# markp-gc/ipu_ray_lib

Measured on AMD Instinct MI355X. Metric: rays/sec (ray casts/s: CompactBvh intersect+occluded calls, whole node), built-in scene 1440x1440 path-trace, higher is better.
Workload: dtype f32

## Files before the change

__graft_entry__.py:

```python
from __future__ import annotations

import os
import shutil
import subprocess
import sys
from pathlib import Path

ROOT = Path(__file__).resolve().parent
PKG = ROOT / "ipu_ray_lib_amd"
CSRC = PKG / "csrc"

HOST_SRCS = [CSRC / "host" / n for n in ("bvh_sah.cpp", "lbvh.cpp", "glb_reader.cpp", "dae_reader.cpp", "scene_builtin.cpp", "scene_api.cpp", "nif_assets.cpp", "point_query_host.cpp", "box_query_host.cpp", "cross_host.cpp", "hot_order.cpp")]
HOST_DEPS = HOST_SRCS + [CSRC / "ray_math.h", CSRC / "hot_order.hpp", CSRC / "point_math.hpp", CSRC / "box_math.hpp", CSRC / "cross_math.hpp", CSRC / "canon_prims.hpp", CSRC / "bvh_cost_host.hpp", CSRC / "scene_blob.hpp", CSRC / "ray_shard.hpp", CSRC / "host" / "scene_types.hpp", CSRC / "host" / "json_min.hpp",
                         ROOT / "include" / "mi_raylib.h", ROOT / "include" / "mi_scene_host.h"]
HIP_SRCS = [CSRC / "raylib.hip"]
HIP_DEPS = HIP_SRCS + [CSRC / "ray_math.h", CSRC / "trace_kernels.hpp", CSRC / "trace_wavefront.hpp", CSRC / "hot_order.hpp", CSRC / "query_kernels.hpp", CSRC / "point_kernels.hpp", CSRC / "point_math.hpp", CSRC / "count_kernels.hpp", CSRC / "list_kernels.hpp", CSRC / "near_kernels.hpp", CSRC / "box_kernels.hpp", CSRC / "box_math.hpp", CSRC / "cross_math.hpp", CSRC / "refit_kernels.hpp", CSRC / "rebuild_kernels.hpp", CSRC / "canon_prims.hpp", CSRC / "canon_kernels.hpp", CSRC / "cost_kernels.hpp", CSRC / "bvh_cost_host.hpp", CSRC / "trace_pool.hpp", CSRC / "nif_kernels.hpp", CSRC / "nif_regs_pack.hpp", CSRC / "nif_regs_kernel.hpp", CSRC / "nif_asm_kernel.hpp", CSRC / "nif_asm_gen.py", CSRC / "scene_blob.hpp", CSRC / "ray_shard.hpp", CSRC / "group_render.hpp", CSRC / "query_drivers.hpp", ROOT / "include" / "mi_raylib.h"]

EXACT_FLAGS = ["-ffp-contract=off", "-fno-fast-math"]


def _deps_hash(deps, flags=()) -> str:
    import hashlib
    h = hashlib.sha256()
    for f in flags:
        h.update(str(f).encode() + b"\0")
    for d in sorted(str(x) for x in deps):
        q = Path(d)
        h.update(q.name.encode() + b"\0")
        if q.exists() and q.is_file():
            h.update(q.read_bytes())
    return h.hexdigest()


def _sidecar(target: Path) -> Path:
    return target.with_name(target.name + ".srchash")


def _stale(target: Path, deps, flags=()) -> bool:
    side = _sidecar(target)
    if not target.exists() or not side.exists():
        return True
    return side.read_text().strip() != _deps_hash(deps, flags)


def _record(target: Path, deps, flags=()) -> None:
    _sidecar(target).write_text(_deps_hash(deps, flags) + "\n")


class StaleBinary(RuntimeError):
    pass


def _run(cmd, **kw):
    if os.environ.get("MI_NO_BUILD") == "1":
        raise StaleBinary(f"stale binary: MI_NO_BUILD=1 forbids running `{' '.join(str(c) for c in cmd[:3])} ...` here; run "
                          "`python3 -c 'import __graft_entry__ as ge; ge.build()'` first, without a profiler")
    print("+", " ".join(str(c) for c in cmd), file=sys.stderr, flush=True)
    try:
        sys.stderr.fileno()
        kw.setdefault("stdout", sys.stderr)
    except (AttributeError, OSError, ValueError):
        kw.setdefault("stdout", sys.__stderr__)
    subprocess.run([str(c) for c in cmd], check=True, **kw)


def build_host() -> Path:
    out = PKG / "libmi_scene_host.so"
    if _stale(out, HOST_DEPS):
        _run(["g++", "-std=c++17", "-O2", *EXACT_FLAGS, "-fPIC", "-Wall", "-shared", "-o", out, *HOST_SRCS, "-ldl"])
        _record(out, HOST_DEPS)
    build_h5_plugin()
    return out


def hdf5_root():
    for cand in (os.environ.get("MI_HDF5_ROOT"), "/opt/conda", "/usr", "/usr/local"):
        if cand and (Path(cand) / "include" / "hdf5.h").exists() and (Path(cand) / "lib" / "libhdf5.so").exists():
            return Path(cand)
    return None


def build_h5_plugin():
    out = PKG / "libmi_nif_h5.so"
    src = CSRC / "host" / "nif_h5.c"
    root = hdf5_root()
    if root is None:
        print("note: no HDF5 installation found; converted.hdf5 NIF models cannot be read (nif_weights.bin still can)", file=sys.stderr)
        return None
    if _stale(out, [src]):
        _run(["gcc", "-std=c11", "-O2", "-fPIC", "-Wall", "-shared", "-I", root / "include", "-o", out, src,
              f"-L{root / 'lib'}", "-lhdf5", f"-Wl,-rpath,{root / 'lib'}"])
        _record(out, [src])
    return out


def build_oracle() -> Path:
    out = ROOT / "oracle" / "libray_oracle.so"
    deps = [ROOT / "oracle" / "ray_oracle.c", ROOT / "oracle" / "ray_oracle.h", ROOT / "oracle" / "Makefile"]
    if _stale(out, deps):
# ... 198 lines not shown
```

include/mi_scene_host.h:

```cpp
#ifndef MI_SCENE_HOST_H
#define MI_SCENE_HOST_H

#include "mi_raylib.h"

#ifdef __cplusplus
extern "C" {
#endif

typedef struct mi_host_scene mi_host_scene;

int mi_host_scene_builtin(const char* scene_name, const char* mesh_file, mi_host_scene** out);

int mi_host_scene_import(const char* file, int load_normals, mi_host_scene** out);

int mi_host_scene_from_arrays(const mi_scene_desc* geometry_only, mi_host_scene** out);

int mi_host_scene_fill_desc(const mi_host_scene* scene, mi_scene_desc* desc);

void mi_host_scene_destroy(mi_host_scene* scene);

int mi_build_compact_bvh(const float* lower, const float* upper, const uint16_t* geom_ids,
                         const uint32_t* prim_ids, uint32_t n,
                         mi_bvh_node* nodes, uint32_t* num_nodes, uint32_t* max_leaf_depth);

int mi_refit_compact_bvh(const mi_scene_desc* desc, mi_bvh_node* out);

int mi_build_lbvh_compact(const mi_scene_desc* desc, mi_bvh_node* out, uint32_t* num_nodes, uint32_t* max_leaf_depth);

int mi_canonical_prims(const mi_scene_desc* desc, void* out , uint32_t capacity, uint32_t* count);

int mi_bvh_cost_compact(const mi_bvh_node* nodes, uint32_t n, double out[3]);
int mi_bvh_cost_compact_block(const mi_bvh_node* nodes, uint32_t n, uint32_t block, double out[3]);
double mi_bvh_cost_estimate(const double cost[3]);

int mi_point_query_host(const mi_scene_desc* desc, int kind, const mi_point* points, void* out, size_t n, uint64_t visits[2]);

int mi_near_offsets_host(const mi_scene_desc* desc, const mi_point* points, uint64_t* offsets , size_t n, uint64_t visits[2]);
int mi_near_fill_host(const mi_scene_desc* desc, const mi_point* points, const uint64_t* offsets, mi_neighbour* hits, size_t capacity,
                      size_t n, uint64_t visits[2]);

int mi_box_query_host(const mi_scene_desc* desc, int kind, const mi_box* boxes, void* out, size_t n, uint64_t visits[2]);
int mi_box_offsets_host(const mi_scene_desc* desc, const mi_box* boxes, uint64_t* offsets , size_t n, uint64_t visits[2]);
int mi_box_fill_host(const mi_scene_desc* desc, const mi_box* boxes, const uint64_t* offsets, mi_overlap* hits, size_t capacity,
                     size_t n, uint64_t visits[2]);

uint32_t mi_sphere_crossings_host(const float centre[3], float radius2, const float origin[3], const float direction[3],
                                  float t_min, float t_max);

uint32_t mi_sphere_roots_host(const float centre[3], float radius2, const float origin[3], const float direction[3],
                              float t_min, float t_max, float t[2]);

int mi_hot_nodes(const mi_bvh_node* compact, uint32_t num_nodes, void* preorder, uint32_t* order, void* hot, uint32_t* leaf_link);

int mi_hot_share(const void* preorder, uint32_t num_nodes, const uint32_t* order, double* share);

uint32_t mi_hot_walk(const void* nodes, uint32_t num_nodes, const uint32_t* leaf_link, const float origin[3], const float direction[3],
                     uint32_t* visits, uint32_t capacity, int* status);

int mi_hot_collapse(const mi_bvh_node* compact, uint32_t num_nodes, double theta, void* preorder, uint8_t* keep, uint32_t* from, void* collapsed,
                    uint32_t* order, void* hot, uint32_t* leaf_link, double* share, uint32_t counts[2]);

int mi_hot_join(const void* thin, const uint32_t* thin_link, uint32_t m, const void* full, const uint32_t* full_link, uint32_t n, void* joined, uint32_t* joined_link,
                uint32_t* exact_start);
int mi_hot_cast_is_literal(const float origin[3], const float direction[3]);

uint32_t mi_hot_walk_count(const void* nodes, uint32_t num_nodes, const uint32_t* leaf_link, uint32_t start, const float origin[3], const float direction[3], float t_max,
                           uint32_t* visits, uint32_t capacity, uint32_t* box_tests, int* status);

int mi_init_ray_stream(const mi_scene_desc* desc, mi_trace_result* rays, size_t capacity);

void mi_scale_rgb(mi_trace_result* rays, size_t n, float scale);

size_t mi_scene_blob_size(const mi_scene_desc* desc);
int mi_scene_serialise(const mi_scene_desc* desc, uint8_t* out, size_t capacity, size_t* written);
int mi_scene_deserialise(const uint8_t* blob, size_t size, mi_scene_desc* desc, size_t* consumed);
uint32_t mi_blob_padding(uint32_t base_align, size_t offset, uint32_t align);

size_t mi_shard_band_rays(size_t n, uint32_t window_w);
size_t mi_shard_count(size_t n, size_t band, uint32_t replicas, uint32_t r);
int mi_shard_stream_index(size_t n, size_t band, uint32_t replicas, uint32_t r, uint64_t* out, size_t capacity);
int mi_shard_frame_index(size_t n, size_t band, uint32_t replicas, uint64_t* out);

typedef struct mi_host_nif mi_host_nif;

typedef struct mi_nif_desc {
  uint32_t num_layers;
  const float* const* kernels;
  const float* const* biases;
  const uint32_t* rows;
  const uint32_t* cols;
  const uint8_t* relu;
  uint32_t embedding_dimension;
  uint32_t hidden_size;
  float max_value;
  float mean[3];
  int32_t log_tonemap;
  int32_t weights_are_half;
  const char* name;
  const char* source;
} mi_nif_desc;

int mi_host_nif_load(const char* asset_path, mi_host_nif** out);
int mi_host_nif_describe(const mi_host_nif* nif, mi_nif_desc* desc);
void mi_host_nif_destroy(mi_host_nif* nif);
const char* mi_host_nif_last_error(void);

const char* mi_host_last_error(void);

#ifdef __cplusplus
}
#endif
#endif
```

ipu_ray_lib_amd/__init__.py:

```python
from __future__ import annotations

import ctypes as C
import os
import sys
from pathlib import Path

import numpy as np

PKG_DIR = Path(__file__).resolve().parent
REPO_ROOT = PKG_DIR.parent
DEFAULT_MESH = REPO_ROOT / "assets" / "monkey_bust.glb"

VEC3 = np.dtype([("x", "<f4"), ("y", "<f4"), ("z", "<f4")])
RAY = np.dtype([("origin", VEC3), ("tMin", "<f4"), ("direction", VEC3), ("tMax", "<f4")])
HIT = np.dtype([("r", RAY), ("primID", "<u4"), ("normal", VEC3), ("throughput", VEC3),
                ("geomID", "<u2"), ("flags", "<u2")])
TRACE_RESULT = np.dtype([("rgb", VEC3), ("u", "<f4"), ("v", "<f4"), ("h", HIT)])
BVH_NODE = np.dtype([("min_x", "<f4"), ("min_y", "<f4"), ("min_z", "<f4"), ("link", "<u4"),
                     ("dx", "<u2"), ("dy", "<u2"), ("dz", "<u2"), ("geomID", "<u2")])
MATERIAL = np.dtype([("albedo", VEC3), ("ior", "<f4"), ("emission", VEC3), ("type", "<i4"),
                     ("emissive", "u1"), ("pad", "u1", (3,))])
MESH_INFO = np.dtype([("firstIndex", "<u4"), ("firstVertex", "<u4"), ("numTriangles", "<u4"), ("numVertices", "<u4")])
GEOM_REF = np.dtype([("index", "<u2"), ("type", "u1"), ("pad", "u1")])
SPHERE = np.dtype([("x", "<f4"), ("y", "<f4"), ("z", "<f4"), ("radius", "<f4")])
# ... 78 lines not shown
class SceneGeometry(C.Structure):
    _fields_ = [("geometry", C.c_void_p), ("num_geometry", C.c_uint32),
                ("mesh_info", C.c_void_p), ("num_meshes", C.c_uint32),
                ("mat_ids", C.c_void_p), ("num_mat_ids", C.c_uint32),
                ("materials", C.c_void_p), ("num_materials", C.c_uint32),
                ("mesh_tris", C.c_void_p), ("num_tris", C.c_uint32),
                ("mesh_verts", C.c_void_p), ("num_verts", C.c_uint32),
                ("mesh_normals", C.c_void_p), ("num_normals", C.c_uint32),
                ("spheres", C.c_void_p), ("num_spheres", C.c_uint32),
                ("discs", C.c_void_p), ("num_discs", C.c_uint32)]

    @classmethod
    def from_desc(cls, desc: "SceneDesc") -> "SceneGeometry":
        g = cls()
        for name, _ in cls._fields_:
            setattr(g, name, getattr(desc, name))
        return g


CANON_PRIM = np.dtype([("a", "<u4"), ("b", "<u4"), ("c", "<u4"), ("kind", "<u4"), ("geomID", "<u4"), ("primID", "<u4"),
                       ("triBase", "<u4"), ("matIndex", "<u4")])
assert CANON_PRIM.itemsize == 32


class NifDesc(C.Structure):
    _fields_ = [("num_layers", C.c_uint32), ("kernels", C.POINTER(C.POINTER(C.c_float))),
                ("biases", C.POINTER(C.POINTER(C.c_float))), ("rows", C.POINTER(C.c_uint32)),
                ("cols", C.POINTER(C.c_uint32)), ("relu", C.POINTER(C.c_uint8)),
                ("embedding_dimension", C.c_uint32), ("hidden_size", C.c_uint32), ("max_value", C.c_float),
                ("mean", C.c_float * 3), ("log_tonemap", C.c_int32), ("weights_are_half", C.c_int32),
                ("name", C.c_char_p), ("source", C.c_char_p)]


class RaylibError(RuntimeError):
    pass


_host = None
_device = {}


def _load(path: Path) -> C.CDLL:
    if not path.exists():
        raise RaylibError(f"{path.name} is not built (run `python -c 'import __graft_entry__ as g; g.build()'` at the repo root)")
    return C.CDLL(str(path))


def host_lib() -> C.CDLL:
    global _host
    if _host is None:
        lib = _load(Path(os.environ["MI_SCENE_HOST_LIB"]) if os.environ.get("MI_SCENE_HOST_LIB") else PKG_DIR / "libmi_scene_host.so")
        lib.mi_host_last_error.restype = C.c_char_p
        lib.mi_host_scene_builtin.argtypes = [C.c_char_p, C.c_char_p, C.POINTER(C.c_void_p)]
        lib.mi_host_scene_import.argtypes = [C.c_char_p, C.c_int, C.POINTER(C.c_void_p)]
        lib.mi_host_scene_from_arrays.argtypes = [C.POINTER(SceneDesc), C.POINTER(C.c_void_p)]
        lib.mi_host_scene_fill_desc.argtypes = [C.c_void_p, C.POINTER(SceneDesc)]
        lib.mi_host_scene_destroy.argtypes = [C.c_void_p]
        lib.mi_host_scene_destroy.restype = None
        lib.mi_build_compact_bvh.argtypes = [C.c_void_p, C.c_void_p, C.c_void_p, C.c_void_p, C.c_uint32,
                                             C.c_void_p, C.POINTER(C.c_uint32), C.POINTER(C.c_uint32)]
        lib.mi_refit_compact_bvh.argtypes = [C.POINTER(SceneDesc), C.c_void_p]
        lib.mi_build_lbvh_compact.argtypes = [C.POINTER(SceneDesc), C.c_void_p, C.POINTER(C.c_uint32), C.POINTER(C.c_uint32)]
        lib.mi_canonical_prims.argtypes = [C.POINTER(SceneDesc), C.c_void_p, C.c_uint32, C.POINTER(C.c_uint32)]
        lib.mi_point_query_host.argtypes = [C.POINTER(SceneDesc), C.c_int, C.c_void_p, C.c_void_p, C.c_size_t, C.POINTER(C.c_uint64)]
        lib.mi_near_offsets_host.argtypes = [C.POINTER(SceneDesc), C.c_void_p, C.c_void_p, C.c_size_t, C.POINTER(C.c_uint64)]
        lib.mi_near_fill_host.argtypes = [C.POINTER(SceneDesc), C.c_void_p, C.c_void_p, C.c_void_p, C.c_size_t, C.c_size_t, C.POINTER(C.c_uint64)]
        lib.mi_box_query_host.argtypes = [C.POINTER(SceneDesc), C.c_int, C.c_void_p, C.c_void_p, C.c_size_t, C.POINTER(C.c_uint64)]
        lib.mi_box_offsets_host.argtypes = [C.POINTER(SceneDesc), C.c_void_p, C.c_void_p, C.c_size_t, C.POINTER(C.c_uint64)]
        lib.mi_box_fill_host.argtypes = [C.POINTER(SceneDesc), C.c_void_p, C.c_void_p, C.c_void_p, C.c_size_t, C.c_size_t, C.POINTER(C.c_uint64)]
        lib.mi_sphere_crossings_host.argtypes = [C.POINTER(C.c_float), C.c_float, C.POINTER(C.c_float), C.POINTER(C.c_float), C.c_float, C.c_float]
        lib.mi_sphere_crossings_host.restype = C.c_uint32
        lib.mi_sphere_roots_host.argtypes = [C.POINTER(C.c_float), C.c_float, C.POINTER(C.c_float), C.POINTER(C.c_float), C.c_float, C.c_float, C.POINTER(C.c_float)]
        lib.mi_sphere_roots_host.restype = C.c_uint32
        lib.mi_hot_nodes.argtypes = [C.c_void_p, C.c_uint32, C.c_void_p, C.c_void_p, C.c_void_p, C.c_void_p]
        lib.mi_hot_walk.argtypes = [C.c_void_p, C.c_uint32, C.c_void_p, C.POINTER(C.c_float), C.POINTER(C.c_float), C.c_void_p, C.c_uint32, C.POINTER(C.c_int)]
        lib.mi_hot_walk.restype = C.c_uint32
        lib.mi_hot_share.argtypes = [C.c_void_p, C.c_uint32, C.c_void_p, C.c_void_p]
        lib.mi_hot_collapse.argtypes = [C.c_void_p, C.c_uint32, C.c_double] + [C.c_void_p] * 8 + [C.POINTER(C.c_uint32)]
        lib.mi_hot_join.argtypes = [C.c_void_p, C.c_void_p, C.c_uint32, C.c_void_p, C.c_void_p, C.c_uint32, C.c_void_p, C.c_void_p, C.POINTER(C.c_uint32)]
        lib.mi_hot_cast_is_literal.argtypes = [C.POINTER(C.c_float), C.POINTER(C.c_float)]
        lib.mi_hot_walk_count.argtypes = [C.c_void_p, C.c_uint32, C.c_void_p, C.c_uint32, C.POINTER(C.c_float), C.POINTER(C.c_float), C.c_float, C.c_void_p, C.c_uint32,
                                          C.POINTER(C.c_uint32), C.POINTER(C.c_int)]
        lib.mi_hot_walk_count.restype = C.c_uint32
        lib.mi_bvh_cost_compact.argtypes = [C.c_void_p, C.c_uint32, C.POINTER(C.c_double)]
        lib.mi_bvh_cost_compact_block.argtypes = [C.c_void_p, C.c_uint32, C.c_uint32, C.POINTER(C.c_double)]
        lib.mi_bvh_cost_estimate.argtypes = [C.POINTER(C.c_double)]
        lib.mi_bvh_cost_estimate.restype = C.c_double
        lib.mi_init_ray_stream.argtypes = [C.POINTER(SceneDesc), C.c_void_p, C.c_size_t]
        lib.mi_scale_rgb.argtypes = [C.c_void_p, C.c_size_t, C.c_float]
        lib.mi_scale_rgb.restype = None
        lib.mi_scene_blob_size.argtypes = [C.POINTER(SceneDesc)]
        lib.mi_scene_blob_size.restype = C.c_size_t
        lib.mi_scene_serialise.argtypes = [C.POINTER(SceneDesc), C.c_void_p, C.c_size_t, C.POINTER(C.c_size_t)]
        lib.mi_scene_deserialise.argtypes = [C.c_void_p, C.c_size_t, C.POINTER(SceneDesc), C.POINTER(C.c_size_t)]
        lib.mi_blob_padding.argtypes = [C.c_uint32, C.c_size_t, C.c_uint32]
        lib.mi_blob_padding.restype = C.c_uint32
        lib.mi_shard_band_rays.argtypes = [C.c_size_t, C.c_uint32]
        lib.mi_shard_band_rays.restype = C.c_size_t
        lib.mi_shard_count.argtypes = [C.c_size_t, C.c_size_t, C.c_uint32, C.c_uint32]
        lib.mi_shard_count.restype = C.c_size_t
        lib.mi_shard_stream_index.argtypes = [C.c_size_t, C.c_size_t, C.c_uint32, C.c_uint32, C.c_void_p, C.c_size_t]
        lib.mi_shard_frame_index.argtypes = [C.c_size_t, C.c_size_t, C.c_uint32, C.c_void_p]
        lib.mi_host_nif_load.argtypes = [C.c_char_p, C.POINTER(C.c_void_p)]
        lib.mi_host_nif_describe.argtypes = [C.c_void_p, C.POINTER(NifDesc)]
        lib.mi_host_nif_destroy.argtypes = [C.c_void_p]
        lib.mi_host_nif_destroy.restype = None
        lib.mi_host_nif_last_error.restype = C.c_char_p
        _host = lib
    return _host


def device_lib(variants: bool = False) -> C.CDLL:
    global _device
    if variants not in _device:
        try:
            import torch
        except ImportError:
            pass
        if variants:
            lib = _load(Path(os.environ["MI_RAYLIB_VARIANTS_LIB"]) if os.environ.get("MI_RAYLIB_VARIANTS_LIB") else PKG_DIR / "libmi_raylib_variants.so")
        else:
            lib = _load(Path(os.environ["MI_RAYLIB_LIB"]) if os.environ.get("MI_RAYLIB_LIB") else PKG_DIR / "libmi_raylib.so")
        lib.mi_last_error.restype = C.c_char_p
        lib.mi_version.restype = C.c_char_p
        lib.mi_scene_create.argtypes = [C.POINTER(SceneDesc), C.POINTER(C.c_void_p)]
        lib.mi_scene_create_from_blob.argtypes = [C.c_void_p, C.c_size_t, C.POINTER(SceneDesc), C.POINTER(C.c_void_p)]
        lib.mi_scene_destroy.argtypes = [C.c_void_p]
        lib.mi_scene_destroy.restype = None
        lib.mi_render.argtypes = [C.c_void_p, C.c_int, C.c_void_p, C.c_size_t, C.c_void_p, C.c_void_p]
        lib.mi_render_device.argtypes = [C.c_void_p, C.c_int, C.c_void_p, C.c_size_t, C.c_void_p]
        lib.mi_trace_time_secs.argtypes = [C.c_void_p]
        lib.mi_trace_time_secs.restype = C.c_double
        lib.mi_get_counters.argtypes = [C.c_void_p, C.POINTER(C.c_uint64)]
        lib.mi_reset_counters.argtypes = [C.c_void_p]
        lib.mi_get_phase_stats.argtypes = [C.c_void_p, C.POINTER(C.c_uint64)]
        lib.mi_scene_set_nif.argtypes = [C.c_void_p, C.c_uint32, C.c_void_p, C.c_void_p, C.c_void_p, C.c_void_p,
                                         C.c_void_p, C.c_uint32, C.c_float, C.c_void_p, C.c_int32]
        lib.mi_scene_set_hdri_rotation.argtypes = [C.c_void_p, C.c_float]
        lib.mi_scene_set_max_nif_batch.argtypes = [C.c_void_p, C.c_size_t]
        lib.mi_scene_set_ray_batch.argtypes = [C.c_void_p, C.c_size_t]
        lib.mi_nif_infer_device.argtypes = [C.c_void_p, C.c_void_p, C.c_void_p, C.c_void_p, C.c_size_t, C.c_void_p]
        lib.mi_query.argtypes = [C.c_void_p, C.c_int, C.c_void_p, C.c_void_p, C.c_size_t]
        lib.mi_scene_update.argtypes = [C.c_void_p, C.POINTER(GeometryUpdate)]
        lib.mi_scene_update_device.argtypes = [C.c_void_p, C.POINTER(GeometryUpdate), C.c_void_p]
        lib.mi_scene_rebuild.argtypes = [C.c_void_p, C.c_void_p, C.POINTER(C.c_uint32)]
        lib.mi_scene_set_geometry.argtypes = [C.c_void_p, C.POINTER(SceneGeometry), C.POINTER(C.c_uint32)]
        lib.mi_scene_set_geometry_device.argtypes = [C.c_void_p, C.POINTER(SceneGeometry), C.c_void_p, C.POINTER(C.c_uint32)]
        lib.mi_get_rebuild_timing.argtypes = [C.c_void_p, C.POINTER(C.c_double)]
        lib.mi_scene_get_bvh.argtypes = [C.c_void_p, C.c_void_p, C.c_uint32, C.POINTER(C.c_uint32)]
        lib.mi_scene_bvh_cost.argtypes = [C.c_void_p, C.c_void_p, C.POINTER(C.c_double)]
        lib.mi_get_live_stats.argtypes = [C.c_void_p, C.POINTER(C.c_uint64)]
        lib.mi_query_device.argtypes = [C.c_void_p, C.c_int, C.c_void_p, C.c_void_p, C.c_size_t, C.c_void_p]
        lib.mi_point_query.argtypes = [C.c_void_p, C.c_int, C.c_void_p, C.c_void_p, C.c_size_t]
        lib.mi_point_query_device.argtypes = [C.c_void_p, C.c_int, C.c_void_p, C.c_void_p, C.c_size_t, C.c_void_p]
        lib.mi_count_query.argtypes = [C.c_void_p, C.c_void_p, C.c_void_p, C.c_size_t]
        lib.mi_count_query_device.argtypes = [C.c_void_p, C.c_void_p, C.c_void_p, C.c_size_t, C.c_void_p]
        lib.mi_list_offsets.argtypes = [C.c_void_p, C.c_void_p, C.c_void_p, C.c_size_t]
        lib.mi_list_offsets_device.argtypes = [C.c_void_p, C.c_void_p, C.c_void_p, C.c_size_t, C.c_void_p]
        lib.mi_list_fill.argtypes = [C.c_void_p, C.c_void_p, C.c_void_p, C.c_void_p, C.c_size_t, C.c_size_t]
        lib.mi_list_fill_device.argtypes = [C.c_void_p, C.c_void_p, C.c_void_p, C.c_void_p, C.c_size_t, C.c_size_t, C.c_void_p]
        lib.mi_near_offsets.argtypes = [C.c_void_p, C.c_void_p, C.c_void_p, C.c_size_t]
        lib.mi_near_offsets_device.argtypes = [C.c_void_p, C.c_void_p, C.c_void_p, C.c_size_t, C.c_void_p]
        lib.mi_near_fill.argtypes = [C.c_void_p, C.c_void_p, C.c_void_p, C.c_void_p, C.c_size_t, C.c_size_t]
        lib.mi_near_fill_device.argtypes = [C.c_void_p, C.c_void_p, C.c_void_p, C.c_void_p, C.c_size_t, C.c_size_t, C.c_void_p]
        lib.mi_box_query.argtypes = [C.c_void_p, C.c_int, C.c_void_p, C.c_void_p, C.c_size_t]
        lib.mi_box_query_device.argtypes = [C.c_void_p, C.c_int, C.c_void_p, C.c_void_p, C.c_size_t, C.c_void_p]
# ... 228 lines not shown
    _check_host(host_lib().mi_box_query_host(C.byref(desc), int(kind), src.ctypes.data if src.size else None,
                                             out.ctypes.data if src.size else None, src.size, visits))
    return (out.view(np.bool_) if kind == BOX_ANY else out), {"box_tests": int(visits[0]), "prim_evals": int(visits[1])}


def box_offsets_host(desc: SceneDesc, boxes: np.ndarray):
    assert boxes.dtype == BOX and boxes.ndim == 1
    src = np.ascontiguousarray(boxes)
    offsets = np.zeros(src.size + 1, np.uint64)
    visits = (C.c_uint64 * 2)()
    _check_host(host_lib().mi_box_offsets_host(C.byref(desc), src.ctypes.data if src.size else None, offsets.ctypes.data, src.size, visits))
    return offsets, {"box_tests": int(visits[0]), "prim_evals": int(visits[1])}


def box_fill_host(desc: SceneDesc, boxes: np.ndarray, offsets: np.ndarray, capacity: int | None = None, hits: np.ndarray | None = None):
    assert boxes.dtype == BOX and boxes.ndim == 1
    src = np.ascontiguousarray(boxes)
    offsets = np.ascontiguousarray(offsets, np.uint64)
    assert offsets.ndim == 1 and offsets.size == src.size + 1
    if hits is None:
        size = int(offsets.max()) if capacity is None else int(capacity)
        hits = np.zeros(max(size, 1), OVERLAP)[:size]
    assert hits.dtype == OVERLAP and hits.flags["C_CONTIGUOUS"]
    capacity = hits.size if capacity is None else int(capacity)
    assert 0 <= capacity <= hits.size
    visits = (C.c_uint64 * 2)()
    base = hits.ctypes.data if hits.size else np.zeros(1, OVERLAP).ctypes.data
    _check_host(host_lib().mi_box_fill_host(C.byref(desc), src.ctypes.data if src.size else None, offsets.ctypes.data, base, capacity, src.size, visits))
    return hits, {"box_tests": int(visits[0]), "prim_evals": int(visits[1])}


DEVICE_NODE = np.dtype([("box", "<f4", (6,)), ("link", "<u4"), ("hit", "<u4")])


def hot_nodes(nodes: np.ndarray) -> dict:
    nodes = np.ascontiguousarray(nodes, dtype=BVH_NODE)
    n = nodes.size
    out = {"preorder": np.zeros(n, DEVICE_NODE), "order": np.zeros(n, np.uint32), "hot": np.zeros(n, DEVICE_NODE), "leaf_link": np.zeros(n, np.uint32)}
    _check_host(host_lib().mi_hot_nodes(nodes.ctypes.data if n else None, n, *[out[k].ctypes.data if n else None for k in ("preorder", "order", "hot", "leaf_link")]))
    out["share"] = np.zeros(n, np.float64)
    _check_host(host_lib().mi_hot_share(out["preorder"].ctypes.data if n else None, n, out["order"].ctypes.data if n else None, out["share"].ctypes.data if n else None))
    return out


def hot_walk(device_nodes: np.ndarray, origin, direction, leaf_link: np.ndarray | None = None) -> np.ndarray:
    assert device_nodes.dtype == DEVICE_NODE and device_nodes.flags.c_contiguous
    o, d = ((C.c_float * 3)(*[float(np.float32(x)) for x in v]) for v in (origin, direction))
    link = None if leaf_link is None else np.ascontiguousarray(leaf_link, np.uint32)
    cap = 4 * device_nodes.size + 4
    visits = np.zeros(cap, np.uint32)
    status = C.c_int(0)
    cnt = host_lib().mi_hot_walk(device_nodes.ctypes.data, device_nodes.size, None if link is None else link.ctypes.data, o, d, visits.ctypes.data, cap, C.byref(status))
    _check_host(status.value)
    return visits[:min(cnt, cap)].copy()


def hot_collapse(nodes: np.ndarray, theta: float = -1.0) -> dict:
    nodes = np.ascontiguousarray(nodes, dtype=BVH_NODE)
    n = nodes.size
    out = {"preorder": np.zeros(n, DEVICE_NODE), "keep": np.zeros(n, np.uint8), "from": np.zeros(n, np.uint32), "collapsed": np.zeros(n, DEVICE_NODE),
           "order": np.zeros(n, np.uint32), "hot": np.zeros(n, DEVICE_NODE), "leaf_link": np.zeros(n, np.uint32), "share": np.zeros(n, np.float64)}
    counts = (C.c_uint32 * 2)()
    _check_host(host_lib().mi_hot_collapse(nodes.ctypes.data if n else None, n, float(theta),
                                           *[out[k].ctypes.data if n else None for k in ("preorder", "keep", "from", "collapsed", "order", "hot", "leaf_link", "share")], counts))
    m = int(counts[0])
    for k in ("from", "collapsed", "order", "hot", "leaf_link", "share"):
        out[k] = out[k][:m].copy()
    out["blocked"] = int(counts[1])
    return out


def hot_join(collapse: dict, full: dict) -> dict:
    m, n = collapse["hot"].size, full["hot"].size
    out = {"nodes": np.zeros(m + n, DEVICE_NODE), "leaf_link": np.zeros(m + n, np.uint32)}
    start = C.c_uint32(0)
    ptr = lambda a: a.ctypes.data if a.size else None
    _check_host(host_lib().mi_hot_join(ptr(collapse["hot"]), ptr(collapse["leaf_link"]), m, ptr(full["hot"]), ptr(full["leaf_link"]), n, ptr(out["nodes"]), ptr(out["leaf_link"]),
                                       C.byref(start)))
    out["exact_start"] = int(start.value)
    out["place"] = np.concatenate([collapse["from"][collapse["order"]], full["order"]]).astype(np.uint32)
    return out


def hot_cast_is_literal(origin, direction) -> bool:
    o, d = ((C.c_float * 3)(*[float(np.float32(x)) for x in v]) for v in (origin, direction))
    return bool(host_lib().mi_hot_cast_is_literal(o, d))


def hot_walk_count(device_nodes: np.ndarray, origin, direction, leaf_link: np.ndarray | None = None, t_max: float = float("inf"), start: int = 0):
    assert device_nodes.dtype == DEVICE_NODE and device_nodes.flags.c_contiguous
    o, d = ((C.c_float * 3)(*[float(np.float32(x)) for x in v]) for v in (origin, direction))
    link = None if leaf_link is None else np.ascontiguousarray(leaf_link, np.uint32)
    cap = 4 * device_nodes.size + 4
    visits = np.zeros(cap, np.uint32)
    status, tests = C.c_int(0), C.c_uint32(0)
    cnt = host_lib().mi_hot_walk_count(device_nodes.ctypes.data, device_nodes.size, None if link is None else link.ctypes.data, int(start), o, d, C.c_float(float(np.float32(t_max))),
                                       visits.ctypes.data, cap, C.byref(tests), C.byref(status))
    _check_host(status.value)
    return visits[:min(cnt, cap)].copy(), int(tests.value)


def sphere_crossings_host(centre, radius2, origin, direction, t_min=0.0, t_max=float("inf")) -> int:
    c, o, d = ((C.c_float * 3)(*[float(np.float32(x)) for x in v]) for v in (centre, origin, direction))
    return int(host_lib().mi_sphere_crossings_host(c, C.c_float(float(np.float32(radius2))), o, d, C.c_float(float(np.float32(t_min))),
                                                   C.c_float(float(np.float32(t_max)))))


def sphere_roots_host(centre, radius2, origin, direction, t_min=0.0, t_max=float("inf")):
    c, o, d = ((C.c_float * 3)(*[float(np.float32(x)) for x in v]) for v in (centre, origin, direction))
    t = (C.c_float * 2)(float("nan"), float("nan"))
    mask = int(host_lib().mi_sphere_roots_host(c, C.c_float(float(np.float32(radius2))), o, d, C.c_float(float(np.float32(t_min))),
                                               C.c_float(float(np.float32(t_max))), t))
    return mask, float(t[0]), float(t[1])


def _geometry_array(a, dtype, width):
    if a is None:
        return None
    a = np.asarray(a)
    if a.dtype != dtype:
        a = np.ascontiguousarray(a, dtype=np.float32)
        if a.ndim != 2 or a.shape[1] != width:
            raise ValueError(f"expected a {dtype} array or an [n, {width}] float32 array, got shape {a.shape}")
        return a.view(dtype).reshape(-1)
    return np.ascontiguousarray(a).reshape(-1)


def serialise_scene(desc: SceneDesc) -> np.ndarray:
    lib = host_lib()
    n = lib.mi_scene_blob_size(C.byref(desc))
    out = aligned_bytes(n)
    written = C.c_size_t()
    _check_host(lib.mi_scene_serialise(C.byref(desc), out.ctypes.data, n, C.byref(written)))
    assert written.value == n
    return out


def deserialise_scene(blob: np.ndarray, into: SceneDesc | None = None) -> SceneDesc:
    d = into if into is not None else SceneDesc()
    used = C.c_size_t()
    _check_host(host_lib().mi_scene_deserialise(blob.ctypes.data, blob.size, C.byref(d), C.byref(used)))
    d._blob = blob
    d._blob_bytes_used = used.value
    return d


class NifAssets:

    def __init__(self, asset_path):
        lib = host_lib()
        h = C.c_void_p()
        if lib.mi_host_nif_load(os.fspath(asset_path).encode(), C.byref(h)) != 0:
            raise RaylibError(lib.mi_host_nif_last_error().decode())
        try:
            d = NifDesc()
            if lib.mi_host_nif_describe(h, C.byref(d)) != 0:
                raise RaylibError(lib.mi_host_nif_last_error().decode())
            self.kernels, self.biases, self.relu = [], [], []
            for i in range(d.num_layers):
                r, c = int(d.rows[i]), int(d.cols[i])
                self.kernels.append(np.ctypeslib.as_array(d.kernels[i], shape=(r, c)).copy())
                self.biases.append(np.ctypeslib.as_array(d.biases[i], shape=(c,)).copy() if d.biases[i] else None)
                self.relu.append(bool(d.relu[i]))
            self.embedding_dimension = int(d.embedding_dimension)
            self.hidden_size = int(d.hidden_size)
            self.max_value = float(d.max_value)
# ... 681 lines not shown
```

ipu_ray_lib_amd/csrc/ray_math.h:

```cpp
#pragma once

#include <stdint.h>
#include <string.h>
#include <math.h>

#if defined(__HIPCC__)
#define MI_HD __host__ __device__ __forceinline__
#else
#define MI_HD inline
#endif

namespace mi {

struct f3 { float x, y, z; };

MI_HD f3 mk(float x, float y, float z) { f3 r; r.x = x; r.y = y; r.z = z; return r; }
MI_HD f3 operator+(f3 a, f3 b) { return mk(a.x + b.x, a.y + b.y, a.z + b.z); }
MI_HD f3 operator-(f3 a, f3 b) { return mk(a.x - b.x, a.y - b.y, a.z - b.z); }
MI_HD f3 operator*(f3 a, f3 b) { return mk(a.x * b.x, a.y * b.y, a.z * b.z); }
MI_HD f3 operator*(f3 a, float s) { return mk(a.x * s, a.y * s, a.z * s); }
MI_HD f3 operator-(f3 a) { return mk(-a.x, -a.y, -a.z); }
MI_HD f3 abs3(f3 a) { return mk(fabsf(a.x), fabsf(a.y), fabsf(a.z)); }
MI_HD float dot(f3 a, f3 b) { return a.x * b.x + a.y * b.y + a.z * b.z; }
MI_HD float sqnorm(f3 a) { return a.x * a.x + a.y * a.y + a.z * a.z; }
// ... 217 lines not shown
  return out;
}
MI_HD float rng_uniform01(Rng& r) {
  const uint64_t bits = (0x3FFull << 52) | (rng_next(r) >> 12);
  double d;
  __builtin_memcpy(&d, &bits, 8);
  return (float)(d - 1.0);
}

MI_HD uint32_t f2u_sat(float f) {
  if (!(f > 0.f)) return 0u;
  if (f >= 4294967296.f) return 0xFFFFFFFFu;
  return (uint32_t)f;
}
constexpr uint32_t kSegmentSamplesMin = 4, kSegmentSamplesMax = 64, kSegmentsPerPixel = 16;
MI_HD uint32_t segment_shift(uint32_t samplesPerPixel) {
  const uint32_t want = (samplesPerPixel + kSegmentsPerPixel - 1) / kSegmentsPerPixel;
  const uint32_t shift = want <= 1u ? 0u : 32u - (uint32_t)__builtin_clz(want - 1u);
  return shift < 2u ? 2u : shift > 6u ? 6u : shift;
}
MI_HD uint32_t segment_samples(uint32_t samplesPerPixel) { return 1u << segment_shift(samplesPerPixel); }
MI_HD void rng_seed_pixel_segment(Rng& r, uint64_t userSeed, float row, float col, uint32_t segment) {
  const uint64_t pix = ((uint64_t)f2u_sat(row) << 32) | (uint64_t)f2u_sat(col);
  rng_seed(r, (userSeed ^ ((pix + 1ull) * 0x9e3779b97f4a7c15ull)) ^ ((uint64_t)segment * 0xd1b54a32d192ed03ull));
}
MI_HD void rng_seed_pixel(Rng& r, uint64_t userSeed, float row, float col) { rng_seed_pixel_segment(r, userSeed, row, col, 0u); }

MI_HD float log_det(float x) {
  uint32_t b;
  __builtin_memcpy(&b, &x, 4);
  int e = (int)((b >> 23) & 0xFFu) - 126;
  const uint32_t mb = (b & 0x007FFFFFu) | 0x3F000000u;
  float m;
  __builtin_memcpy(&m, &mb, 4);
  if (m < 0.707106781186547524f) { e -= 1; m = m + m - 1.0f; }
  else { m = m - 1.0f; }
  float z = m * m;
  float y = 7.0376836292e-2f;
  y = y * m + -1.1514610310e-1f;
  y = y * m + 1.1676998740e-1f;
  y = y * m + -1.2420140846e-1f;
  y = y * m + 1.4249322787e-1f;
  y = y * m + -1.6668057665e-1f;
  y = y * m + 2.0000714765e-1f;
  y = y * m + -2.4999993993e-1f;
  y = y * m + 3.3333331174e-1f;
  y = y * m * z;
  const float fe = (float)e;
  y = y + -2.12194440e-4f * fe;
  y = y + -0.5f * z;
  z = m + y;
  z = z + 0.693359375f * fe;
  return z;
}
MI_HD void rng_gauss2(Rng& r, const float* sinTbl, float& g0, float& g1) {
  const float ua = rng_uniform01(r);
  const float ub = rng_uniform01(r);
  float w = 1.f - ua;
  if (w < 2.98023223876953125e-08f) w = 2.98023223876953125e-08f;
  const float rad = sqrtf(-2.f * log_det(w));
  float sn, cs;
  sincos_deg_table(6.283185307179586f * ub, sinTbl, sn, cs);
  g0 = rad * cs;
  g1 = rad * sn;
}

MI_HD f3 pixel_to_ray_dir(float x, float y, float w, float h, float tanTheta) {
  const float aspect = w / h;
  x = (x / w) - .5f;
  y = (y / h) - .5f;
  return normalized(mk(2.f * x * aspect * tanTheta, -2.f * y * tanTheta, -1.f));
}

MI_HD f3 offset_origin(f3 origin, f3 dir, f3 n) {
  const float m = (1.f + min_comp(abs3(origin))) * kRayEpsilon * copysignf(1.f, dot(n, dir));
  return origin + n * m;
}

MI_HD void sample_disc_concentric(float u1, float u2, const float* sinTbl, float& ox, float& oy) {
  const float ux = 2.f * u1 - 1.f, uy = 2.f * u2 - 1.f;
  if (ux == 0.f && uy == 0.f) { ox = ux; oy = uy; return; }
  const float piby4 = (float)(3.14159265358979323846264338327950288 / 4.0);
  const float piby2 = (float)(3.14159265358979323846264338327950288 / 2.0);
  float r, th;
  if (fabsf(ux) > fabsf(uy)) { r = ux; th = piby4 * (uy / ux); }
  else { r = uy; th = piby2 - piby4 * (ux / uy); }
  float s, c;
  sincos_deg_table(th, sinTbl, s, c);
  ox = r * c; oy = r * s;
}
MI_HD f3 cosine_sample_hemisphere(float u1, float u2, const float* sinTbl) {
  float x, y;
  sample_disc_concentric(u1, u2, sinTbl, x, y);
  const float z = sqrtf(fmaxf(0.f, 1.f - x * x - y * y));
  return mk(x, y, z);
}
MI_HD f3 sample_diffuse(f3 n, float u1, float u2, const float* sinTbl) {
  f3 xb;
  const f3 a = abs3(n), sq = n * n;
  if (a.x > a.y) { const float il = 1.f / sqrtf(sq.x + sq.z); xb = mk(-n.z * il, 0.f, n.x * il); }
  else { const float il = 1.f / sqrtf(sq.y + sq.z); xb = mk(0.f, n.z * il, -n.y * il); }
  const f3 yb = cross(n, xb);
  const f3 wi = cosine_sample_hemisphere(u1, u2, sinTbl);
  return mk(dot(mk(xb.x, yb.x, n.x), wi), dot(mk(xb.y, yb.y, n.y), wi), dot(mk(xb.z, yb.z, n.z), wi));
}
MI_HD f3 reflect_dir(f3 d, f3 n) {
  const float cosTheta = dot(d, n);
  return normalized(d - n * (cosTheta * 2.f));
}
MI_HD float schlick(float cosTheta, float ri) {
  float r0 = (1.f - ri) / (1.f + ri);
  r0 = r0 * r0;
  const float base = 1.f - cosTheta;
  const float base2 = base * base;
  const float base5 = base2 * base * base2;
  return r0 + (1.f - r0) * base5;
}
MI_HD f3 refract_dir(f3 dir, f3 n, float ndotr, float ri) {
  const float cosTheta = -ndotr;
  const f3 rPerp = (dir + n * cosTheta) * ri;
  const f3 rPar = n * -sqrtf(fabsf(1.f - sqnorm(rPerp)));
  return rPerp + rPar;
}
MI_HD bool dielectric(f3 dir, f3 n, float ri, float u1, f3& out) {
  if (dot(n, dir) > 0.f) n = -n; else ri = 1.f / ri;
  const float ndotr = dot(n, dir);
  const float cost1 = -ndotr;
  const float cost2 = 1.f - ri * ri * (1.f - cost1 * cost1);
  if (cost2 > 0.f && u1 > schlick(cost1, ri)) { out = refract_dir(dir, n, ndotr, ri); return true; }
  out = reflect_dir(dir, n);
  return false;
}
MI_HD bool roulette_stop(float u1, f3& tp) {
  const float p = min_comp(tp);
  if (p == 0.f || u1 > p) return true;
  tp = tp * (1.f / p);
  return false;
}

#define MI_SIN_TABLE_BITS \
  0x00000000u, 0x3c8ef859u, 0x3d0ef2c6u, 0x3d565e3au, 0x3d8edc7bu, 0x3db27eb6u, 0x3dd61305u, 0x3df996a2u, \
  0x3e0e8365u, 0x3e20305bu, 0x3e31d0d4u, 0x3e43636fu, 0x3e54e6cdu, 0x3e665992u, 0x3e77ba60u, 0x3e8483eeu, \
  0x3e8d2057u, 0x3e95b1beu, 0x3e9e377au, 0x3ea6b0dfu, 0x3eaf1d44u, 0x3eb77c01u, 0x3ebfcc6fu, 0x3ec80de9u, \
  0x3ed03fc9u, 0x3ed8616cu, 0x3ee0722fu, 0x3ee87171u, 0x3ef05e94u, 0x3ef838f7u, 0x3f000000u, 0x3f03d989u, \
  0x3f07a8cau, 0x3f0b6d77u, 0x3f0f2744u, 0x3f12d5e8u, 0x3f167918u, 0x3f1a108du, 0x3f1d9bfeu, 0x3f211b24u, \
  0x3f248dbbu, 0x3f27f37cu, 0x3f2b4c25u, 0x3f2e9772u, 0x3f31d522u, 0x3f3504f3u, 0x3f3826a7u, 0x3f3b39ffu, \
  0x3f3e3ebdu, 0x3f4134a6u, 0x3f441b7du, 0x3f46f30au, 0x3f49bb13u, 0x3f4c7360u, 0x3f4f1bbdu, 0x3f51b3f3u, \
  0x3f543bceu, 0x3f56b31du, 0x3f5919aeu, 0x3f5b6f51u, 0x3f5db3d7u, 0x3f5fe714u, 0x3f6208dau, 0x3f641901u, \
  0x3f66175eu, 0x3f6803cau, 0x3f69de1du, 0x3f6ba635u, 0x3f6d5becu, 0x3f6eff20u, 0x3f708fb2u, 0x3f720d81u, \
  0x3f737871u, 0x3f74d063u, 0x3f76153fu, 0x3f7746eau, 0x3f78654du, 0x3f797051u, 0x3f7a67e2u, 0x3f7b4bebu, \
  0x3f7c1c5cu, 0x3f7cd925u, 0x3f7d8235u, 0x3f7e1781u, 0x3f7e98fdu, 0x3f7f069eu, 0x3f7f605cu, 0x3f7fa62fu, \
  0x3f7fd814u, 0x3f7ff605u, 0x3f800000u, 0x3f7ff605u

}
```

ipu_ray_lib_amd/csrc/raylib.hip:

```cpp
#include <hip/hip_runtime.h>

#include <algorithm>
#include <chrono>
#include <cmath>
#include <cstdio>
#include <cstring>
#include <map>
#include <stdexcept>
#include <string>
#include <vector>

#include "../../include/mi_raylib.h"
#include "ray_math.h"
#include "trace_kernels.hpp"
#include "trace_wavefront.hpp"
#include "hot_order.hpp"
#include "query_kernels.hpp"
#include "point_kernels.hpp"
#include "count_kernels.hpp"
#include "list_kernels.hpp"
#include "near_kernels.hpp"
#include "box_kernels.hpp"
#include "refit_kernels.hpp"
#include "rebuild_kernels.hpp"
// ... 19 lines not shown
static_assert(sizeof(mi_ray) == 32, "Ray layout");
static_assert(sizeof(mi_bvh_node) == 24, "CompactBVH2Node layout");
static_assert(sizeof(mi_material) == 36, "Material layout");
static_assert(sizeof(mi_mesh_info) == 16 && sizeof(mi_geom_ref) == 4, "MeshInfo/GeomRef layout");
static_assert(offsetof(mi_trace_result, u) == 12 && offsetof(mi_trace_result, h) == 20, "TraceResult offsets");
static_assert(offsetof(mi_hit_record, prim_id) == 32 && offsetof(mi_hit_record, normal) == 36 &&
              offsetof(mi_hit_record, throughput) == 48 && offsetof(mi_hit_record, geom_id) == 60 &&
              offsetof(mi_hit_record, flags) == 62, "HitRecord offsets");
static_assert(sizeof(mi_query_hit) == 32 && offsetof(mi_query_hit, prim_id) == 4 && offsetof(mi_query_hit, geom_id) == 8 &&
              offsetof(mi_query_hit, flags) == 10 && offsetof(mi_query_hit, normal) == 12 && offsetof(mi_query_hit, b1) == 24 &&
              offsetof(mi_query_hit, b2) == 28, "mi_query_hit layout");
static_assert(sizeof(mi_point) == 16 && offsetof(mi_point, radius) == 12, "mi_point layout");
static_assert(sizeof(mi_point_hit) == 32 && offsetof(mi_point_hit, prim_id) == 4 && offsetof(mi_point_hit, geom_id) == 8 &&
              offsetof(mi_point_hit, flags) == 10 && offsetof(mi_point_hit, point) == 12 && offsetof(mi_point_hit, b1) == 24 &&
              offsetof(mi_point_hit, b2) == 28, "mi_point_hit layout");

namespace {

thread_local std::string g_err;

struct DeviceError : std::runtime_error { using std::runtime_error::runtime_error; };
struct ArgError : std::runtime_error { using std::runtime_error::runtime_error; };

#define HIP_CHECK(expr)                                                                      \
  do {                                                                                       \
    hipError_t _e = (expr);                                                                  \
    if (_e != hipSuccess)                                                                    \
      throw DeviceError(std::string(#expr) + ": " + hipGetErrorString(_e));                  \
  } while (0)

template <class F>
int guarded(F&& f) {
  try { f(); g_err.clear(); return MI_OK; }
  catch (const ArgError& e) { g_err = e.what(); return MI_ERR_INVALID_ARG; }
  catch (const DeviceError& e) { g_err = e.what(); return MI_ERR_DEVICE; }
  catch (const std::exception& e) { g_err = e.what(); return MI_ERR_DEVICE; }
  catch (...) { g_err = "unknown exception (not derived from std::exception)"; return MI_ERR_DEVICE; }
}

template <class T>
T* upload(const std::vector<T>& v) {
  if (v.empty()) return nullptr;
  T* d = nullptr;
  HIP_CHECK(hipMalloc(&d, v.size() * sizeof(T)));
  HIP_CHECK(hipMemcpy(d, v.data(), v.size() * sizeof(T), hipMemcpyHostToDevice));
  return d;
}

const float* hostSinTable() {
  static const uint32_t bits[92] = {MI_SIN_TABLE_BITS};
  static float tbl[92];
  static bool init = false;
  if (!init) { memcpy(tbl, bits, sizeof tbl); init = true; }
  return tbl;
}

}

constexpr uint32_t kNifSplDefault = 512, kNifSplMax = 1024;
constexpr int kHotNodesAuto = -1;
constexpr double kHotAutoShare = 0.9;
constexpr uint32_t kHotThreads = 768;
constexpr uint32_t kLdsPerCU = 160 * 1024, kLdsGranule = 1280;
struct SceneOptions {
  bool fullStats = false;
  WaveTune tune = kDefaultTune;
  int kernelChoice = 1;
#if MI_RAYLIB_VARIANTS
  PoolTune poolTune;
#endif
  uint32_t cus = 0;
  std::string why;
  int poolWaves = 4;
  int wavesPerSimd = 6;
  bool mergeTurns = true;
  bool specLeaf = false;
  bool tiles = true;
  size_t segBudgetKb = (size_t)8 * 1024 * 1024;
  uint32_t nifSamplesPerLaunch = 0;
  bool pin = true;
  uint32_t nifShape = 7;
  bool leafRot = true;
  bool leanHit = true;
  bool coords = true;
  int nifOverlap = -1;
  uint32_t nifTraceWgs = 0;
  uint32_t nifSplit = 0;
  bool nifFirstTest = false;
  bool nifTiming = false;
  bool refitTiming = false;
  bool rebuildTiming = false;
  uint32_t nifGenerations = kNifGenerations;
  bool rootStart = true;
  bool sayGrid = false;
  bool doubleFallback = false;
  bool fast = false;
  int queryKernel = 0;
  QueryTune queryTune = kDefaultQueryTune;
  int hotNodes = kHotNodesAuto;
  double autoRebuild = 0.0;

  static bool flag01(const char* v, bool& out) {
    if ((v[0] != '0' && v[0] != '1') || v[1] != '\0') return false;
    out = v[0] == '1';
    return true;
  }
  static bool number(const char* v, unsigned long long lo, unsigned long long hi, unsigned long long& out) {
    if (!*v) return false;
    char* end = nullptr;
    const unsigned long long q = strtoull(v, &end, 10);
    if (!end || *end != '\0' || v[0] == '-' || q < lo || q > hi) return false;
    out = q;
    return true;
  }
  static bool autoRebuildValue(const char* v, double& out) {
    if (!v || !*v) return false;
    if (!strcmp(v, "0")) { out = 0.0; return true; }
    for (const char* c = v; *c; ++c) if (!((*c >= '0' && *c <= '9') || *c == '.' || *c == 'e' || *c == 'E' || *c == '+' || *c == '-')) return false;
    char* end = nullptr;
    const double r = strtod(v, &end);
    if (!end || end == v || *end != '\0' || !(r > 1.0) || !std::isfinite(r)) return false;
    out = r;
    return true;
  }
  bool set(const std::string& key, const char* v) {
    why = "unknown option or bad value";
    if (!v) return false;
    unsigned long long q = 0;
    if (key == "full_stats") {
      bool b = fullStats;
      if (!flag01(v, b)) return false;
      if (b && fast) { why = "full_stats cannot be combined with fast (the tolerance tier has no instrumented build)"; return false; }
      fullStats = b; return true;
    }
#if MI_RAYLIB_VARIANTS
    if (fast && (key == "kernel" || key == "waves" || key == "spec" || key == "merge" || key == "tune")) {
      SceneOptions probe = *this; probe.fast = false;
      if (!probe.set(key, v)) { why = probe.why; return false; }
      if (probe.kernelChoice != 1 || probe.specLeaf || probe.wavesPerSimd != 6 || !probe.mergeTurns || !(probe.tune == kDefaultTune)) {
        why = "fast is a build of the default kernel only (kernel 1, 6 waves, one SHADE / GEN turn, default weights, no spec): clear fast first"; return false;
      }
      return true;
    }
    if (key == "kernel") { if (!number(v, 0, 3, q)) return false; kernelChoice = (int)q; return true; }
    if (key == "pool_waves") { if (!number(v, 4, 16, q) || (q != 4 && q != 8 && q != 16)) return false; poolWaves = (int)q; return true; }
    if (key == "pool_tune") {
      unsigned a, b, c, d, e, f, db = 4, mx = 5, ln = 1, pr = 1;
      if (sscanf(v, "%u,%u,%u,%u,%u,%u,%u,%u,%u,%u", &a, &b, &c, &d, &e, &f, &db, &mx, &ln, &pr) < 6) return false;
      poolTune = {a, b, c ? c : 1, d ? d : 1, e, f, db ? db : 65, mx, ln, pr};
      return true;
    }
    if (key == "waves") { if (!number(v, 4, 7, q)) return false; wavesPerSimd = (int)q; return true; }
    if (key == "spec") return flag01(v, specLeaf);
    if (key == "merge") return flag01(v, mergeTurns);
#else
    if (key == "kernel") {
      if (!number(v, 0, 3, q)) return false;
      if (q > 1) { why = "kernel 2 / 3 are not compiled into this library (the variants build, -DMI_RAYLIB_VARIANTS=1, has them)"; return false; }
      kernelChoice = (int)q; return true;
    }
    if (key == "pool_waves" || key == "pool_tune" || key == "tune") { why = "not compiled into this library (the variants build, -DMI_RAYLIB_VARIANTS=1, has it)"; return false; }
    if (key == "waves") { if (!number(v, 4, 7, q)) return false; if (q != 6) { why = "the 4-, 5- and 7-wave builds are not compiled into this library (variants build)"; return false; } return true; }
    if (key == "merge") { bool b = true; if (!flag01(v, b)) return false; if (!b) { why = "the two-turn form is not compiled into this library (variants build)"; return false; } return true; }
    if (key == "spec") { bool b = false; if (!flag01(v, b)) return false; if (b) { why = "the speculative walk is not compiled into this library (variants build)"; return false; } return true; }
#endif
    if (key == "cus") { if (!number(v, 0, 4096, q)) return false; cus = (uint32_t)q; return true; }
    if (key == "tiles") return flag01(v, tiles);
    if (key == "seg_budget_kb") { if (!number(v, 1, ~0ull >> 12, q)) return false; segBudgetKb = (size_t)q; return true; }
    if (key == "nif_spl") { if (!number(v, 0, kNifSplMax, q)) return false; nifSamplesPerLaunch = (uint32_t)q; return true; }
    if (key == "pin") return flag01(v, pin);
    if (key == "nif_timing") return flag01(v, nifTiming);
    if (key == "refit_timing") return flag01(v, refitTiming);
    if (key == "rebuild_timing") return flag01(v, rebuildTiming);
    if (key == "nif_generations") { if (!number(v, 1, 4096, q)) return false; nifGenerations = (uint32_t)q; return true; }
    if (key == "root_start") return flag01(v, rootStart);
    if (key == "say_grid") return flag01(v, sayGrid);
    if (key == "nif_overlap") { if (!strcmp(v, "auto")) { nifOverlap = -1; return true; } bool on = false; if (!flag01(v, on)) return false; nifOverlap = on ? 1 : 0; return true; }
    if (key == "nif_first_test") return flag01(v, nifFirstTest);
    if (key == "nif_split") { if (!number(v, 0, 1024, q)) return false; nifSplit = (uint32_t)q; return true; }
    if (key == "nif_trace_wgs") { if (!number(v, 0, 16, q)) return false; nifTraceWgs = (uint32_t)q; return true; }
    if (key == "coords") return flag01(v, coords);
    if (key == "query_kernel") { if (!number(v, 0, 1, q)) return false; queryKernel = (int)q; return true; }
    if (key == "query_tune") {
      unsigned a, b, c, dd, e;
      char tail = 0;
      if (sscanf(v, "%u,%u,%u,%u,%u%c", &a, &b, &c, &dd, &e, &tail) != 5) return false;
      if (b == 0 || dd == 0 || e > 8 || c > 64) return false;
      queryTune = {a, b, c, dd, e};
      return true;
    }
    if (key == "lean_hit") return flag01(v, leanHit);
    if (key == "auto_rebuild") { if (!autoRebuildValue(v, autoRebuild)) { why = "auto_rebuild takes 0 (off) or a decimal ratio above 1"; return false; } return true; }
    if (key == "leaf_rot") return flag01(v, leafRot);
    if (key == "hot_nodes") { if (!strcmp(v, "auto")) { hotNodes = kHotNodesAuto; return true; } if (!number(v, 0, 65535, q)) return false; hotNodes = (int)q; return true; }
    if (key == "double_fallback") {
      bool b = doubleFallback;
      if (!flag01(v, b)) return false;
      if (b && fast) { why = "double_fallback cannot be combined with fast"; return false; }
      doubleFallback = b; return true;
    }
    if (key == "fast") {
      bool b = fast;
      if (!flag01(v, b)) return false;
      if (b && (fullStats || doubleFallback)) { why = "fast cannot be combined with full_stats or double_fallback"; return false; }
#if MI_RAYLIB_VARIANTS
      if (b && (kernelChoice != 1 || specLeaf || wavesPerSimd != 6 || !mergeTurns || !(tune == kDefaultTune))) { why = "fast is a build of the default kernel only (kernel 1, 6 waves, one SHADE / GEN turn, default weights, no spec)"; return false; }
#endif
      fast = b; return true;
    }
    if (key == "nif_shape") {
      const std::string s(v);
      if (s == "w6") nifShape = 0; else if (s == "t6") nifShape = 1; else if (s == "t4") nifShape = 2; else if (s == "a8") nifShape = 6; else if (s == "auto") nifShape = 7; else if (s == "b4") nifShape = 8;
#if MI_RAYLIB_VARIANTS
      else if (s == "r8") nifShape = 4; else if (s == "r8s") nifShape = 5;
#else
      else if (s == "r8" || s == "r8s") { why = "K3r (nif_shape r8 / r8s) is not compiled into this library (the variants build, -DMI_RAYLIB_VARIANTS=1, has it)"; return false; }
#endif
      else return false;
      return true;
    }
#if MI_RAYLIB_VARIANTS
    if (key == "tune") {
      unsigned a, b, c, dd = 48, k8 = 3, db = 4, mx = 6, ln = 1, pr = 1, lp = 40, pb = 0;
      if (sscanf(v, "%u,%u,%u,%u,%u,%u,%u,%u,%u,%u,%u", &a, &b, &c, &dd, &k8, &db, &mx, &ln, &pr, &lp, &pb) < 3) return false;
      if (mx > 7 || pb > 3) return false;
      tune = {a, b, c, dd, k8, db ? db : 65, mx, ln, pr, lp ? lp : 1, pb};
      return true;
    }
#endif
    return false;
  }
  void fromEnvironment() {
    static const char* const map[][2] = {{"MI_RAYLIB_FULL_STATS", "full_stats"}, {"MI_RAYLIB_KERNEL", "kernel"}, {"MI_RAYLIB_WAVES", "waves"}, {"MI_RAYLIB_SPEC", "spec"},
                                         {"MI_RAYLIB_SEG_BUDGET_KB", "seg_budget_kb"}, {"MI_RAYLIB_NIF_SPL", "nif_spl"}, {"MI_RAYLIB_PIN", "pin"},
                                         {"MI_RAYLIB_NIF_SHAPE", "nif_shape"}, {"MI_RAYLIB_TUNE", "tune"},
                                         {"MI_RAYLIB_POOL_TUNE", "pool_tune"}, {"MI_RAYLIB_POOL_WAVES", "pool_waves"}, {"MI_RAYLIB_CUS", "cus"},
                                         {"MI_RAYLIB_NIF_OVERLAP", "nif_overlap"}, {"MI_RAYLIB_COORDS", "coords"},
                                         {"MI_RAYLIB_NIF_TRACE_WGS", "nif_trace_wgs"}, {"MI_RAYLIB_NIF_SPLIT", "nif_split"}, {"MI_RAYLIB_NIF_GENERATIONS", "nif_generations"},
                                         {"MI_RAYLIB_HOT_NODES", "hot_nodes"}};
    for (const auto& m : map) if (const char* e = getenv(m[0])) (void)set(m[1], e);
    if (getenv("MI_RAYLIB_NO_TILES")) tiles = false;
    if (getenv("MI_RAYLIB_NO_ROOT_START")) rootStart = false;
    if (getenv("MI_RAYLIB_SAY_GRID")) sayGrid = true;
  }
};

struct LaunchSlot {
  hipStream_t stream = nullptr;
  uint32_t* d_workCounter = nullptr;
  float* d_segPart = nullptr; size_t segPartFloats = 0;
  float2* d_coords = nullptr; size_t coordsCap = 0;
  uint32_t* d_poolScratch = nullptr; size_t poolScratchWords = 0;
  hipEvent_t lastWork = nullptr;
  uint64_t* d_scanSums = nullptr; size_t scanSumsCap = 0;
};

struct mi_scene {
  int device = 0;
  int numCUs = 256;
  mi_scene_desc params{};
  DeviceScene ds{};
  SceneOptions opt;
  std::vector<void*> allocations;
  unsigned long long* d_counters = nullptr;
  std::vector<LaunchSlot> slots;
  std::map<const void*, int> residentPerCU;
  uint32_t cus() const { return opt.cus ? opt.cus : (uint32_t)numCUs; }
  bool nifOverlapOn() const { return opt.nifOverlap < 0 ? (opt.nifSplit > 0 || !((opt.nifShape >= 6 && opt.nifShape <= 8) && nif_asm_covers(nif.regs))) : opt.nifOverlap != 0; }
  DeviceScene view() const { DeviceScene v = ds; if (!opt.rootStart) v.rootInterior = 0; return v; }
  struct HotCopy { const GNode* nodes = nullptr; const GLeaf* leaves = nullptr; const GLeafRot* rot = nullptr; const float* leafNormals = nullptr; bool valid = false;
                   uint32_t numNodes = 0, thinNodes = 0, exactBase = 0;
                   std::vector<double> share; } hot, thin;
  DeviceScene hotView(const HotCopy& c) const { DeviceScene v = view(); v.nodes = c.nodes; v.numNodes = c.numNodes; v.exactBase = c.exactBase; v.leaves = c.leaves; v.leavesRot = c.rot; v.leafNormals = c.leafNormals; return v; }
  DeviceScene& touchArrays() { hot.valid = false; thin.valid = false; return ds; }
  void freeRetiredHot() {
    if (hot.valid || thin.valid) return;
    for (const HotCopy* c : {&hot, &thin})
      for (const void* p : {(const void*)c->nodes, (const void*)c->leaves, (const void*)c->rot, (const void*)c->leafNormals}) release(p);
    hot = HotCopy{};
    thin = HotCopy{};
  }
  bool hotRoomSaid = false;
  std::map<const void*, uint32_t> hotRoomOf;
  uint32_t hotRoom(const void* kern, int threads) {
    auto it = hotRoomOf.find(kern);
    if (it != hotRoomOf.end()) return it->second;
    hipFuncAttributes fa{};
    int nb0 = 0;
    uint32_t room = 0;
    if (hipFuncGetAttributes(&fa, kern) == hipSuccess && hipOccupancyMaxActiveBlocksPerMultiprocessor(&nb0, kern, threads, 0) == hipSuccess && nb0 > 0) {
      long bytes = ((long)(kLdsPerCU / (uint32_t)nb0 / kLdsGranule * kLdsGranule) - (long)fa.sharedSizeBytes) & ~31L;
      for (; bytes >= 32; bytes -= 256) {
        int nb = 0;
        if (hipOccupancyMaxActiveBlocksPerMultiprocessor(&nb, kern, threads, (size_t)bytes) == hipSuccess && nb >= nb0) break;
      }
      if (bytes >= 32) room = (uint32_t)bytes;
    }
    (void)hipGetLastError();
    if (room && hipFuncSetAttribute(kern, hipFuncAttributeMaxDynamicSharedMemorySize, (int)room) != hipSuccess) { (void)hipGetLastError(); room = 0; }
    if (!room && !hotRoomSaid) {
      hotRoomSaid = true;
      fprintf(stderr, "mi_raylib: option hot_nodes: the runtime leaves no LDS for hot nodes beside a %d-thread workgroup's own; rendering from the shared arrays\n", threads);
    }
    hotRoomOf.emplace(kern, room);
    return room;
  }
  uint32_t residentBlocks(const void* kern, int threads, size_t ldsBytes) {
    auto it = residentPerCU.find(kern);
    if (it == residentPerCU.end()) {
      int nb = 0;
      if (hipOccupancyMaxActiveBlocksPerMultiprocessor(&nb, kern, threads, ldsBytes) != hipSuccess || nb <= 0) { (void)hipGetLastError(); nb = 8; }
      it = residentPerCU.emplace(kern, nb).first;
    }
    return (uint32_t)it->second;
  }
  bool poolAttrSet[2][3] = {{false, false, false}, {false, false, false}};
  bool ldsAttrSet[2] = {false, false};
  hipEvent_t nifDone = nullptr; bool nifPending = false;
  mi_trace_result* d_batch[2] = {nullptr, nullptr}; size_t batchCap[2] = {0, 0};
  hipStream_t pipeStream[2] = {nullptr, nullptr};
  double traceTimeSecs = 0.0;
  float hdriRotationDegrees = 0.f;
  size_t maxNifBatch = 0;
  size_t rayBatch = 0;
  void* d_qRays[2] = {nullptr, nullptr}; void* d_qOut[2] = {nullptr, nullptr}; size_t qCap[2] = {0, 0};
  NifDevice nif;
  struct NifSlots {
    float* u = nullptr; float* v = nullptr; float* bgr = nullptr; float* color = nullptr; float* tp = nullptr;
    uint32_t* index = nullptr; uint32_t* count = nullptr;
    hipEvent_t traced = nullptr, done = nullptr; bool donePending = false;
  } nifSlots[2];
  hipStream_t nifAux = nullptr;
  hipStream_t debugStream = nullptr;
  hipStream_t nifSplitMlp = nullptr, nifSplitTrace = nullptr;
  uint32_t splitUnits = 0; bool splitRefused = false;
  hipEvent_t splitFirst = nullptr;
  Rng* d_rng = nullptr; size_t scratchRays = 0;
  float* d_segTotal = nullptr;
  uint32_t scratchSamples = 0;
  uint32_t scratchAsked = 0;
  bool scratchOneSet = false;
  std::vector<std::pair<hipEvent_t, hipEvent_t>> nifTimes;
  struct Refit {
    std::vector<mi_bvh_node> nodes;
    bool tables = false; uint32_t levelCap = 0;
    std::vector<uint32_t> matIds;
    std::vector<mi_geom_ref> geometry; std::vector<mi_mesh_info> meshInfo; std::vector<uint16_t> tris;
    std::vector<mi_vec3> verts; std::vector<mi_sphere> spheres; std::vector<mi_disc> discs;
    uint32_t numVerts = 0, numNormals = 0, numSpheres = 0, numDiscs = 0;
    bool ready = false;
    RefitPrim* d_prims = nullptr;
    uint32_t* d_order = nullptr;
    std::vector<uint32_t> levelStart; uint32_t* d_levelStart = nullptr;
    uint32_t topFirst = 0;
    RefitBox* d_boxes = nullptr;
    mi_bvh_node* d_cnodes[2] = {nullptr, nullptr}; int live = -1;
// ... 163 lines not shown
        const mi_disc& c = d.discs[r.index];
        L.f[0] = c.nx; L.f[1] = c.ny; L.f[2] = c.nz; L.f[3] = c.cx; L.f[4] = c.cy; L.f[5] = c.cz; L.f[6] = c.r * c.r;
        L.type = LEAF_DISC | ((uint32_t)n.geom_id << 16); L.primID = 0;
      }
      L.matIndex = d.mat_ids[n.geom_id];
      g.hit = (skip[i] << 5) | kLeafFlag;
      leaves[i] = L;
      isLeafNode[i] = 1;
    }
    nodes[i] = g;
  }

  DeviceScene& ds = S.ds;
  ds.nodes = S.keep(upload(nodes)); ds.numNodes = N;
  ds.leaves = S.keep(upload(leaves)); ds.numLeaves = (uint32_t)leaves.size();
  struct Private { mi_scene::HotCopy* copy; std::vector<uint32_t> at, link; std::vector<GNode> nodes; } priv[2] = {{&S.hot, {}, {}, {}}, {&S.thin, {}, {}, {}}};
  {
    const HotNode* pre = reinterpret_cast<const HotNode*>(nodes.data());
    std::vector<uint8_t> keepNode(N);
    const uint32_t M = hot_collapse_keep(pre, N, kHotCollapseTheta, keepNode.data(), nullptr);
    std::vector<HotNode> thinPre(M);
    std::vector<uint32_t> thinFrom(M);
    hot_collapse_nodes(pre, N, keepNode.data(), thinPre.data(), thinFrom.data());
    need(M == 0 || (thinFrom[0] == 0 && (M == 1 || (thinPre[0].hit == 32u) == !node_is_leaf(nodes[0]))), "the collapsed tree lost its root");
    for (int c = 0; c < 2; ++c) {
      const HotNode* src = c ? thinPre.data() : pre;
      const uint32_t n = c ? M : N;
      std::vector<uint32_t> order(n);
      priv[c].nodes.resize(n);
      priv[c].link.resize(n);
      hot_first_order(src, n, order.data());
      hot_permute_nodes(src, n, order.data(), reinterpret_cast<HotNode*>(priv[c].nodes.data()), priv[c].link.data());
      priv[c].copy->share.resize(n);
      if (c) hot_prefix_share_any(src, n, order.data(), S.thin.share.data()); else hot_prefix_share(src, n, order.data(), S.hot.share.data());
      priv[c].at.resize(n);
      for (uint32_t k = 0; k < n; ++k) priv[c].at[k] = c ? thinFrom[order[k]] : order[k];
      priv[c].copy->numNodes = priv[c].copy->thinNodes = n;
    }
    {
      std::vector<GNode> joined(M + N);
      std::vector<uint32_t> joinedLink(M + N);
      hot_join_regions(reinterpret_cast<const HotNode*>(priv[1].nodes.data()), priv[1].link.data(), M, reinterpret_cast<const HotNode*>(priv[0].nodes.data()), priv[0].link.data(), N,
                       reinterpret_cast<HotNode*>(joined.data()), joinedLink.data());
      priv[1].nodes.swap(joined);
      priv[1].link.swap(joinedLink);
      priv[1].at.insert(priv[1].at.end(), priv[0].at.begin(), priv[0].at.end());
      S.thin.numNodes = M + N;
      S.thin.exactBase = M << 5;
    }
    for (Private& p : priv) p.copy->nodes = S.keep(upload(p.nodes));
    for (Private& p : priv) {
      std::vector<GLeaf> hotLeaves(p.at.size());
      for (uint32_t k = 0; k < p.at.size(); ++k) { hotLeaves[k] = leaves[p.at[k]]; if (isLeafNode[p.at[k]]) hotLeaves[k].triBase = p.link[k]; }
      p.copy->leaves = S.keep(upload(hotLeaves));
    }
  }
  {
    std::vector<GLeafRot> rot(leaves.size());
    memset(rot.data(), 0, rot.size() * sizeof(GLeafRot));
    for (size_t i = 0; i < leaves.size(); ++i)
      for (uint32_t kz = 0; kz < 3; ++kz) {
        GLeafBlock& B = rot[i].b[kz];
        B.type = leaves[i].type;
        for (int q = 0; q < 9; ++q) B.f[q] = leaves[i].f[q];
        if (leaf_kind(leaves[i]) == LEAF_TRI) {
          const uint32_t kx = (kz + 1) % 3, ky = (kz + 2) % 3;
          for (int v = 0; v < 3; ++v) { B.f[3 * v] = leaves[i].f[3 * v + kx]; B.f[3 * v + 1] = leaves[i].f[3 * v + ky]; B.f[3 * v + 2] = leaves[i].f[3 * v + kz]; }
        }
      }
    ds.leavesRot = S.keep(upload(rot));
    for (Private& p : priv) {
      std::vector<GLeafRot> hotRot(p.at.size());
      for (uint32_t k = 0; k < p.at.size(); ++k) {
        hotRot[k] = rot[p.at[k]];
        if (isLeafNode[p.at[k]]) for (uint32_t kz = 0; kz < 3; ++kz) hotRot[k].b[kz].type = p.link[k] | leaf_kind(leaves[p.at[k]]);
      }
      p.copy->rot = S.keep(upload(hotRot));
    }
  }
  ds.matIDs = S.keep(upload(std::vector<uint32_t>(d.mat_ids, d.mat_ids + d.num_mat_ids)));
  ds.materials = S.keep(upload(std::vector<mi_material>(d.materials, d.materials + d.num_materials)));
  ds.numMaterials = d.num_materials;
  ds.hasNormals = d.num_normals ? 1u : 0u;
  ds.leafNormals = nullptr;
  S.hot.leafNormals = S.thin.leafNormals = nullptr;
  S.hot.valid = S.thin.valid = true;
  if (ds.hasNormals) {
    std::vector<float> ln(9 * leaves.size(), 0.f);
    for (size_t k = 0; k < leaves.size(); ++k) {
      const GLeaf& L = leaves[k];
      if (!isLeafNode[k] || leaf_kind(L) != LEAF_TRI) continue;
      const uint32_t fv = geomFirstVertex[leaf_geom(L)];
      for (int c = 0; c < 3; ++c) {
        const size_t at = (size_t)fv + d.mesh_tris[L.triBase + c];
        need(at < d.num_normals, "vertex normal index out of range");
        const mi_vec3& nn = d.mesh_normals[at];
        ln[9 * k + 3 * c] = nn.x; ln[9 * k + 3 * c + 1] = nn.y; ln[9 * k + 3 * c + 2] = nn.z;
      }
    }
    ds.leafNormals = S.keep(upload(ln));
    for (Private& p : priv) {
      std::vector<float> hotLn(9 * p.at.size());
      for (uint32_t k = 0; k < p.at.size(); ++k) memcpy(&hotLn[9 * (size_t)k], &ln[9 * (size_t)p.at[k]], 9 * sizeof(float));
      p.copy->leafNormals = S.keep(upload(hotLn));
    }
    ds.meshTris = S.keep(upload(std::vector<uint16_t>(d.mesh_tris, d.mesh_tris + 3 * (size_t)d.num_tris)));
    ds.meshNormals = S.keep(upload(std::vector<mi_vec3>(d.mesh_normals, d.mesh_normals + d.num_normals)));
    ds.geomFirstVertex = S.keep(upload(geomFirstVertex));
  }
  ds.rootInterior = 0;
  if (N > 1) {
    ds.rootLoX = nodes[0].minx; ds.rootHiX = nodes[0].maxx; ds.rootLoY = nodes[0].miny; ds.rootHiY = nodes[0].maxy;
    ds.rootLoZ = nodes[0].minz; ds.rootHiZ = nodes[0].maxz; ds.rootInterior = node_is_leaf(nodes[0]) ? 0u : 1u;
  }
  ds.imageWidth = d.image_width; ds.imageHeight = d.image_height;
  float s, c;
  sincos_deg_table(d.fov_radians / 2.f, hostSinTable(), s, c);
  ds.tanTheta = s / c;
  ds.antiAliasScale = d.anti_alias_scale;
  ds.maxPathLength = d.max_path_length; ds.rouletteStartDepth = d.roulette_start_depth;
  ds.samplesPerPixel = d.samples_per_pixel;
  ds.rngSeed = d.rng_seed;
  HIP_CHECK(hipMalloc(&S.d_counters, 32 * sizeof(unsigned long long)));
  S.keep(S.d_counters);
  HIP_CHECK(hipMemset(S.d_counters, 0, 32 * sizeof(unsigned long long)));
  ds.counters = S.d_counters;

  mi_scene::Refit& R = S.refit;
  R.nodes.assign(d.bvh_nodes, d.bvh_nodes + N);
  R.geometry.assign(d.geometry, d.geometry + d.num_geometry);
  R.matIds.assign(d.mat_ids, d.mat_ids + d.num_geometry);
  R.meshInfo.assign(d.mesh_info, d.mesh_info + d.num_meshes);
  R.tris.assign(d.mesh_tris, d.mesh_tris + (d.num_meshes ? 3 * (size_t)d.num_tris : 0));
  R.verts.assign(d.mesh_verts, d.mesh_verts + (d.num_meshes ? d.num_verts : 0));
  R.spheres.assign(d.spheres, d.spheres + d.num_spheres);
  R.discs.assign(d.discs, d.discs + d.num_discs);
  R.numVerts = d.num_meshes ? d.num_verts : 0; R.numNormals = d.num_normals; R.numSpheres = d.num_spheres; R.numDiscs = d.num_discs;
}

void refitAlloc(mi_scene& S) {
  mi_scene::Refit& R = S.refit;
  if (R.ready) return;
  const uint32_t N = (uint32_t)R.nodes.size();
  if (N) {
    HIP_CHECK(hipMalloc(&R.d_prims, (size_t)N * sizeof(RefitPrim)));
    S.keep(R.d_prims);
    HIP_CHECK(hipMalloc(&R.d_order, (size_t)N * sizeof(uint32_t)));
    S.keep(R.d_order);
    HIP_CHECK(hipMalloc(&R.d_boxes, (size_t)N * sizeof(RefitBox)));
    S.keep(R.d_boxes);
  }
  R.d_cnodes[0] = S.keep(upload(R.nodes));
  R.d_cnodes[1] = S.keep(upload(R.nodes));
  HIP_CHECK(hipMalloc(&R.d_err, sizeof(uint32_t)));
  S.keep(R.d_err);
  R.d_verts = S.keep(upload(R.verts));
  R.d_spheres = S.keep(upload(R.spheres));
  R.d_discs = S.keep(upload(R.discs));
  R.verts = {}; R.spheres = {}; R.discs = {};
  R.ready = true;
}

void refitLevelRoom(mi_scene& S, mi_scene::Refit& R, uint32_t entries) {
  if (entries <= R.levelCap) return;
  R.levelCap = 2 * entries;
  HIP_CHECK(hipMalloc(&R.d_levelStart, R.levelCap * sizeof(uint32_t)));
  S.keep(R.d_levelStart);
}

void refitTopFirst(mi_scene::Refit& R) {
  const uint32_t H = (uint32_t)R.levelStart.size() - 2;
  R.topFirst = H + 1;
  while (R.topFirst > 1 && R.levelStart[R.topFirst] - R.levelStart[R.topFirst - 1] <= kRefitTopThreads) --R.topFirst;
}

void refitTables(mi_scene& S) {
  mi_scene::Refit& R = S.refit;
  refitAlloc(S);
  if (R.tables) return;
  ++S.live.hostDerivations;
  const uint32_t N = (uint32_t)R.nodes.size();
  std::vector<RefitPrim> prims(N);
  std::vector<uint32_t> height(N, 0);
  for (uint32_t i = N; i-- > 0;) {
    const mi_bvh_node& n = R.nodes[i];
    RefitPrim p{0u, 0u, 0u, REFIT_INTERIOR};
    if (n.geom_id == MI_INVALID_GEOM) {
      p.a = n.prim_or_second_child;
      height[i] = 1 + std::max(height[i + 1], height[p.a]);
    } else {
      const mi_geom_ref& r = R.geometry[n.geom_id];
      if (r.type == 0) {
        const mi_mesh_info& m = R.meshInfo[r.index];
        const size_t base = 3 * ((size_t)m.first_index + n.prim_or_second_child);
        p = {m.first_vertex + R.tris[base], m.first_vertex + R.tris[base + 1], m.first_vertex + R.tris[base + 2], REFIT_TRI};
      } else {
        p = {r.index, 0u, 0u, r.type == 1 ? (uint32_t)REFIT_SPHERE : (uint32_t)REFIT_DISC};
      }
    }
    prims[i] = p;
  }
  const uint32_t H = N ? height[0] : 0;
  R.levelStart.assign(H + 2, 0);
  for (uint32_t i = 0; i < N; ++i) ++R.levelStart[height[i] + 1];
  for (uint32_t h = 0; h <= H; ++h) R.levelStart[h + 1] += R.levelStart[h];
  std::vector<uint32_t> order(N), at(R.levelStart.begin(), R.levelStart.end() - 1);
  for (uint32_t i = 0; i < N; ++i) order[at[height[i]]++] = i;
  refitTopFirst(R);
  refitLevelRoom(S, R, (uint32_t)R.levelStart.size());
  HIP_CHECK(hipMemcpy(R.d_levelStart, R.levelStart.data(), R.levelStart.size() * sizeof(uint32_t), hipMemcpyHostToDevice));
  if (N) {
    HIP_CHECK(hipMemcpy(R.d_prims, prims.data(), (size_t)N * sizeof(RefitPrim), hipMemcpyHostToDevice));
    HIP_CHECK(hipMemcpy(R.d_order, order.data(), (size_t)N * sizeof(uint32_t), hipMemcpyHostToDevice));
  }
  R.tables = true;
}

void sceneCost(mi_scene& S, hipStream_t stream, double out[3]) {
  const uint32_t N = S.ds.numNodes;
  mi_scene::Live& L = S.live;
  const mi_scene::Refit& R = S.refit;
  ++L.costEvals;
  out[0] = out[1] = out[2] = 0.0;
  if (!N) return;
  if (R.live < 0) { bvh_cost_host(R.nodes.data(), N, kCostBlock, out); return; }
  uint32_t sizes[8]; int levels = 0;
  uint32_t total = 0;
  for (uint32_t n = N;;) { n = cost_blocks(n, kCostBlock); sizes[levels++] = n; total += n; if (n == 1) break; }
  if (!L.d_cost) { HIP_CHECK(hipMalloc(&L.d_cost, ((size_t)total + 1) * sizeof(Cost2))); S.keep(L.d_cost); }
  auto levelAt = [&](int k) { uint32_t at = 1; for (int j = levels - 1; j > k; --j) at += sizes[j]; return L.d_cost + at; };
  hipLaunchKernelGGL(cost_term_kernel, dim3(sizes[0]), dim3(kCostBlock), 0, stream, R.d_cnodes[R.live], N, levelAt(0), &L.d_cost[0].all);
  for (int k = 1; k < levels; ++k)
    hipLaunchKernelGGL(cost_partials_kernel, dim3(sizes[k]), dim3(kCostBlock), 0, stream, levelAt(k - 1), sizes[k - 1], levelAt(k));
  HIP_CHECK(hipGetLastError());
  Cost2 back[2];
  HIP_CHECK(hipMemcpyAsync(back, L.d_cost, sizeof back, hipMemcpyDeviceToHost, stream));
  HIP_CHECK(hipStreamSynchronize(stream));
  out[0] = back[1].all; out[1] = back[1].leaf; out[2] = back[0].all;
}

void updateArgs(const char* fn, const mi_scene* S, const mi_geometry_update* u) {
  auto bad = [&](const char* why) { throw ArgError(std::string(fn) + ": " + why); };
  if (!S) bad("null scene");
  if (!u) bad("null update");
  if ((!u->mesh_verts && u->num_verts) || (!u->mesh_normals && u->num_normals) || (!u->spheres && u->num_spheres) || (!u->discs && u->num_discs))
    bad("a count without its array");
  const mi_scene::Refit& R = S->refit;
  if (u->mesh_verts && u->num_verts != R.numVerts) bad("num_verts differs from the scene's vertex count");
  if (u->mesh_normals && R.numNormals == 0) bad("normals given to a scene created without normals");
  if (u->mesh_normals && u->num_normals != R.numNormals) bad("num_normals differs from the scene's normal count");
  if (u->spheres && u->num_spheres != R.numSpheres) bad("num_spheres differs from the scene's sphere count");
  if (u->discs && u->num_discs != R.numDiscs) bad("num_discs differs from the scene's disc count");
}

uint32_t rebuildScene(mi_scene& S, hipStream_t stream);
void refitScene(mi_scene& S, const mi_geometry_update& u, hipStream_t stream) {
  refitTables(S);
  mi_scene::Refit& R = S.refit;
  DeviceScene& ds = S.touchArrays();
  const uint32_t N = ds.numNodes;
  RefitGeom g;
  g.verts = u.mesh_verts ? (const mi_vec3*)u.mesh_verts : R.d_verts;
  g.spheres = u.spheres ? u.spheres : R.d_spheres;
  g.discs = u.discs ? u.discs : R.d_discs;
  g.normals = u.mesh_normals;
  const int scratch = R.live == 0 ? 1 : 0;
  mi_bvh_node* cn = R.d_cnodes[scratch];
  mi_bvh_node root{};
  const bool timing = S.opt.refitTiming && N;
  if (timing && !R.ev[0]) for (hipEvent_t& e : R.ev) HIP_CHECK(hipEventCreate(&e));
  if (N) {
    HIP_CHECK(hipMemsetAsync(R.d_err, 0, sizeof(uint32_t), stream));
    const uint32_t leaves = R.levelStart[1];
    if (timing) HIP_CHECK(hipEventRecord(R.ev[0], stream));
    hipLaunchKernelGGL(refit_leaf_kernel, dim3((leaves + 255) / 256), dim3(256), 0, stream, R.d_order, leaves, R.d_prims, g, R.d_boxes, cn, R.d_err);
    if (timing) HIP_CHECK(hipEventRecord(R.ev[1], stream));
    for (uint32_t h = 1; h < R.topFirst; ++h) {
      const uint32_t cnt = R.levelStart[h + 1] - R.levelStart[h];
      hipLaunchKernelGGL(refit_level_kernel, dim3((cnt + 255) / 256), dim3(256), 0, stream, R.d_order, R.levelStart[h], cnt, R.d_prims, R.d_boxes, cn, R.d_err);
    }
    const uint32_t H = (uint32_t)R.levelStart.size() - 2;
    if (R.topFirst <= H)
      hipLaunchKernelGGL(refit_top_kernel, dim3(1), dim3(kRefitTopThreads), 0, stream, R.d_order, R.d_levelStart, R.topFirst, H, R.d_prims, R.d_boxes, cn, R.d_err);
    HIP_CHECK(hipGetLastError());
    if (timing) HIP_CHECK(hipEventRecord(R.ev[2], stream));
    uint32_t err = 0;
    HIP_CHECK(hipMemcpyAsync(&err, R.d_err, sizeof err, hipMemcpyDeviceToHost, stream));
    HIP_CHECK(hipMemcpyAsync(&root, cn, sizeof root, hipMemcpyDeviceToHost, stream));
    HIP_CHECK(hipStreamSynchronize(stream));
    if (timing) {
      float a = 0.f, b = 0.f;
      HIP_CHECK(hipEventElapsedTime(&a, R.ev[0], R.ev[1])); HIP_CHECK(hipEventElapsedTime(&b, R.ev[1], R.ev[2]));
      R.ms[0] = a; R.ms[1] = b;
    }
    if (err) ++S.live.refused;
    if (err & (1u << kBoxNotFinite)) throw ArgError("mi_scene_update: a node box is not finite; the scene is unchanged");
    if (err) throw ArgError("mi_scene_update: a node extent is above 65504 (Cannot compress BVH bounds into fp16 (half)); the scene is unchanged");
  }
  const double ratio = S.opt.autoRebuild;
  if (ratio > 0.0 && N && !S.live.baselineValid) {
    double c[3];
    sceneCost(S, stream, c);
    S.live.baseline = bvh_cost_estimate(c); S.live.baselineValid = true;
  }
  for (LaunchSlot& l : S.slots) if (l.stream != stream) HIP_CHECK(hipStreamWaitEvent(stream, l.lastWork, 0));
  if (N) {
    if (timing) HIP_CHECK(hipEventRecord(R.ev[3], stream));
    hipLaunchKernelGGL(refit_write_kernel, dim3((N + 255) / 256), dim3(256), 0, stream, N, R.d_prims, cn, g, const_cast<GNode*>(ds.nodes),
                       const_cast<GLeaf*>(ds.leaves), const_cast<GLeafRot*>(ds.leavesRot), const_cast<float*>(ds.leafNormals));
    HIP_CHECK(hipGetLastError());
  }
  if (u.mesh_verts && R.numVerts) HIP_CHECK(hipMemcpyAsync(R.d_verts, u.mesh_verts, (size_t)R.numVerts * sizeof(mi_vec3), hipMemcpyDeviceToDevice, stream));
  if (u.spheres && R.numSpheres) HIP_CHECK(hipMemcpyAsync(R.d_spheres, u.spheres, (size_t)R.numSpheres * sizeof(mi_sphere), hipMemcpyDeviceToDevice, stream));
  if (u.discs && R.numDiscs) HIP_CHECK(hipMemcpyAsync(R.d_discs, u.discs, (size_t)R.numDiscs * sizeof(mi_disc), hipMemcpyDeviceToDevice, stream));
  if (u.mesh_normals && ds.meshNormals)
    HIP_CHECK(hipMemcpyAsync(const_cast<mi_vec3*>(ds.meshNormals), u.mesh_normals, (size_t)R.numNormals * sizeof(mi_vec3), hipMemcpyDeviceToDevice, stream));
  if (timing) HIP_CHECK(hipEventRecord(R.ev[1], stream));
  HIP_CHECK(hipStreamSynchronize(stream));
  if (timing) { float w = 0.f; HIP_CHECK(hipEventElapsedTime(&w, R.ev[3], R.ev[1])); R.ms[2] = w; }
  ++S.live.applied;
  S.freeRetiredHot();
  if (!N) return;
  R.live = scratch;
  if (N > 1) {
    ds.rootLoX = root.min_x; ds.rootHiX = root.min_x + half_bits_to_float(root.dx);
    ds.rootLoY = root.min_y; ds.rootHiY = root.min_y + half_bits_to_float(root.dy);
    ds.rootLoZ = root.min_z; ds.rootHiZ = root.min_z + half_bits_to_float(root.dz);
  }
  if (ratio > 0.0) {
    double c[3];
    sceneCost(S, stream, c);
    if (c[2] > 0.0 && bvh_cost_estimate(c) > ratio * S.live.baseline) {
      rebuildScene(S, stream);
      ++S.live.autoRebuilds;
    }
  }
}

template <class K>
void rebuildSort(mi_scene::Rebuild& B, K* keys[2], uint32_t* vals[2], uint32_t n, unsigned endBit, hipStream_t stream, K*& keysOut, uint32_t*& valsOut) {
  rocprim::double_buffer<K> kb(keys[0], keys[1]);
  rocprim::double_buffer<uint32_t> vb(vals[0], vals[1]);
  size_t bytes = B.sortTmpBytes;
  HIP_CHECK(rocprim::radix_sort_pairs(B.d_sortTmp, bytes, kb, vb, n, 0u, endBit, stream));
  keysOut = kb.current(); valsOut = vb.current();
}
template <class K>
size_t rebuildSortBytes(uint32_t n, unsigned endBit) {
  rocprim::double_buffer<K> kb(nullptr, nullptr);
  rocprim::double_buffer<uint32_t> vb(nullptr, nullptr);
  size_t bytes = 0;
  HIP_CHECK(rocprim::radix_sort_pairs(nullptr, bytes, kb, vb, n, 0u, endBit, (hipStream_t) nullptr));
  return bytes;
}

void rebuildScratch(mi_scene& S, mi_scene::Rebuild& B, uint32_t P) {
  const size_t N = 2 * (size_t)P - 1;
  const uint32_t I = P - 1;
  const size_t sortBytes = std::max({rebuildSortBytes<uint64_t>(P, 3 * kMortonBits), rebuildSortBytes<uint32_t>(std::max(I, 1u), 8),
                                     rebuildSortBytes<uint32_t>((uint32_t)N, 8)});
  if (B.capPrims >= P && B.sortTmpBytes >= sortBytes) return;
  auto alloc = [&](auto*& p, size_t count) { HIP_CHECK(hipMalloc(&p, std::max<size_t>(count, 1) * sizeof(*p))); S.keep(p); };
  alloc(B.d_primBoxes, P); alloc(B.d_parts, kRebuildParts); alloc(B.d_sceneBox, 1);
  for (int k = 0; k < 2; ++k) { alloc(B.d_keys[k], P); alloc(B.d_vals[k], P); alloc(B.d_depth[k], I); alloc(B.d_ids[k], I); }
  alloc(B.d_child, I); alloc(B.d_range, I); alloc(B.d_parent, N); alloc(B.d_swapped, I); alloc(B.d_index, N);
  alloc(B.d_levelStart, kRebuildMaxDepth + 2);
  alloc(B.d_height, N); alloc(B.d_hvals[0], N); alloc(B.d_hvals[1], N); alloc(B.d_heightStart, kRebuildHeightSlots);
  B.sortTmpBytes = sortBytes;
  HIP_CHECK(hipMalloc(&B.d_sortTmp, std::max<size_t>(B.sortTmpBytes, 16)));
  S.keep(B.d_sortTmp);
  B.capPrims = P;
}
std::vector<void*> rebuildScratchBuffers(const mi_scene::Rebuild& B) {
  return {B.d_primBoxes, B.d_parts, B.d_sceneBox, B.d_keys[0], B.d_keys[1], B.d_vals[0], B.d_vals[1], B.d_depth[0], B.d_depth[1],
          B.d_ids[0], B.d_ids[1], B.d_child, B.d_range, B.d_parent, B.d_swapped, B.d_index, B.d_levelStart, B.d_height, B.d_hvals[0],
          B.d_hvals[1], B.d_heightStart, B.d_sortTmp};
}

void rebuildTables(mi_scene& S) {
  mi_scene::Rebuild& B = S.rebuild;
  if (B.ready) return;
  const mi_scene::Refit& R = S.refit;
  mi_scene_geometry d{};
  d.geometry = R.geometry.data(); d.num_geometry = (uint32_t)R.geometry.size(); d.mesh_info = R.meshInfo.data(); d.num_meshes = (uint32_t)R.meshInfo.size();
  std::vector<uint32_t> primStart(d.num_geometry + 1);
  const size_t P = canon_prim_starts(d, primStart.data()), N = R.nodes.size();
  std::vector<RebuildPrim> canon(P);
  for (uint32_t p = 0; p < (uint32_t)P; ++p)
    (void)canon_prim(p, primStart.data(), d.num_geometry, d.geometry, d.mesh_info, R.matIds.data(), R.tris.data(), canon[p]);
  if (N != (P ? 2 * P - 1 : 0)) throw ArgError("mi_scene_rebuild: the scene's BVH does not hold every primitive exactly once (one leaf per primitive is what a rebuild keeps)");
  B.numPrims = (uint32_t)P;
  if (P) {
// ... 4 lines not shown
}

uint32_t rebuildPasses(mi_scene& S, mi_scene::Refit& R, mi_scene::Rebuild& B, DeviceScene& ds, hipStream_t stream, const char* fn, bool inPlace) {
  const uint32_t N = ds.numNodes;
  const uint32_t P = B.numPrims, I = P - 1;
  RefitGeom g;
  g.verts = R.d_verts; g.spheres = R.d_spheres; g.discs = R.d_discs;
  g.normals = ds.hasNormals ? ds.meshNormals : nullptr;
  const int scratch = R.live == 0 ? 1 : 0;
  const bool timing = S.opt.rebuildTiming;
  if (timing && !B.ev[0]) for (hipEvent_t& e : B.ev) HIP_CHECK(hipEventCreate(&e));
  auto mark = [&](int k) { if (timing) HIP_CHECK(hipEventRecord(B.ev[k], stream)); };
  auto blocks = [](uint32_t n) { return dim3((n + 255) / 256); };
  RebuildTree t;
  t.numPrims = P; t.child = B.d_child; t.range = B.d_range; t.parent = B.d_parent; t.swapped = B.d_swapped; t.boxes = R.d_boxes; t.index = B.d_index;
  t.height = B.d_height;

  if (inPlace) HIP_CHECK(hipMemsetAsync(R.d_err, 0, sizeof(uint32_t), stream));
  mark(0);
  const uint32_t parts = std::min((P + 255) / 256, kRebuildParts);
  hipLaunchKernelGGL(rebuild_prim_kernel, dim3(parts), dim3(256), 0, stream, P, B.d_canon, g, B.d_primBoxes, B.d_parts, R.d_err);
  hipLaunchKernelGGL(rebuild_scene_kernel, dim3(1), dim3(kRebuildParts), 0, stream, B.d_parts, parts, B.d_sceneBox);
  hipLaunchKernelGGL(rebuild_key_kernel, blocks(P), dim3(256), 0, stream, P, B.d_primBoxes, B.d_sceneBox, B.d_keys[0], B.d_vals[0]);
  HIP_CHECK(hipGetLastError());
  mark(1);
  uint64_t* keys = nullptr; uint32_t* sorted = nullptr;
  rebuildSort<uint64_t>(B, B.d_keys, B.d_vals, P, 3 * kMortonBits, stream, keys, sorted);
  t.sorted = sorted;
  mark(2);
  hipLaunchKernelGGL(rebuild_hierarchy_kernel, blocks(P), dim3(256), 0, stream, keys, B.d_primBoxes, t);
  uint32_t levelStart[kRebuildMaxDepth + 2] = {0};
  uint32_t* order = nullptr;
  if (I) {
    hipLaunchKernelGGL(rebuild_depth_kernel, blocks(I), dim3(256), 0, stream, I, B.d_parent, B.d_depth[0], B.d_ids[0]);
    HIP_CHECK(hipGetLastError());
    uint32_t* depth = nullptr;
    rebuildSort<uint32_t>(B, B.d_depth, B.d_ids, I, 8, stream, depth, order);
    HIP_CHECK(hipMemsetAsync(B.d_levelStart, 0, sizeof levelStart, stream));
    hipLaunchKernelGGL(rebuild_levels_kernel, blocks(I), dim3(256), 0, stream, I, depth, B.d_levelStart);
    HIP_CHECK(hipGetLastError());
    HIP_CHECK(hipMemcpyAsync(levelStart, B.d_levelStart, sizeof levelStart, hipMemcpyDeviceToHost, stream));
    HIP_CHECK(hipStreamSynchronize(stream));
  }
  mark(3);
  const uint32_t D = levelStart[kRebuildMaxDepth + 1];
  if (I) {
    if (D >= kRebuildMaxDepth) throw DeviceError(std::string(fn) + ": interior depth out of range");
    uint32_t top = 0;
    while (top < D && levelStart[top + 2] - levelStart[top + 1] <= kRefitTopThreads) ++top;
    for (uint32_t d = D; d > top; --d) {
      const uint32_t cnt = levelStart[d + 1] - levelStart[d];
      hipLaunchKernelGGL(rebuild_level_kernel, blocks(cnt), dim3(256), 0, stream, order, levelStart[d], cnt, t, R.d_err);
    }
    hipLaunchKernelGGL(rebuild_top_kernel, dim3(1), dim3(kRefitTopThreads), 0, stream, order, B.d_levelStart, top, t, R.d_err);
    HIP_CHECK(hipGetLastError());
  }
  mark(4);
  hipLaunchKernelGGL(rebuild_preorder_kernel, blocks(N), dim3(256), 0, stream, t);
  HIP_CHECK(hipGetLastError());
  mark(5);
  uint32_t* hkeys[2] = {(uint32_t*)B.d_keys[0], (uint32_t*)B.d_keys[1]};
  hipLaunchKernelGGL(rebuild_heightkey_kernel, blocks(N), dim3(256), 0, stream, t, hkeys[0], B.d_hvals[0]);
  HIP_CHECK(hipGetLastError());
  uint32_t* heights = nullptr; uint32_t* byHeight = nullptr;
  rebuildSort<uint32_t>(B, hkeys, B.d_hvals, N, 8, stream, heights, byHeight);
  uint32_t heightStart[kRebuildHeightSlots] = {0};
  HIP_CHECK(hipMemsetAsync(B.d_heightStart, 0, sizeof heightStart, stream));
  hipLaunchKernelGGL(rebuild_heights_kernel, blocks(N), dim3(256), 0, stream, N, heights, B.d_heightStart);
  HIP_CHECK(hipGetLastError());
  uint32_t err = 0;
  RefitBox rootBox{};
  HIP_CHECK(hipMemcpyAsync(&err, R.d_err, sizeof err, hipMemcpyDeviceToHost, stream));
  HIP_CHECK(hipMemcpyAsync(&rootBox, R.d_boxes, sizeof rootBox, hipMemcpyDeviceToHost, stream));
  HIP_CHECK(hipMemcpyAsync(heightStart, B.d_heightStart, sizeof heightStart, hipMemcpyDeviceToHost, stream));
  HIP_CHECK(hipStreamSynchronize(stream));
  if (err & (1u << kTriIndexOutOfRange)) throw ArgError(std::string(fn) + ": triangle vertex index out of range; the scene is unchanged");
  if (err & (1u << kBoxNotFinite)) throw ArgError(std::string(fn) + ": a node box is not finite; the scene is unchanged");
  if (err) throw ArgError(std::string(fn) + ": a node extent is above 65504 (Cannot compress BVH bounds into fp16 (half)); the scene is unchanged");
  const uint32_t H = heightStart[kRebuildHeightSlots - 1];
  if (H > kRebuildMaxDepth || heightStart[H + 1] != N) throw DeviceError(std::string(fn) + ": node heights out of range");
  refitLevelRoom(S, R, H + 2);
  if (inPlace) for (LaunchSlot& l : S.slots) if (l.stream != stream) HIP_CHECK(hipStreamWaitEvent(stream, l.lastWork, 0));
  hipLaunchKernelGGL(rebuild_scatter_kernel, blocks(N), dim3(256), 0, stream, t, B.d_canon, g, R.d_cnodes[scratch], const_cast<GNode*>(ds.nodes),
                     const_cast<GLeaf*>(ds.leaves), const_cast<GLeafRot*>(ds.leavesRot), const_cast<float*>(ds.leafNormals), R.d_prims);
  HIP_CHECK(hipGetLastError());
  HIP_CHECK(hipMemcpyAsync(R.d_cnodes[1 - scratch], R.d_cnodes[scratch], (size_t)N * sizeof(mi_bvh_node), hipMemcpyDeviceToDevice, stream));
  HIP_CHECK(hipMemcpyAsync(R.d_order, byHeight, (size_t)N * sizeof(uint32_t), hipMemcpyDeviceToDevice, stream));
  HIP_CHECK(hipMemcpyAsync(R.d_levelStart, B.d_heightStart, (H + 2) * sizeof(uint32_t), hipMemcpyDeviceToDevice, stream));
  mark(6);
  HIP_CHECK(hipStreamSynchronize(stream));
  if (timing)
    for (int k = 0; k < 6; ++k) { float w = 0.f; HIP_CHECK(hipEventElapsedTime(&w, B.ev[k], B.ev[k + 1])); B.ms[k] = w; }
  R.live = scratch;
  R.levelStart.assign(heightStart, heightStart + H + 2);
  refitTopFirst(R);
  R.tables = true;
  ds.rootInterior = 0;
  if (N > 1) {
    Box3 rb; rb.lo = mk(rootBox.lx, rootBox.ly, rootBox.lz); rb.hi = mk(rootBox.hx, rootBox.hy, rootBox.hz);
    mi_bvh_node root{};
    box_encode(rb, root.min_x, root.min_y, root.min_z, root.dx, root.dy, root.dz);
    ds.rootLoX = root.min_x; ds.rootHiX = root.min_x + half_bits_to_float(root.dx);
    ds.rootLoY = root.min_y; ds.rootHiY = root.min_y + half_bits_to_float(root.dy);
    ds.rootLoZ = root.min_z; ds.rootHiZ = root.min_z + half_bits_to_float(root.dz);
    ds.rootInterior = 1u;
  }
  return I ? D + 2 : 1u;
}

void rebuildBaseline(mi_scene& S, hipStream_t stream) {
  S.live.baselineValid = false;
  if (S.opt.autoRebuild > 0.0 && S.ds.numNodes) {
    double c[3];
    sceneCost(S, stream, c);
    S.live.baseline = bvh_cost_estimate(c); S.live.baselineValid = true;
  }
}

uint32_t rebuildScene(mi_scene& S, hipStream_t stream) {
  if (!S.ds.numNodes) return 0;
  refitAlloc(S);
  rebuildTables(S);
  S.live.maxLeafDepth = rebuildPasses(S, S.refit, S.rebuild, S.touchArrays(), stream, "mi_scene_rebuild", true);
  rebuildBaseline(S, stream);
  S.freeRetiredHot();
  return S.live.maxLeafDepth;
}

uint32_t setGeometry(mi_scene& S, const mi_scene_geometry& g, hipStream_t stream, hipMemcpyKind kind, const char* fn) {
  canon_check_control(g, kLeafFlag >> 5, [&](bool ok, const char* what) { if (!ok) throw ArgError(std::string(fn) + ": " + what); });
  const uint32_t G = g.num_geometry, M = g.num_meshes;
  std::vector<uint32_t> primStart(G + 1);
  const uint32_t P = canon_prim_starts(g, primStart.data());
  const uint32_t N = P ? 2 * P - 1 : 0;
  const uint32_t numVerts = M ? g.num_verts : 0, numTris = M ? g.num_tris : 0;
  if (!S.refit.d_err) { HIP_CHECK(hipMalloc(&S.refit.d_err, sizeof(uint32_t))); S.keep(S.refit.d_err); }
  if (S.opt.rebuildTiming && !S.rebuild.ev[0]) for (hipEvent_t& e : S.rebuild.ev) HIP_CHECK(hipEventCreate(&e));

  const size_t mark = S.allocations.size();
  std::vector<void*> staged;
  DeviceScene ds = S.ds;
  mi_scene::Refit R;
  mi_scene::Rebuild B = S.rebuild;
  uint32_t depth = 0;
  try {
    auto alloc = [&](auto*& p, size_t count) { p = nullptr; if (count) { HIP_CHECK(hipMalloc(&p, count * sizeof(*p))); S.keep(p); } };
    auto put = [&](void* dst, const void* src, size_t bytes, hipMemcpyKind k) { if (bytes) HIP_CHECK(hipMemcpyAsync(dst, src, bytes, k, stream)); };
    auto stage = [&](auto*& p, const void* src, size_t count) {
      p = nullptr;
      if (!count) return;
      HIP_CHECK(hipMalloc(&p, count * sizeof(*p)));
      staged.push_back(p);
      put(p, src, count * sizeof(*p), hipMemcpyHostToDevice);
    };
    uint32_t* matIDs; mi_material* materials; uint16_t* tris; mi_vec3* normals; uint32_t* firstVertex;
    alloc(matIDs, g.num_mat_ids); put(matIDs, g.mat_ids, (size_t)g.num_mat_ids * sizeof(uint32_t), hipMemcpyHostToDevice);
    alloc(materials, g.num_materials); put(materials, g.materials, (size_t)g.num_materials * sizeof(mi_material), hipMemcpyHostToDevice);
    alloc(R.d_verts, numVerts); put(R.d_verts, g.mesh_verts, (size_t)numVerts * sizeof(mi_vec3), kind);
    alloc(R.d_spheres, g.num_spheres); put(R.d_spheres, g.spheres, (size_t)g.num_spheres * sizeof(mi_sphere), kind);
    alloc(R.d_discs, g.num_discs); put(R.d_discs, g.discs, (size_t)g.num_discs * sizeof(mi_disc), kind);
    alloc(tris, 3 * (size_t)numTris); put(tris, g.mesh_tris, 3 * (size_t)numTris * sizeof(uint16_t), kind);
    alloc(normals, g.num_normals); put(normals, g.mesh_normals, (size_t)g.num_normals * sizeof(mi_vec3), kind);
    alloc(firstVertex, G);
    R.numVerts = numVerts; R.numNormals = g.num_normals; R.numSpheres = g.num_spheres; R.numDiscs = g.num_discs;
    R.d_err = S.refit.d_err;
    for (int k = 0; k < 4; ++k) R.ev[k] = S.refit.ev[k];
    for (int k = 0; k < 3; ++k) R.ms[k] = S.refit.ms[k];
    R.ready = true;
    GNode* nodes; GLeaf* leaves; GLeafRot* rot; float* leafNormals;
    alloc(nodes, N); alloc(leaves, N); alloc(rot, N); alloc(leafNormals, g.num_normals ? 9 * (size_t)N : 0);
    alloc(R.d_prims, N); alloc(R.d_order, N); alloc(R.d_boxes, N); alloc(R.d_cnodes[0], N); alloc(R.d_cnodes[1], N);
    ds.nodes = nodes; ds.numNodes = N; ds.leaves = leaves; ds.numLeaves = N; ds.leavesRot = rot;
    ds.matIDs = matIDs; ds.materials = materials; ds.numMaterials = g.num_materials;
    ds.hasNormals = g.num_normals ? 1u : 0u; ds.leafNormals = leafNormals;
    ds.meshTris = tris; ds.meshNormals = normals; ds.geomFirstVertex = firstVertex;
    ds.rootInterior = 0;
    ds.rootLoX = ds.rootHiX = ds.rootLoY = ds.rootHiY = ds.rootLoZ = ds.rootHiZ = 0.f;
    B.numPrims = P; B.ready = true;
    alloc(B.d_canon, P);
    if (P) {
      rebuildScratch(S, B, P);
      uint32_t* d_primStart; mi_geom_ref* d_geometry; mi_mesh_info* d_meshInfo;
      stage(d_primStart, primStart.data(), (size_t)G + 1); stage(d_geometry, g.geometry, G); stage(d_meshInfo, g.mesh_info, M);
      HIP_CHECK(hipMemsetAsync(R.d_err, 0, sizeof(uint32_t), stream));
      hipLaunchKernelGGL(canon_prim_kernel, dim3((P + 255) / 256), dim3(256), 0, stream, P, d_primStart, G, d_geometry, d_meshInfo, matIDs, tris, B.d_canon, R.d_err);
      hipLaunchKernelGGL(canon_first_vertex_kernel, dim3((G + 255) / 256), dim3(256), 0, stream, G, d_geometry, d_meshInfo, firstVertex);
      HIP_CHECK(hipGetLastError());
      depth = rebuildPasses(S, R, B, ds, stream, fn, false);
    } else {
      if (G) {
        mi_geom_ref* d_geometry; mi_mesh_info* d_meshInfo;
        stage(d_geometry, g.geometry, G); stage(d_meshInfo, g.mesh_info, M);
        hipLaunchKernelGGL(canon_first_vertex_kernel, dim3((G + 255) / 256), dim3(256), 0, stream, G, d_geometry, d_meshInfo, firstVertex);
        HIP_CHECK(hipGetLastError());
      }
      HIP_CHECK(hipStreamSynchronize(stream));
      R.levelStart.assign(2, 0u);
      refitTopFirst(R);
      R.tables = true; R.live = 0;
    }
    for (LaunchSlot& l : S.slots) HIP_CHECK(hipEventSynchronize(l.lastWork));
  } catch (...) {
    (void)hipStreamSynchronize(stream);
    for (void* p : staged) (void)hipFree(p);
    for (size_t k = mark; k < S.allocations.size(); ++k) (void)hipFree(S.allocations[k]);
    S.allocations.resize(mark);
    throw;
  }
  for (void* p : staged) (void)hipFree(p);
  const DeviceScene& o = S.ds;
  const mi_scene::Refit& oR = S.refit;
  std::vector<const void*> old = {o.nodes, o.leaves, o.leavesRot, o.matIDs, o.materials, o.leafNormals, o.meshTris, o.meshNormals, o.geomFirstVertex,
                                  oR.d_prims, oR.d_order, oR.d_boxes, oR.d_cnodes[0], oR.d_cnodes[1], oR.d_levelStart, oR.d_verts, oR.d_spheres, oR.d_discs,
                                  S.rebuild.d_canon, S.live.d_cost,
                                  S.hot.nodes, S.hot.leaves, S.hot.rot, S.hot.leafNormals,
                                  S.thin.nodes, S.thin.leaves, S.thin.rot, S.thin.leafNormals};
  if (B.d_primBoxes != S.rebuild.d_primBoxes) for (void* p : rebuildScratchBuffers(S.rebuild)) old.push_back(p);
  for (const void* p : old) S.release(p);
  S.hot = mi_scene::HotCopy{};
  S.thin = mi_scene::HotCopy{};
  S.touchArrays() = ds;
  S.refit = std::move(R);
  S.rebuild = B;
  S.live.d_cost = nullptr;
  S.live.maxLeafDepth = depth;
  ++S.live.geometrySets;
  rebuildBaseline(S, stream);
  return depth;
}

constexpr uint32_t kMaxSlotWorkgroups = 4096;

void ensureScratch(mi_scene& S, size_t n) {
  {
    const uint32_t asked = S.opt.nifSamplesPerLaunch;
    const uint32_t segLen = segment_samples(S.ds.samplesPerPixel);
    uint32_t v = (asked >= 1 && asked <= kNifSplMax) ? asked : kNifSplDefault;
    v = ((v + segLen - 1) / segLen) * segLen;
    v = std::min(v, std::max(segLen, ((S.ds.samplesPerPixel + segLen - 1) / segLen) * segLen));
    const bool haveTwo = S.nifSlots[1].u != nullptr;
    auto setsFor = [&](uint32_t vv) { return (S.nifOverlapOn() && S.ds.samplesPerPixel > vv) ? 2u : 1u; };
    constexpr uint64_t kSlotBytes = 48;
    uint64_t budget = (uint64_t)64 << 30;
    {
      size_t freeB = 0, totalB = 0;
      if (hipMemGetInfo(&freeB, &totalB) == hipSuccess) {
        const uint64_t held = (uint64_t)S.scratchRays * S.scratchSamples * kSlotBytes * (haveTwo ? 2u : 1u);
        budget = std::min<uint64_t>(budget, ((uint64_t)freeB + held) / 2);
      } else (void)hipGetLastError();
    }
    if (!(asked >= 1 && asked <= kNifSplMax))
      while (v > segLen && (uint64_t)n * v * kSlotBytes * setsFor(v) > budget) v -= segLen;
    const bool oneSetOnly = setsFor(v) == 2u && (uint64_t)n * v * kSlotBytes * 2u > budget;
    if (S.scratchRays >= n && S.scratchAsked == asked && S.scratchSamples >= segLen && S.scratchSamples % segLen == 0 &&
        (haveTwo || oneSetOnly || !(S.nifOverlapOn() && S.ds.samplesPerPixel > S.scratchSamples))) return;
    S.scratchAsked = asked;
    S.scratchOneSet = oneSetOnly;
    if (v != S.scratchSamples || (!haveTwo && !oneSetOnly && S.nifOverlapOn() && S.ds.samplesPerPixel > v)) { S.scratchSamples = v; S.scratchRays = 0; }
  }
  if (S.scratchRays >= n) return;
  if (S.nifPending) { HIP_CHECK(hipDeviceSynchronize()); S.nifPending = false; }
  if (S.d_rng) (void)hipFree(S.d_rng);
  if (S.d_segTotal) (void)hipFree(S.d_segTotal);
  S.freeNifSlots();
  S.d_rng = nullptr; S.d_segTotal = nullptr; S.scratchRays = 0;
  const size_t slots = n * S.scratchSamples;
  HIP_CHECK(hipMalloc(&S.d_rng, n * sizeof(Rng)));
  HIP_CHECK(hipMalloc(&S.d_segTotal, 3 * n * sizeof(float)));
  const int sets = (S.nifOverlapOn() && S.ds.samplesPerPixel > S.scratchSamples && !S.scratchOneSet) ? 2 : 1;
  for (int k = 0; k < sets; ++k) {
    mi_scene::NifSlots& q = S.nifSlots[k];
    HIP_CHECK(hipMalloc(&q.u, slots * sizeof(float)));
    HIP_CHECK(hipMalloc(&q.v, slots * sizeof(float)));
    HIP_CHECK(hipMalloc(&q.bgr, 3 * slots * sizeof(float)));
    HIP_CHECK(hipMalloc(&q.color, 3 * slots * sizeof(float)));
    HIP_CHECK(hipMalloc(&q.tp, 3 * slots * sizeof(float)));
    HIP_CHECK(hipMalloc(&q.index, (slots + (size_t)kMaxSlotWorkgroups * 4u * kEnvChunk) * sizeof(uint32_t)));
    if (!q.count) HIP_CHECK(hipMalloc(&q.count, sizeof(uint32_t)));
    if (!q.traced) HIP_CHECK(hipEventCreateWithFlags(&q.traced, hipEventDisableTiming));
    if (!q.done) HIP_CHECK(hipEventCreateWithFlags(&q.done, hipEventDisableTiming));
  }
  S.scratchRays = n;
}

[[maybe_unused]] constexpr uint32_t kLdsBudgetBytes = 160 * 1024 - 2048 - 23 * 1024 * 4;

constexpr uint64_t kMaxWorkItems = 0xFFFFFFFFull - ((uint64_t)1 << 22);

template <bool STATS>
void launchWavefront(mi_scene& S, mi_trace_result* d_rays, uint32_t cnt, hipStream_t stream, const WaveExtras& ex = WaveExtras{}, uint32_t wgCap = 0, uint32_t unitsHere = 0) {
  LaunchSlot& slot = S.slotFor(stream);
  const uint32_t units = unitsHere ? unitsHere : S.cus();
  uint32_t* workCounter = slot.d_workCounter;
  const DeviceScene dsv = S.view();
  const uint32_t w = (uint32_t)S.params.window_w;
// ... 664 lines not shown
```

ipu_ray_lib_amd/csrc/rebuild_kernels.hpp:

```cpp
#pragma once

#include <hip/hip_runtime.h>

#include "ray_math.h"
#include "trace_kernels.hpp"
#include "refit_kernels.hpp"
#include "canon_prims.hpp"
#include "../../include/mi_raylib.h"

namespace mi {

static_assert(REFIT_TRI == 0 && REFIT_SPHERE == 1 && REFIT_DISC == 2, "a RebuildPrim's kind is its geometry's type");

struct RebuildTree {
  uint32_t numPrims;
  const uint32_t* sorted;
  uint2* child;
  uint2* range;
  uint32_t* parent;
  uint8_t* swapped;
  RefitBox* boxes;
  uint32_t* index;
  uint32_t* height;
};
// ... 62 lines not shown
  t.child[j] = make_uint2(l, r);
  t.range[j] = make_uint2(first, last);
  t.parent[l] = j; t.parent[r] = j;
}

__global__ void __launch_bounds__(256) rebuild_depth_kernel(uint32_t I, const uint32_t* parent, uint32_t* depth, uint32_t* iota) {
  const uint32_t i = blockIdx.x * blockDim.x + threadIdx.x;
  if (i >= I) return;
  uint32_t d = 0;
  for (uint32_t c = i; c != 0; c = parent[c]) ++d;
  depth[i] = d;
  iota[i] = i;
}
__global__ void __launch_bounds__(256) rebuild_levels_kernel(uint32_t I, const uint32_t* depth, uint32_t* levelStart) {
  const uint32_t k = blockIdx.x * blockDim.x + threadIdx.x;
  if (k >= I) return;
  const uint32_t d = depth[k];
  if (d >= kRebuildMaxDepth) { if (k == I - 1) levelStart[kRebuildMaxDepth + 1] = d; return; }
  if (k == 0 || depth[k - 1] != d) levelStart[d] = k;
  if (k == I - 1) { levelStart[d + 1] = I; levelStart[kRebuildMaxDepth + 1] = d; }
}

__device__ __forceinline__ void rebuild_interior(uint32_t i, const RebuildTree& t, uint32_t* err) {
  const uint2 c = t.child[i];
  const Box3 l = refit_load_box(t.boxes, c.x), r = refit_load_box(t.boxes, c.y);
  const bool sw = box_centre_dist2(r) < box_centre_dist2(l);
  const Box3 u = sw ? box_union(r, l) : box_union(l, r);
  t.swapped[i] = sw ? 1 : 0;
  const uint32_t hl = t.height[c.x], hr = t.height[c.y];
  t.height[i] = 1u + (hl > hr ? hl : hr);
  rebuild_store_box(t.boxes, i, u);
  rebuild_check_box(u, err);
}
__global__ void __launch_bounds__(256) rebuild_level_kernel(const uint32_t* order, uint32_t begin, uint32_t count, RebuildTree t, uint32_t* err) {
  const uint32_t k = blockIdx.x * blockDim.x + threadIdx.x;
  if (k >= count) return;
  rebuild_interior(order[begin + k], t, err);
}
__global__ void __launch_bounds__(kRefitTopThreads) rebuild_top_kernel(const uint32_t* order, const uint32_t* levelStart, uint32_t first, RebuildTree t, uint32_t* err) {
  for (uint32_t d = first + 1; d-- > 0;) {
    const uint32_t b = levelStart[d], e = levelStart[d + 1];
    for (uint32_t k = b + threadIdx.x; k < e; k += blockDim.x) rebuild_interior(order[k], t, err);
    __syncthreads();
  }
}

__device__ __forceinline__ uint32_t rebuild_size(const RebuildTree& t, uint32_t n) {
  if (n >= t.numPrims - 1) return 1u;
  const uint2 r = t.range[n];
  return 2u * (r.y - r.x + 1u) - 1u;
}

__global__ void __launch_bounds__(256) rebuild_preorder_kernel(RebuildTree t) {
  const uint32_t n = blockIdx.x * blockDim.x + threadIdx.x;
  if (n >= 2 * t.numPrims - 1) return;
  uint32_t at = 0;
  for (uint32_t c = n; c != 0;) {
    const uint32_t a = t.parent[c];
    const uint2 ch = t.child[a];
    const uint32_t firstChild = t.swapped[a] ? ch.y : ch.x;
    at += c == firstChild ? 1u : 1u + rebuild_size(t, firstChild);
    c = a;
  }
  t.index[n] = at;
}

__global__ void __launch_bounds__(256) rebuild_heightkey_kernel(RebuildTree t, uint32_t* keys, uint32_t* vals) {
  const uint32_t n = blockIdx.x * blockDim.x + threadIdx.x;
  if (n >= 2 * t.numPrims - 1) return;
  const uint32_t i = t.index[n];
  keys[i] = t.height[n];
  vals[i] = i;
}
__global__ void __launch_bounds__(256) rebuild_heights_kernel(uint32_t N, const uint32_t* height, uint32_t* heightStart) {
  const uint32_t k = blockIdx.x * blockDim.x + threadIdx.x;
  if (k >= N) return;
  const uint32_t h = height[k];
  if (h > kRebuildMaxDepth) { if (k == N - 1) heightStart[kRebuildHeightSlots - 1] = h; return; }
  if (k == 0 || height[k - 1] != h) heightStart[h] = k;
  if (k == N - 1) { heightStart[h + 1] = N; heightStart[kRebuildHeightSlots - 1] = h; }
}

__global__ void __launch_bounds__(256) rebuild_scatter_kernel(RebuildTree t, const RebuildPrim* canon, RefitGeom g, mi_bvh_node* cnodes,
                                                              GNode* nodes, GLeaf* leaves, GLeafRot* rot, float* leafNormals, RefitPrim* prims) {
  const uint32_t n = blockIdx.x * blockDim.x + threadIdx.x;
  const uint32_t P = t.numPrims, I = P - 1;
  if (n >= 2 * P - 1) return;
  const uint32_t i = t.index[n];
  const uint32_t end = i + rebuild_size(t, n);
  mi_bvh_node c;
  box_encode(refit_load_box(t.boxes, n), c.min_x, c.min_y, c.min_z, c.dx, c.dy, c.dz);
  GNode nd;
  nd.minx = c.min_x; nd.maxx = c.min_x + half_bits_to_float(c.dx);
  nd.miny = c.min_y; nd.maxy = c.min_y + half_bits_to_float(c.dy);
  nd.minz = c.min_z; nd.maxz = c.min_z + half_bits_to_float(c.dz);
  nd.link = end << 5;
  GLeaf L;
  GLeafRot R;
  __builtin_memset(&L, 0, sizeof L);
  __builtin_memset(&R, 0, sizeof R);
  float vn[9] = {0.f, 0.f, 0.f, 0.f, 0.f, 0.f, 0.f, 0.f, 0.f};
  RefitPrim rp;
  if (n < I) {
    const uint2 ch = t.child[n];
    c.geom_id = MI_INVALID_GEOM;
    c.prim_or_second_child = i + 1u + rebuild_size(t, t.swapped[n] ? ch.y : ch.x);
    nd.hit = (i + 1u) << 5;
    rp.a = c.prim_or_second_child; rp.b = 0u; rp.c = 0u; rp.kind = REFIT_INTERIOR;
  } else {
    const RebuildPrim p = canon[t.sorted[n - I]];
    rp.a = p.a; rp.b = p.b; rp.c = p.c; rp.kind = p.kind;
    c.geom_id = (uint16_t)p.geomID;
    c.prim_or_second_child = p.primID;
    nd.hit = (end << 5) | kLeafFlag;
    L.primID = p.primID; L.matIndex = p.matIndex;
    if (p.kind == REFIT_TRI) {
      const f3 p0 = refit_vertex(g.verts, p.a), p1 = refit_vertex(g.verts, p.b), p2 = refit_vertex(g.verts, p.c);
      L.f[0] = p0.x; L.f[1] = p0.y; L.f[2] = p0.z; L.f[3] = p1.x; L.f[4] = p1.y; L.f[5] = p1.z; L.f[6] = p2.x; L.f[7] = p2.y; L.f[8] = p2.z;
      L.type = LEAF_TRI | (p.geomID << 16); L.triBase = p.triBase;
      const f3 fn = normalized(cross(p1 - p0, p2 - p0));
      L.n[0] = fn.x; L.n[1] = fn.y; L.n[2] = fn.z;
      if (g.normals) {
        const uint32_t v[3] = {p.a, p.b, p.c};
        for (int k = 0; k < 3; ++k) { const mi_vec3 q = g.normals[v[k]]; vn[3 * k] = q.x; vn[3 * k + 1] = q.y; vn[3 * k + 2] = q.z; }
      }
    } else if (p.kind == REFIT_SPHERE) {
      const mi_sphere s = g.spheres[p.a];
      L.f[0] = s.x; L.f[1] = s.y; L.f[2] = s.z; L.f[3] = s.radius; L.f[4] = s.radius * s.radius;
      L.type = LEAF_SPHERE | (p.geomID << 16);
    } else {
      const mi_disc d = g.discs[p.a];
      L.f[0] = d.nx; L.f[1] = d.ny; L.f[2] = d.nz; L.f[3] = d.cx; L.f[4] = d.cy; L.f[5] = d.cz; L.f[6] = d.r * d.r;
      L.type = LEAF_DISC | (p.geomID << 16);
    }
    for (uint32_t kz = 0; kz < 3; ++kz) {
      GLeafBlock& B = R.b[kz];
      B.type = L.type;
      for (int q = 0; q < 9; ++q) B.f[q] = L.f[q];
      if (p.kind == REFIT_TRI) {
        const uint32_t kx = (kz + 1) % 3, ky = (kz + 2) % 3;
        for (int v = 0; v < 3; ++v) { B.f[3 * v] = L.f[3 * v + kx]; B.f[3 * v + 1] = L.f[3 * v + ky]; B.f[3 * v + 2] = L.f[3 * v + kz]; }
      }
    }
  }
  cnodes[i] = c;
  prims[i] = rp;
  nodes[i] = nd;
  leaves[i] = L;
  rot[i] = R;
  if (leafNormals) for (int k = 0; k < 9; ++k) leafNormals[9 * (size_t)i + k] = vn[k];
}

}
```

ipu_ray_lib_amd/csrc/refit_kernels.hpp:

```cpp
#pragma once

#include <hip/hip_runtime.h>

#include "ray_math.h"
#include "trace_kernels.hpp"
#include "../../include/mi_raylib.h"

namespace mi {

enum : uint32_t { REFIT_TRI = 0, REFIT_SPHERE = 1, REFIT_DISC = 2, REFIT_INTERIOR = 3 };
struct __attribute__((aligned(16))) RefitPrim { uint32_t a, b, c, kind; };
static_assert(sizeof(RefitPrim) == 16, "RefitPrim: 16 B");

struct RefitGeom {
  const mi_vec3* verts;
  const mi_sphere* spheres;
  const mi_disc* discs;
  const mi_vec3* normals;
};

struct __attribute__((aligned(8))) RefitBox { float lx, ly, lz, hx, hy, hz; };
static_assert(sizeof(RefitBox) == 24, "RefitBox: 24 B");

__device__ __forceinline__ f3 refit_vertex(const mi_vec3* v, uint32_t i) { const mi_vec3 p = v[i]; return mk(p.x, p.y, p.z); }

__device__ __forceinline__ Box3 refit_prim_box(const RefitPrim& p, const RefitGeom& g) {
  if (p.kind == REFIT_TRI) return triangle_box(refit_vertex(g.verts, p.a), refit_vertex(g.verts, p.b), refit_vertex(g.verts, p.c));
  if (p.kind == REFIT_SPHERE) { const mi_sphere s = g.spheres[p.a]; return ball_box(s.x, s.y, s.z, s.radius); }
  const mi_disc c = g.discs[p.a];
  return ball_box(c.cx, c.cy, c.cz, c.r);
}

__device__ __forceinline__ Box3 refit_load_box(const RefitBox* boxes, uint32_t i) {
  const RefitBox r = boxes[i];
  Box3 b; b.lo = mk(r.lx, r.ly, r.lz); b.hi = mk(r.hx, r.hy, r.hz);
  return b;
}

__device__ __forceinline__ void refit_store(uint32_t i, const Box3& b, RefitBox* boxes, mi_bvh_node* cnodes, uint32_t* err) {
  RefitBox r; r.lx = b.lo.x; r.ly = b.lo.y; r.lz = b.lo.z; r.hx = b.hi.x; r.hy = b.hi.y; r.hz = b.hi.z;
  boxes[i] = r;
  mi_bvh_node c = cnodes[i];
  const uint32_t code = box_encode(b, c.min_x, c.min_y, c.min_z, c.dx, c.dy, c.dz);
  cnodes[i] = c;
  if (code != kBoxOk) atomicOr(err, 1u << code);
}

__global__ void __launch_bounds__(256) refit_leaf_kernel(const uint32_t* order, uint32_t count, const RefitPrim* prims, RefitGeom g,
                                                         RefitBox* boxes, mi_bvh_node* cnodes, uint32_t* err) {
  const uint32_t k = blockIdx.x * blockDim.x + threadIdx.x;
  if (k >= count) return;
  const uint32_t i = order[k];
  refit_store(i, refit_prim_box(prims[i], g), boxes, cnodes, err);
}

__device__ __forceinline__ void refit_interior(uint32_t i, const RefitPrim* prims, RefitBox* boxes, mi_bvh_node* cnodes, uint32_t* err) {
  refit_store(i, box_union(refit_load_box(boxes, i + 1), refit_load_box(boxes, prims[i].a)), boxes, cnodes, err);
}

__global__ void __launch_bounds__(256) refit_level_kernel(const uint32_t* order, uint32_t begin, uint32_t count, const RefitPrim* prims,
                                                          RefitBox* boxes, mi_bvh_node* cnodes, uint32_t* err) {
  const uint32_t k = blockIdx.x * blockDim.x + threadIdx.x;
  if (k >= count) return;
  refit_interior(order[begin + k], prims, boxes, cnodes, err);
}

constexpr uint32_t kRefitTopThreads = 1024;
__global__ void __launch_bounds__(kRefitTopThreads) refit_top_kernel(const uint32_t* order, const uint32_t* levelStart, uint32_t first, uint32_t last,
                                                                     const RefitPrim* prims, RefitBox* boxes, mi_bvh_node* cnodes, uint32_t* err) {
  for (uint32_t h = first; h <= last; ++h) {
    const uint32_t b = levelStart[h], e = levelStart[h + 1];
    for (uint32_t k = b + threadIdx.x; k < e; k += blockDim.x) refit_interior(order[k], prims, boxes, cnodes, err);
    __syncthreads();
  }
}

__global__ void __launch_bounds__(256) refit_write_kernel(uint32_t n, const RefitPrim* prims, const mi_bvh_node* cnodes, RefitGeom g,
                                                          GNode* nodes, GLeaf* leaves, GLeafRot* rot, float* leafNormals) {
  const uint32_t i = blockIdx.x * blockDim.x + threadIdx.x;
  if (i >= n) return;
  const mi_bvh_node c = cnodes[i];
  GNode nd = nodes[i];
  nd.minx = c.min_x; nd.maxx = c.min_x + half_bits_to_float(c.dx);
  nd.miny = c.min_y; nd.maxy = c.min_y + half_bits_to_float(c.dy);
  nd.minz = c.min_z; nd.maxz = c.min_z + half_bits_to_float(c.dz);
  nodes[i] = nd;
  const RefitPrim p = prims[i];
  if (p.kind == REFIT_INTERIOR) return;
  GLeaf L = leaves[i];
  if (p.kind == REFIT_TRI) {
    const f3 p0 = refit_vertex(g.verts, p.a), p1 = refit_vertex(g.verts, p.b), p2 = refit_vertex(g.verts, p.c);
    L.f[0] = p0.x; L.f[1] = p0.y; L.f[2] = p0.z; L.f[3] = p1.x; L.f[4] = p1.y; L.f[5] = p1.z; L.f[6] = p2.x; L.f[7] = p2.y; L.f[8] = p2.z;
    const f3 fn = normalized(cross(p1 - p0, p2 - p0));
    L.n[0] = fn.x; L.n[1] = fn.y; L.n[2] = fn.z;
    if (g.normals && leafNormals) {
      const uint32_t v[3] = {p.a, p.b, p.c};
      for (int k = 0; k < 3; ++k) {
        const mi_vec3 q = g.normals[v[k]];
        leafNormals[9 * (size_t)i + 3 * k] = q.x; leafNormals[9 * (size_t)i + 3 * k + 1] = q.y; leafNormals[9 * (size_t)i + 3 * k + 2] = q.z;
      }
    }
  } else if (p.kind == REFIT_SPHERE) {
    const mi_sphere s = g.spheres[p.a];
    L.f[0] = s.x; L.f[1] = s.y; L.f[2] = s.z; L.f[3] = s.radius; L.f[4] = s.radius * s.radius;
  } else {
    const mi_disc d = g.discs[p.a];
    L.f[0] = d.nx; L.f[1] = d.ny; L.f[2] = d.nz; L.f[3] = d.cx; L.f[4] = d.cy; L.f[5] = d.cz; L.f[6] = d.r * d.r;
  }
  leaves[i] = L;
  for (uint32_t kz = 0; kz < 3; ++kz) {
    GLeafBlock B;
    B.type = L.type;
    for (int q = 0; q < 9; ++q) B.f[q] = L.f[q];
    if (p.kind == REFIT_TRI) {
      const uint32_t kx = (kz + 1) % 3, ky = (kz + 2) % 3;
      for (int v = 0; v < 3; ++v) { B.f[3 * v] = L.f[3 * v + kx]; B.f[3 * v + 1] = L.f[3 * v + ky]; B.f[3 * v + 2] = L.f[3 * v + kz]; }
    }
    rot[i].b[kz] = B;
  }
}

}
```

ipu_ray_lib_amd/csrc/trace_kernels.hpp:

```cpp
#pragma once

#include <hip/hip_runtime.h>

#include "ray_math.h"
#include "../../include/mi_raylib.h"

namespace mi {

struct __attribute__((aligned(16))) GNode {
  float minx, maxx, miny, maxy, minz, maxz;
  uint32_t link;
  uint32_t hit;
};
constexpr uint32_t kLeafFlag = 0x80000000u;
__host__ __device__ __forceinline__ bool node_is_leaf(const GNode& nd) { return (nd.hit & kLeafFlag) != 0u; }
static_assert(sizeof(GNode) == 32, "GNode must stay 32 bytes");

enum : uint32_t { LEAF_TRI = 0, LEAF_SPHERE = 1, LEAF_DISC = 2 };

struct __attribute__((aligned(16))) GLeaf {
  uint32_t type;
  float f[9];
  uint32_t primID;
  uint32_t triBase;
  float n[3];
  uint32_t matIndex;
};
static_assert(sizeof(GLeaf) == 64, "GLeaf must stay 64 bytes");
__host__ __device__ __forceinline__ uint32_t leaf_kind(const GLeaf& L) { return L.type & 0xFFFFu; }
__host__ __device__ __forceinline__ uint32_t leaf_geom(const GLeaf& L) { return L.type >> 16; }

struct __attribute__((aligned(8))) GLeafBlock { uint32_t type; float f[9]; };
struct __attribute__((aligned(128))) GLeafRot { GLeafBlock b[3]; uint32_t pad[2]; };
static_assert(sizeof(GLeafBlock) == 40 && sizeof(GLeafRot) == 128, "GLeafRot: three 40-byte blocks in a 128-byte line");
__device__ __forceinline__ uint32_t leaf_kind(const GLeafBlock& B) { return B.type & 0xFFFFu; }

struct DeviceScene {
  const GNode* nodes;        uint32_t numNodes;
  const GLeaf* leaves;       uint32_t numLeaves;
  const GLeafRot* leavesRot;
  const uint32_t* matIDs;
  const mi_material* materials; uint32_t numMaterials;
  const uint16_t* meshTris; const mi_vec3* meshNormals; const uint32_t* geomFirstVertex; uint32_t hasNormals;
  const float* leafNormals;
  float imageWidth, imageHeight, tanTheta, antiAliasScale;
  uint32_t maxPathLength, rouletteStartDepth, samplesPerPixel;
  uint64_t rngSeed;
  unsigned long long* counters;
  float rootLoX, rootLoY, rootLoZ, rootHiX, rootHiY, rootHiZ;
  uint32_t rootInterior;
  uint32_t exactBase;
};

__device__ __forceinline__ uint32_t root_start(const DeviceScene& sc, f3 o, uint32_t& visited) {
  const bool inside = (o.x > sc.rootLoX) & (o.x < sc.rootHiX) & (o.y > sc.rootLoY) & (o.y < sc.rootHiY) & (o.z > sc.rootLoZ) & (o.z < sc.rootHiZ) & (sc.rootInterior != 0u);
  visited = inside ? 1u : 0u;
  return inside ? 1u : 0u;
}

struct Shear { uint32_t kz; float sx, sy, sz; };

__device__ __forceinline__ Shear make_shear(f3 d) {
  Shear s;
  s.kz = min_index(d);
  uint32_t kx = s.kz + 1; if (kx == 3) kx = 0;
  uint32_t ky = kx + 1; if (ky == 3) ky = 0;
  const float dx = comp(d, kx), dy = comp(d, ky), dz = comp(d, s.kz);
  s.sx = -dx / dz;
  s.sy = -dy / dz;
  s.sz = 1.f / dz;
  return s;
}
__device__ __forceinline__ Shear make_shear(f3 d, f3 inv) {
  Shear s;
  s.kz = min_index(d);
  uint32_t kx = s.kz + 1; if (kx == 3) kx = 0;
  uint32_t ky = kx + 1; if (ky == 3) ky = 0;
  const float dx = comp(d, kx), dy = comp(d, ky), dz = comp(d, s.kz);
  s.sx = -dx / dz;
  s.sy = -dy / dz;
  s.sz = comp(inv, s.kz);
  return s;
}

__device__ __forceinline__ f3 fast_inverse(f3 d) { return mk(__builtin_amdgcn_rcpf(d.x), __builtin_amdgcn_rcpf(d.y), __builtin_amdgcn_rcpf(d.z)); }
__device__ __forceinline__ Shear make_shear_fast(f3 d, f3 inv) {
  Shear s;
  s.kz = min_index(d);
  uint32_t kx = s.kz + 1; if (kx == 3) kx = 0;
  uint32_t ky = kx + 1; if (ky == 3) ky = 0;
  s.sz = comp(inv, s.kz);
  s.sx = -comp(d, kx) * s.sz;
  s.sy = -comp(d, ky) * s.sz;
  return s;
}

__device__ __forceinline__ void fast_box_setup(f3 o, f3& inv, f3& oi, float& slabPad) {
  const float big = 1e18f;
  const bool px = !(fabsf(inv.x) < big), py = !(fabsf(inv.y) < big), pz = !(fabsf(inv.z) < big);
  inv = mk(px ? copysignf(big, inv.x) : inv.x, py ? copysignf(big, inv.y) : inv.y, pz ? copysignf(big, inv.z) : inv.z);
  oi = mk(-(o.x * inv.x), -(o.y * inv.y), -(o.z * inv.z));
  slabPad = 4.8e-7f * fmaxf(fmaxf(px ? 0.f : fabsf(oi.x), py ? 0.f : fabsf(oi.y)), pz ? 0.f : fabsf(oi.z));
}

__device__ __forceinline__ f3 permute_kz(f3 p, uint32_t kz) {
  const bool r1 = kz == 0;
  const bool r2 = kz == 1;
  return mk(r1 ? p.y : (r2 ? p.z : p.x), r1 ? p.z : (r2 ? p.x : p.y), r1 ? p.x : (r2 ? p.y : p.z));
}

template <bool DF = false, bool PRE = false>
__device__ __forceinline__ float intersect_triangle(f3 p0, f3 p1, f3 p2, f3 o, const Shear& sh, float& b0, float& b1, float& b2) {
  f3 p0t = PRE ? p0 - o : permute_kz(p0 - o, sh.kz), p1t = PRE ? p1 - o : permute_kz(p1 - o, sh.kz), p2t = PRE ? p2 - o : permute_kz(p2 - o, sh.kz);
  p0t.x += sh.sx * p0t.z; p0t.y += sh.sy * p0t.z;
  p1t.x += sh.sx * p1t.z; p1t.y += sh.sy * p1t.z;
  p2t.x += sh.sx * p2t.z; p2t.y += sh.sy * p2t.z;
  float e0 = p1t.x * p2t.y - p1t.y * p2t.x;
  float e1 = p2t.x * p0t.y - p2t.y * p0t.x;
  float e2 = p0t.x * p1t.y - p0t.y * p1t.x;
  if constexpr (DF) {
    if (e0 == 0.0f || e1 == 0.0f || e2 == 0.0f) {
      const double p2txp1ty = (double)p2t.x * (double)p1t.y;
      const double p2typ1tx = (double)p2t.y * (double)p1t.x;
      e0 = (float)(p2typ1tx - p2txp1ty);
      const double p0txp2ty = (double)p0t.x * (double)p2t.y;
      const double p0typ2tx = (double)p0t.y * (double)p2t.x;
      e1 = (float)(p0typ2tx - p0txp2ty);
// ... 133 lines not shown
__device__ __forceinline__ bool box_hit_exact(const GNode& nd, f3 o, f3 inv, float tMin, float tCur, bool literal) {
  return box_hit(box_hit_span<false>(box_hit_products(nd, o, inv), tMin, tCur, 0.f, literal));
}
__device__ __forceinline__ bool box_hit_fast(const GNode& nd, f3 inv, f3 oi, float slabPad, float tMin, float tCur) {
  return box_hit(box_hit_span<true>(box_hit_products_fast(nd, inv, oi), tMin, tCur, slabPad, false));
}

__device__ __forceinline__ bool needs_literal_box(f3 o, f3 inv) {
  return !(fabsf(inv.x) < kInf && fabsf(inv.y) < kInf && fabsf(inv.z) < kInf && fabsf(o.x) < kInf && fabsf(o.y) < kInf && fabsf(o.z) < kInf);
}

__device__ __forceinline__ f3 ray_dir(f3 d) { return d; }
template <class F> __device__ __forceinline__ f3 ray_dir(const F& load) { return load(); }

template <bool DF = false, bool FAST = false, bool ROT = false, class Rec, class Dir>
__device__ __forceinline__ bool prim_hit(const Rec& L, f3 o, const Dir& d, const Shear& sh, float tMin, float tCur, float& t, float& b0, float& b1, float& b2) {
  static_assert(!(FAST && ROT), "the FAST triangle test has no pre-rotated form");
  b0 = b1 = b2 = 0.f;
  bool cand;
  if (leaf_kind(L) == LEAF_TRI) {
    const f3 p0 = mk(L.f[0], L.f[1], L.f[2]), p1 = mk(L.f[3], L.f[4], L.f[5]), p2 = mk(L.f[6], L.f[7], L.f[8]);
    if constexpr (ROT) t = intersect_triangle<DF, true>(p0, p1, p2, permute_kz(o, sh.kz), sh, b0, b1, b2);
    else if constexpr (FAST) t = intersect_triangle_fast(p0, p1, p2, o, sh, b0, b1, b2);
    else t = intersect_triangle<DF>(p0, p1, p2, o, sh, b0, b1, b2);
    cand = t > 0.f && t < kInf;
  } else {
    const f3 dir = ray_dir(d);
    if (leaf_kind(L) == LEAF_SPHERE) t = intersect_sphere(L, o, dir, tMin);
    else t = intersect_disc(L, o, dir);
    cand = true;
  }
  return cand & (t > tMin) & (t < tCur);
}

struct Hit {
  float t;
  uint32_t leaf;
  uint32_t geomID;
  float b0, b1, b2;
};

struct CastStats { uint32_t nodes, leaves; };

template <bool ANY_HIT, bool STATS, bool DF = false, bool FAST = false>
__device__ __forceinline__ bool traverse(const DeviceScene& sc, f3 o, f3 d, float tMin, float tMax, Hit& hit, CastStats& cs) {
  f3 inv = FAST ? fast_inverse(d) : mk(1.f / d.x, 1.f / d.y, 1.f / d.z), oi = mk(0.f, 0.f, 0.f);
  const Shear sh = FAST ? make_shear_fast(d, inv) : make_shear(d);
  float slabPad = 0.f;
  if constexpr (FAST) fast_box_setup(o, inv, oi, slabPad);
  hit.t = tMax; hit.leaf = 0xFFFFFFFFu; hit.geomID = 0xFFFFu; hit.b0 = hit.b1 = hit.b2 = 0.f;
  const uint32_t numNodes = sc.numNodes;
  uint32_t i = 0;
  while (i < numNodes) {
    const GNode nd = sc.nodes[i];
    if (STATS) cs.nodes++;
    bool boxHit;
    if constexpr (FAST) boxHit = box_hit_fast(nd, inv, oi, slabPad, tMin, hit.t);
    else {
      float t0 = tMin, t1 = hit.t;
      box_hit_literal_axis((nd.minx - o.x) * inv.x, (nd.maxx - o.x) * inv.x, t0, t1);
      box_hit_literal_axis((nd.miny - o.y) * inv.y, (nd.maxy - o.y) * inv.y, t0, t1);
      box_hit_literal_axis((nd.minz - o.z) * inv.z, (nd.maxz - o.z) * inv.z, t0, t1);
      boxHit = !(t0 > t1);
    }
    const bool isLeaf = node_is_leaf(nd);
    if (boxHit && isLeaf) {
      if (STATS) cs.leaves++;
      const GLeaf L = sc.leaves[i];
      float t, b0, b1, b2;
      if (prim_hit<DF, FAST>(L, o, d, sh, tMin, hit.t, t, b0, b1, b2)) {
        if (ANY_HIT) return true;
        hit.t = t; hit.leaf = i; hit.geomID = leaf_geom(L); hit.b0 = b0; hit.b1 = b1; hit.b2 = b2;
      }
    }
    i = (boxHit && !isLeaf) ? i + 1 : (nd.link >> 5);
  }
  return hit.leaf != 0xFFFFFFFFu;
}

__device__ __forceinline__ f3 hit_normal(const DeviceScene& sc, const Hit& h, f3 hp) {
  const GLeaf L = sc.leaves[h.leaf];
  if (leaf_kind(L) == LEAF_TRI) {
    if (!sc.hasNormals) return mk(L.n[0], L.n[1], L.n[2]);
    const float* q = sc.leafNormals + 9 * (size_t)h.leaf;
    return normalized((mk(q[0], q[1], q[2]) * h.b0) + (mk(q[3], q[4], q[5]) * h.b1) + (mk(q[6], q[7], q[8]) * h.b2));
  }
  if (leaf_kind(L) == LEAF_SPHERE) return normalized(hp - mk(L.f[0], L.f[1], L.f[2]));
  return mk(L.f[0], L.f[1], L.f[2]);
}

__device__ __forceinline__ void flush_stats(const DeviceScene& sc, uint32_t casts, const CastStats& cs, uint32_t paths) {
  unsigned long long c = casts, n = cs.nodes, l = cs.leaves, p = paths;
  for (int off = 32; off > 0; off >>= 1) {
    c += __shfl_down(c, off); n += __shfl_down(n, off); l += __shfl_down(l, off); p += __shfl_down(p, off);
  }
  if ((threadIdx.x & 63) == 0) {
    atomicAdd(&sc.counters[0], c);
    if (n) atomicAdd(&sc.counters[1], n);
    if (l) atomicAdd(&sc.counters[2], l);
    if (p) atomicAdd(&sc.counters[3], p);
  }
}

__constant__ uint32_t kSinBits[92] = {MI_SIN_TABLE_BITS};

__device__ __forceinline__ void load_sin_table(float* tbl) {
  for (uint32_t k = threadIdx.x; k < 92; k += blockDim.x) tbl[k] = __uint_as_float(kSinBits[k]);
  __syncthreads();
}

template <bool STATS, bool DF = false>
__global__ void __launch_bounds__(256) shadow_trace_kernel(DeviceScene sc, mi_trace_result* rays, uint32_t n, float ambient, f3 lightPos) {
  const uint32_t idx = blockIdx.x * blockDim.x + threadIdx.x;
  CastStats cs = {0, 0};
  uint32_t casts = 0;
  if (idx < n) {
    mi_trace_result* res = rays + idx;
    const mi_hit_record h = res->h;
    f3 o = mk(h.r.origin.x, h.r.origin.y, h.r.origin.z), d = mk(h.r.direction.x, h.r.direction.y, h.r.direction.z);
    Hit hit;
    ++casts;
    if (traverse<false, STATS, DF>(sc, o, d, h.r.t_min, h.r.t_max, hit, cs)) {
      const f3 hp = o + d * hit.t;
      const f3 nrm = hit_normal(sc, hit, hp);
      const mi_material mat = sc.materials[sc.matIDs[hit.geomID]];
      const f3 lightOffset = lightPos - hp;
      const f3 sd = normalized(lightOffset);
      const f3 so = offset_origin(hp, sd, nrm);
      const float sTmax = sqrtf(sqnorm(lightOffset));
      const f3 albedo = mk(mat.albedo.x, mat.albedo.y, mat.albedo.z);
      f3 color = albedo * ambient;
      Hit shadowHit;
      ++casts;
      if (!traverse<true, STATS, DF>(sc, so, sd, 0.f, sTmax, shadowHit, cs)) color = color + albedo * dot(sd, nrm);
      res->rgb = {color.x, color.y, color.z};
      res->h.r.origin = {hp.x, hp.y, hp.z};
      res->h.r.t_max = hit.t;
      res->h.prim_id = sc.leaves[hit.leaf].primID;
      res->h.normal = {nrm.x, nrm.y, nrm.z};
      res->h.geom_id = (uint16_t)hit.geomID;
    } else {
      res->h.flags = h.flags | MI_FLAG_ESCAPED;
    }
  }
  flush_stats(sc, casts, cs, idx < n ? 1u : 0u);
}

struct PathState {
  f3 o, d, n, tp;
  float tMax;
  uint32_t primID, geomID, flags;
};

template <bool STATS, bool DF = false>
__global__ void __launch_bounds__(256) path_trace_kernel(DeviceScene sc, mi_trace_result* rays, uint32_t n, uint32_t firstSample, uint32_t numSamples, Rng* rngStates) {
  __shared__ float sinTbl[92];
  load_sin_table(sinTbl);
  const uint32_t idx = blockIdx.x * blockDim.x + threadIdx.x;
  CastStats cs = {0, 0};
  uint32_t casts = 0, paths = 0;
  if (idx < n) {
    mi_trace_result* res = rays + idx;
    const float prow = res->u, pcol = res->v;
    Rng rng;
    const uint32_t segLenRender = segment_samples(sc.samplesPerPixel);
    if (rngStates && (firstSample % segLenRender) != 0) rng = rngStates[idx];
    else rng_seed_pixel_segment(rng, sc.rngSeed, prow, pcol, rngStates ? firstSample / segLenRender : 0u);
// ... 86 lines not shown
```

ipu_ray_lib_amd/csrc/trace_wavefront.hpp:

```cpp
#pragma once

#include "trace_kernels.hpp"

namespace mi {

enum : uint32_t { PH_NODE = 0, PH_LEAF = 1, PH_SHADE = 2, PH_GEN = 3, PH_FETCH = 4, PH_DONE = 5 };
constexpr uint32_t kGenNode = 0x7FFFFFFDu, kFetchNode = 0x7FFFFFFEu, kDoneNode = 0x7FFFFFFFu;
static_assert(kGenNode > ((kLeafFlag >> 5) - 1u) << 5 && kDoneNode < kLeafFlag && kFetchNode == kGenNode + (PH_FETCH - PH_GEN) && kDoneNode == kGenNode + (PH_DONE - PH_GEN), "the parked phases lie between the largest byte offset and the leaf flag");

struct WaveTune { uint32_t leafAt, shadeAt, genAt, burst, keep8, dbl = 4, maxExtra = 6, leafThenNode = 1, prio = 1, leafP = 40, probe = 0;
  bool operator==(const WaveTune& o) const { return leafAt == o.leafAt && shadeAt == o.shadeAt && genAt == o.genAt && burst == o.burst && keep8 == o.keep8 && dbl == o.dbl && maxExtra == o.maxExtra && leafThenNode == o.leafThenNode && prio == o.prio && leafP == o.leafP && probe == o.probe; } };

struct WaveExtras {
  uint32_t sampleCount = 0;
  float* u = nullptr; float* v = nullptr;
  float* slotColor = nullptr; float* slotTp = nullptr;
  uint32_t* index = nullptr; uint32_t* count = nullptr;
  float azimuthRotation = 0.f;
  uint32_t fetchChunk = 0;
  float* segPart = nullptr;
  uint32_t segments = 1;
  uint32_t segBase = 0;
  const float2* coords = nullptr;
  uint32_t firstInSetup = 0;
// ... 310 lines not shown
              }
              if (cand && t > 0.f && t < hit.t) {
                hit.t = t; hit.leaf = pend1; hit.b0 = b0; hit.b1 = b1; hit.b2 = b2;
                node = pend1Node;
                pend1 = 0xFFFFFFFFu;
                if (STATS) specNodes = 0;
                ph = (node >= numNodes) ? PH_SHADE : PH_NODE;
              } else {
                if (STATS) { cs.nodes += specNodes; specNodes = 0; }
                pend1 = 0xFFFFFFFFu;
                if (ph == PH_LEAF) {
                  if (pendLeaf != 0xFFFFFFFFu) {
                    pend1 = pendLeaf; pend1Node = node;
                    if (node >= numNodes) pendLeaf = 0xFFFFFFFFu; else ph = PH_NODE;
                  } else ph = PH_SHADE;
                }
              }
            }
          } else
          if (inLeaf()) {
            if (STATS) cs.leaves++;
            const uint32_t at = node & ~kLeafFlag;
            if (!HOT) node = at;
            const uint32_t atLeaf = HOT ? (at >> 5) : (at >> 5) - 1u;
            const uint32_t recNode = HOT ? at : at - 32u;
            GLeaf L;
            if constexpr (ROT) {
              const GLeafBlock B = *reinterpret_cast<const GLeafBlock*>(reinterpret_cast<const char*>(sc.leavesRot) + ((recNode << 2) + sh.kz * 40u));
              L.type = B.type;
#pragma unroll
              for (int q = 0; q < 9; ++q) L.f[q] = B.f[q];
            } else {
              L = *reinterpret_cast<const GLeaf*>(reinterpret_cast<const char*>(sc.leaves) + (recNode << 1));
            }
            float t, b0 = 0.f, b1 = 0.f, b2 = 0.f;
            bool cand;
            const uint32_t kind = (HOT && ROT) ? (L.type & 31u) : leaf_kind(L);
            if constexpr (HOT) node = ROT ? (L.type & ~31u) : L.triBase;
            if (STATS) { const unsigned long long qm = __ballot(kind != LEAF_TRI); itQ += qm ? 1u : 0u; lnQ += (uint32_t)__popcll(qm); }
            if (kind == LEAF_TRI) {
              if constexpr (ROT) t = intersect_triangle<DF, true>(mk(L.f[0], L.f[1], L.f[2]), mk(L.f[3], L.f[4], L.f[5]), mk(L.f[6], L.f[7], L.f[8]), permute_kz(o, sh.kz), sh, b0, b1, b2);
              else
              t = FAST ? intersect_triangle_fast(mk(L.f[0], L.f[1], L.f[2]), mk(L.f[3], L.f[4], L.f[5]), mk(L.f[6], L.f[7], L.f[8]), o, sh, b0, b1, b2)
                       : intersect_triangle<DF>(mk(L.f[0], L.f[1], L.f[2]), mk(L.f[3], L.f[4], L.f[5]), mk(L.f[6], L.f[7], L.f[8]), o, sh, b0, b1, b2);
              cand = t > 0.f && t < kInf;
            } else if (kind == LEAF_SPHERE) {
              t = intersect_sphere(L, o, d, 0.f);
              cand = true;
            } else {
              t = intersect_disc(L, o, d);
              cand = true;
            }
            const bool closer = cand & (t > 0.f) & (t < hit.t);
            hit.t = closer ? t : hit.t; hit.leaf = closer ? atLeaf : hit.leaf;
            if constexpr (BARY) { hit.b0 = closer ? b0 : hit.b0; hit.b1 = closer ? b1 : hit.b1; hit.b2 = closer ? b2 : hit.b2; }
          }
          if (tune.leafThenNode) {
            if (STATS) { itN++; lnN += (uint32_t)__popcll(__ballot(inNode())); }
            if constexpr (SPEC) nodeStep();
            else if (inNode()) {
              if (anyExact) (void)nodeBodyT(std::true_type{}, std::false_type{});
              else (void)nodeBody();
            }
            ++steps;
          }
        }
        cN = (uint32_t)__popcll(__ballot(inNode()));
        cL = (uint32_t)__popcll(__ballot(inLeaf()));
        if (++steps >= tune.burst || (cN + cL) * 8u < startT * tune.keep8 || (cN + cL) == 0) break;
      }
      if (tune.prio == 1) __builtin_amdgcn_s_setprio(0); else if (tune.prio == 2) __builtin_amdgcn_s_setprio(1);
      if (STATS) tTrav += __builtin_amdgcn_s_memtime() - tq0;
    } else if (MERGE) {
      if (STATS) { itS++; lnS += cS + cG; }
      const unsigned long long tq1 = STATS ? __builtin_amdgcn_s_memtime() : 0ull;
      bool envRay = false, pathEnd = false, genNow = false, setup = false;
      uint32_t envSlot = 0;
      const bool wasShade = inShade(), wasGen = inGen();
      if (wasShade || wasGen) pathLoad();
      if (wasShade) {
        bool terminated = false;
        if (hit.leaf != 0xFFFFFFFFu) {
          const GLeaf L = sc.leaves[hit.leaf];
          hit.geomID = leaf_geom(L);
          coldU(6) = hit.leaf; coldF(7) = hit.t;
          o = o + d * hit.t;
          nrm = hit_normal(sc, hit, o);
          mi_material mat;
          if (matsInLds) { mat = matS[L.matIndex].m; asm volatile("" ::: "memory"); } else mat = sc.materials[L.matIndex];
          const f3 albedo = mk(mat.albedo.x, mat.albedo.y, mat.albedo.z);
          if (mat.emissive) color = color + tp * mk(mat.emission.x, mat.emission.y, mat.emission.z);
          if (mat.type == 0) {
            const float u1 = rng_uniform01(rng);
            const float u2 = rng_uniform01(rng);
            d = sample_diffuse(nrm, u1, u2, sinTbl);
            tp = tp * albedo;
          } else if (mat.type == 1) {
            d = reflect_dir(d, nrm);
            tp = tp * albedo;
          } else if (mat.type == 2) {
            const float u1 = rng_uniform01(rng);
            f3 nd2;
            const bool refracted = dielectric(d, nrm, mat.ior, u1, nd2);
            d = nd2;
            if (refracted) tp = tp * albedo;
          } else {
            const float qn = __builtin_nanf("");
            coldF(3) = coldF(3) * qn; coldF(4) = coldF(4) * qn; coldF(5) = coldF(5) * qn;
            oFlags |= MI_FLAG_ERROR;
          }
        } else {
          coldF(7) = kInf;
          oFlags |= MI_FLAG_ESCAPED;
          terminated = true;
        }
        if (!terminated && bounce > sc.rouletteStartDepth) {
          const float u1 = rng_uniform01(rng);
          if (roulette_stop(u1, tp)) terminated = true;
        }
        bounce++;
        if (bounce >= sc.maxPathLength) terminated = true;
        if (terminated) {
          const uint32_t pixNow = getPix();
          mi_trace_result* res = rays + pixNow;
          if (slots) {
            const size_t q = (size_t)sample * n + pixNow;
            ex.slotColor[3 * q] = color.x; ex.slotColor[3 * q + 1] = color.y; ex.slotColor[3 * q + 2] = color.z;
            envRay = (oFlags & MI_FLAG_ESCAPED) != 0;
            envSlot = (uint32_t)q;
            if (!envRay) ex.u[q] = -1.f;
          } else { coldF(3) = coldF(3) + color.x; coldF(4) = coldF(4) + color.y; coldF(5) = coldF(5) + color.z; }
          pathEnd = true;
          ++sample;
          const bool more = segd ? ((sample & segMask) != 0u && sample < spp) : (sample < spp);
          if (more) genNow = true;
          else if (segd && sample < spp) {
            if (!slots && ex.segPart) {
              float* part = ex.segPart + 3 * ((size_t)(((sample - 1u) >> segShift) - ex.segBase) * n + pixNow);
              part[0] = coldF(3); part[1] = coldF(4); part[2] = coldF(5);
            }
            park(PH_FETCH);
          } else {
            if (!slots && ex.segPart) {
              float* part = ex.segPart + 3 * ((size_t)(((sample - 1u) >> segShift) - ex.segBase) * n + pixNow);
              part[0] = coldF(3); part[1] = coldF(4); part[2] = coldF(5);
            } else
            if (!slots) res->rgb = {coldF(3), coldF(4), coldF(5)};
            uint32_t oPrim = MI_INVALID_PRIM, oGeom = MI_INVALID_GEOM;
            const uint32_t lastLeaf = coldU(6);
            if (lastLeaf != 0xFFFFFFFFu) { const GLeaf LL = sc.leaves[lastLeaf]; oPrim = LL.primID; oGeom = leaf_geom(LL); }
            mi_hit_record hr;
            hr.r.origin = {o.x, o.y, o.z}; hr.r.t_min = 0.f;
            hr.r.direction = {d.x, d.y, d.z}; hr.r.t_max = coldF(7);
            hr.prim_id = oPrim;
            hr.normal = {nrm.x, nrm.y, nrm.z};
            hr.throughput = {tp.x, tp.y, tp.z};
            hr.geom_id = (uint16_t)oGeom; hr.flags = (uint16_t)oFlags;
            res->h = hr;
            park(PH_FETCH);
          }
        } else {
          o = offset_origin(o, d, nrm);
          setup = true;
        }
      }
      if (slots) pushEscaped(envRay, envSlot);
      if (genNow || wasGen) {
        if constexpr (kCoordsFromStream) {
          const uint32_t e = coldU(0);
          if (ex.coords) { const float2 pc = ex.coords[e]; prow = pc.x; pcol = pc.y; } else { prow = rays[e].u; pcol = rays[e].v; }
        } else { prow = coldF(1); pcol = coldF(2); }
        float g0, g1;
        rng_gauss2(rng, sinTbl, g0, g1);
        const float jr = prow + sc.antiAliasScale * g0, jc = pcol + sc.antiAliasScale * g1;
        d = pixel_to_ray_dir(jc, jr, sc.imageWidth, sc.imageHeight, sc.tanTheta);
        o = mk(0.f, 0.f, 0.f);
        nrm = mk(0.f, 0.f, 1.f);
// ... 228 lines not shown
```

Measured before the change: 21.08 billion.

## Precompute per-leaf diffuse tangent frames and read them in wavefront shading

Adds a 32-byte per-leaf tangent frame (xb, yb) built from the flat face normal or disc normal. The refit and rebuild kernels fill it when the scene has no vertex normals, reusing the leaf normal buffer. The wavefront shade step loads the frame instead of recomputing the basis with a sqrt and branches for diffuse bounces, falling back to computing it when the frame is zero. The concentric disc sampler and frame construction are also made branchless with selects. The cost is an extra 32-byte gather per hit and more memory, which may cost more than the few ALU ops it saves.

```diff
diff --git a/__graft_entry__.py b/__graft_entry__.py
--- a/__graft_entry__.py
+++ b/__graft_entry__.py
@@ -10,11 +10,11 @@
 PKG = ROOT / "ipu_ray_lib_amd"
 CSRC = PKG / "csrc"
 
-HOST_SRCS = [CSRC / "host" / n for n in ("bvh_sah.cpp", "lbvh.cpp", "glb_reader.cpp", "dae_reader.cpp", "scene_builtin.cpp", "scene_api.cpp", "nif_assets.cpp", "point_query_host.cpp", "box_query_host.cpp", "cross_host.cpp", "hot_order.cpp")]
-HOST_DEPS = HOST_SRCS + [CSRC / "ray_math.h", CSRC / "hot_order.hpp", CSRC / "point_math.hpp", CSRC / "box_math.hpp", CSRC / "cross_math.hpp", CSRC / "canon_prims.hpp", CSRC / "bvh_cost_host.hpp", CSRC / "scene_blob.hpp", CSRC / "ray_shard.hpp", CSRC / "host" / "scene_types.hpp", CSRC / "host" / "json_min.hpp",
+HOST_SRCS = [CSRC / "host" / n for n in ("bvh_sah.cpp", "lbvh.cpp", "glb_reader.cpp", "dae_reader.cpp", "scene_builtin.cpp", "scene_api.cpp", "nif_assets.cpp", "point_query_host.cpp", "box_query_host.cpp", "cross_host.cpp", "hot_order.cpp", "leaf_frame.cpp")]
+HOST_DEPS = HOST_SRCS + [CSRC / "ray_math.h", CSRC / "leaf_frame.hpp", CSRC / "hot_order.hpp", CSRC / "point_math.hpp", CSRC / "box_math.hpp", CSRC / "cross_math.hpp", CSRC / "canon_prims.hpp", CSRC / "bvh_cost_host.hpp", CSRC / "scene_blob.hpp", CSRC / "ray_shard.hpp", CSRC / "host" / "scene_types.hpp", CSRC / "host" / "json_min.hpp",
                          ROOT / "include" / "mi_raylib.h", ROOT / "include" / "mi_scene_host.h"]
 HIP_SRCS = [CSRC / "raylib.hip"]
-HIP_DEPS = HIP_SRCS + [CSRC / "ray_math.h", CSRC / "trace_kernels.hpp", CSRC / "trace_wavefront.hpp", CSRC / "hot_order.hpp", CSRC / "query_kernels.hpp", CSRC / "point_kernels.hpp", CSRC / "point_math.hpp", CSRC / "count_kernels.hpp", CSRC / "list_kernels.hpp", CSRC / "near_kernels.hpp", CSRC / "box_kernels.hpp", CSRC / "box_math.hpp", CSRC / "cross_math.hpp", CSRC / "refit_kernels.hpp", CSRC / "rebuild_kernels.hpp", CSRC / "canon_prims.hpp", CSRC / "canon_kernels.hpp", CSRC / "cost_kernels.hpp", CSRC / "bvh_cost_host.hpp", CSRC / "trace_pool.hpp", CSRC / "nif_kernels.hpp", CSRC / "nif_regs_pack.hpp", CSRC / "nif_regs_kernel.hpp", CSRC / "nif_asm_kernel.hpp", CSRC / "nif_asm_gen.py", CSRC / "scene_blob.hpp", CSRC / "ray_shard.hpp", CSRC / "group_render.hpp", CSRC / "query_drivers.hpp", ROOT / "include" / "mi_raylib.h"]
+HIP_DEPS = HIP_SRCS + [CSRC / "ray_math.h", CSRC / "leaf_frame.hpp", CSRC / "trace_kernels.hpp", CSRC / "trace_wavefront.hpp", CSRC / "hot_order.hpp", CSRC / "query_kernels.hpp", CSRC / "point_kernels.hpp", CSRC / "point_math.hpp", CSRC / "count_kernels.hpp", CSRC / "list_kernels.hpp", CSRC / "near_kernels.hpp", CSRC / "box_kernels.hpp", CSRC / "box_math.hpp", CSRC / "cross_math.hpp", CSRC / "refit_kernels.hpp", CSRC / "rebuild_kernels.hpp", CSRC / "canon_prims.hpp", CSRC / "canon_kernels.hpp", CSRC / "cost_kernels.hpp", CSRC / "bvh_cost_host.hpp", CSRC / "trace_pool.hpp", CSRC / "nif_kernels.hpp", CSRC / "nif_regs_pack.hpp", CSRC / "nif_regs_kernel.hpp", CSRC / "nif_asm_kernel.hpp", CSRC / "nif_asm_gen.py", CSRC / "scene_blob.hpp", CSRC / "ray_shard.hpp", CSRC / "group_render.hpp", CSRC / "query_drivers.hpp", ROOT / "include" / "mi_raylib.h"]
 
 EXACT_FLAGS = ["-ffp-contract=off", "-fno-fast-math"]
 
diff --git a/include/mi_scene_host.h b/include/mi_scene_host.h
--- a/include/mi_scene_host.h
+++ b/include/mi_scene_host.h
@@ -67,6 +67,9 @@
 uint32_t mi_hot_walk_count(const void* nodes, uint32_t num_nodes, const uint32_t* leaf_link, uint32_t start, const float origin[3], const float direction[3], float t_max,
                            uint32_t* visits, uint32_t capacity, uint32_t* box_tests, int* status);
 
+void mi_diffuse_frame(const float normal[3], float xb[3], float yb[3]);
+int mi_leaf_frames(const mi_scene_desc* desc, const uint32_t* at, uint32_t count, float* frames, float* normals);
+
 int mi_init_ray_stream(const mi_scene_desc* desc, mi_trace_result* rays, size_t capacity);
 
 void mi_scale_rgb(mi_trace_result* rays, size_t n, float scale);
diff --git a/ipu_ray_lib_amd/__init__.py b/ipu_ray_lib_amd/__init__.py
--- a/ipu_ray_lib_amd/__init__.py
+++ b/ipu_ray_lib_amd/__init__.py
@@ -184,6 +184,9 @@
         lib.mi_hot_walk_count.argtypes = [C.c_void_p, C.c_uint32, C.c_void_p, C.c_uint32, C.POINTER(C.c_float), C.POINTER(C.c_float), C.c_float, C.c_void_p, C.c_uint32,
                                           C.POINTER(C.c_uint32), C.POINTER(C.c_int)]
         lib.mi_hot_walk_count.restype = C.c_uint32
+        lib.mi_diffuse_frame.argtypes = [C.POINTER(C.c_float)] * 3
+        lib.mi_diffuse_frame.restype = None
+        lib.mi_leaf_frames.argtypes = [C.POINTER(SceneDesc), C.c_void_p, C.c_uint32, C.c_void_p, C.c_void_p]
         lib.mi_bvh_cost_compact.argtypes = [C.c_void_p, C.c_uint32, C.POINTER(C.c_double)]
         lib.mi_bvh_cost_compact_block.argtypes = [C.c_void_p, C.c_uint32, C.c_uint32, C.POINTER(C.c_double)]
         lib.mi_bvh_cost_estimate.argtypes = [C.POINTER(C.c_double)]
@@ -578,6 +581,22 @@
     return out
 
 
+def diffuse_frame(normal) -> np.ndarray:
+    n = (C.c_float * 3)(*[float(np.float32(x)) for x in normal])
+    xb, yb = (C.c_float * 3)(), (C.c_float * 3)()
+    host_lib().mi_diffuse_frame(n, xb, yb)
+    return np.array([list(xb), list(yb)], np.float32)
+
+
+def leaf_frames(desc: SceneDesc, place: np.ndarray | None = None):
+    n = int(desc.num_nodes)
+    at = None if place is None else np.ascontiguousarray(place, np.uint32)
+    count = n if at is None else at.size
+    frames, normals = np.zeros((count, 8), np.float32), np.zeros((n, 3), np.float32)
+    _check_host(host_lib().mi_leaf_frames(C.byref(desc), None if at is None or not count else at.ctypes.data, count, frames.ctypes.data if count else None, normals.ctypes.data if n else None))
+    return frames, normals
+
+
 def hot_cast_is_literal(origin, direction) -> bool:
     o, d = ((C.c_float * 3)(*[float(np.float32(x)) for x in v]) for v in (origin, direction))
     return bool(host_lib().mi_hot_cast_is_literal(o, d))
diff --git a/ipu_ray_lib_amd/csrc/host/diffuse_frame_check.cpp b/ipu_ray_lib_amd/csrc/host/diffuse_frame_check.cpp
--- /dev/null
+++ b/ipu_ray_lib_amd/csrc/host/diffuse_frame_check.cpp
@@ -0,0 +1,114 @@
+#include "../ray_math.h"
+
+#include <cmath>
+#include <cstdint>
+#include <cstdio>
+#include <cstring>
+#include <vector>
+
+namespace {
+
+using mi::f3;
+using mi::mk;
+
+uint32_t bits(float x) { uint32_t b; std::memcpy(&b, &x, 4); return b; }
+float from_bits(uint32_t b) { float x; std::memcpy(&x, &b, 4); return x; }
+
+void frame_branches(f3 n, f3& xb, f3& yb) {
+  const f3 a = mi::abs3(n), sq = n * n;
+  if (a.x > a.y) { const float il = 1.f / sqrtf(sq.x + sq.z); xb = mk(-n.z * il, 0.f, n.x * il); }
+  else { const float il = 1.f / sqrtf(sq.y + sq.z); xb = mk(0.f, n.z * il, -n.y * il); }
+  yb = mi::cross(n, xb);
+}
+
+bool disc_branches(float u1, float u2, float& r, float& th) {
+  const float ux = 2.f * u1 - 1.f, uy = 2.f * u2 - 1.f;
+  if (ux == 0.f && uy == 0.f) { r = ux; th = uy; return false; }
+  const float piby4 = (float)(3.14159265358979323846264338327950288 / 4.0);
+  const float piby2 = (float)(3.14159265358979323846264338327950288 / 2.0);
+  if (fabsf(ux) > fabsf(uy)) { r = ux; th = piby4 * (uy / ux); }
+  else { r = uy; th = piby2 - piby4 * (ux / uy); }
+  return true;
+}
+void disc_reference(float u1, float u2, const float* sinTbl, float& ox, float& oy) {
+  float r, th;
+  if (!disc_branches(u1, u2, r, th)) { ox = r; oy = th; return; }
+  float s, c;
+  mi::sincos_deg_table(th, sinTbl, s, c);
+  ox = r * c; oy = r * s;
+}
+
+uint64_t rngState = 0x9e3779b97f4a7c15ull;
+uint32_t rnd() { rngState ^= rngState << 13; rngState ^= rngState >> 7; rngState ^= rngState << 17; return (uint32_t)(rngState >> 16); }
+float rndUnit() { return (float)(rnd() >> 8) * (1.f / 16777216.f); }
+
+long failures = 0;
+
+bool same_bits(const uint32_t* w, const uint32_t* g, bool nanInput) {
+  for (int k = 0; k < 6; ++k) {
+    if (w[k] == g[k]) continue;
+    if (nanInput && std::isnan(from_bits(w[k])) && std::isnan(from_bits(g[k]))) continue;
+    return false;
+  }
+  return true;
+}
+
+void check_frame(f3 n) {
+  f3 xa, ya, xb, yb;
+  frame_branches(n, xa, ya);
+  mi::diffuse_frame(n, xb, yb);
+  const uint32_t w[6] = {bits(xa.x), bits(xa.y), bits(xa.z), bits(ya.x), bits(ya.y), bits(ya.z)};
+  const uint32_t g[6] = {bits(xb.x), bits(xb.y), bits(xb.z), bits(yb.x), bits(yb.y), bits(yb.z)};
+  if (!same_bits(w, g, std::isnan(n.x) || std::isnan(n.y) || std::isnan(n.z)) && failures++ < 10)
+    std::printf("diffuse_frame differs for n = %08x %08x %08x: want %08x %08x %08x | %08x %08x %08x, got %08x %08x %08x | %08x %08x %08x\n", bits(n.x), bits(n.y), bits(n.z),
+                w[0], w[1], w[2], w[3], w[4], w[5], g[0], g[1], g[2], g[3], g[4], g[5]);
+}
+
+void check_disc(float u1, float u2, const float* sinTbl) {
+  float wx, wy, gx, gy;
+  disc_reference(u1, u2, sinTbl, wx, wy);
+  mi::sample_disc_concentric(u1, u2, sinTbl, gx, gy);
+  if ((bits(wx) != bits(gx) || bits(wy) != bits(gy)) && failures++ < 10)
+    std::printf("sample_disc_concentric differs for u = %08x %08x: want %08x %08x, got %08x %08x\n", bits(u1), bits(u2), bits(wx), bits(wy), bits(gx), bits(gy));
+}
+
+}
+
+int main() {
+  const float inf = INFINITY, qnan = from_bits(0x7FC00000u), nnan = from_bits(0xFFC00001u), pnan = from_bits(0x7FA00123u);
+  const float special[] = {0.f, -0.f, from_bits(1u), -from_bits(1u), from_bits(0x007FFFFFu), -from_bits(0x007FFFFFu), from_bits(0x00800000u), 1e-30f, -1e-30f, 1e-19f, 0.5f, -0.5f,
+                           0.70710678f, -0.70710678f, 1.f, -1.f, from_bits(0x3F7FFFFFu), from_bits(0x3F800001u), 3.f, -3.f, 1e19f, -1e19f, 3e38f, -3e38f, inf, -inf, qnan, nnan, pnan};
+  long frames = 0;
+  for (float x : special) for (float y : special) for (float z : special) { check_frame(mk(x, y, z)); ++frames; }
+  for (int k = 0; k < 200000; ++k) {
+    const float v = (rnd() & 1u) ? rndUnit() : from_bits(rnd());
+    const float z = rndUnit() * 2.f - 1.f;
+    const float up = from_bits(bits(fabsf(v)) + 1u), dn = from_bits(bits(fabsf(v)) - 1u);
+    for (float y : {v, -v, up, -up, dn, -dn}) { check_frame(mk(v, y, z)); check_frame(mk(y, v, z)); frames += 2; }
+  }
+  for (int k = 0; k < 4000000; ++k) {
+    const f3 v = mk(rndUnit() * 2.f - 1.f, rndUnit() * 2.f - 1.f, rndUnit() * 2.f - 1.f);
+    check_frame(mi::normalized(v));
+    ++frames;
+  }
+  for (int k = 0; k < 1000000; ++k) { check_frame(mk(from_bits(rnd()), from_bits(rnd()), from_bits(rnd()))); ++frames; }
+
+  float sinTbl[92];
+  { static const uint32_t tblBits[92] = {MI_SIN_TABLE_BITS}; std::memcpy(sinTbl, tblBits, sizeof sinTbl); }
+  const float half = 0.5f;
+  std::vector<float> us = {0.f, half, 1.f, from_bits(bits(half) - 1u), from_bits(bits(half) + 1u), from_bits(bits(half) - 2u), from_bits(bits(half) + 2u), 0.25f, 0.75f,
+                           from_bits(1u), from_bits(0x00800000u), from_bits(0x3F7FFFFFu), 1e-10f, 0.1f, 0.9f};
+  long discs = 0;
+  for (float a : us) for (float b : us) { check_disc(a, b, sinTbl); ++discs; }
+  for (int k = 0; k < 2000000; ++k) {
+    const float a = rndUnit();
+    const float m = 1.f - a;
+    for (float b : {a, m, from_bits(bits(a) + 1u), from_bits(bits(m) + 1u), a > 0.f ? from_bits(bits(a) - 1u) : a, m > 0.f ? from_bits(bits(m) - 1u) : m, rndUnit(), half}) {
+      check_disc(a, b, sinTbl); check_disc(b, a, sinTbl);
+      discs += 2;
+    }
+  }
+  if (failures) { std::printf("diffuse_frame_check FAILED: %ld differences\n", failures); return 1; }
+  std::printf("diffuse_frame_check OK: %ld frames, %ld disc samples, all bits equal\n", frames, discs);
+  return 0;
+}
diff --git a/ipu_ray_lib_amd/csrc/host/leaf_frame.cpp b/ipu_ray_lib_amd/csrc/host/leaf_frame.cpp
--- /dev/null
+++ b/ipu_ray_lib_amd/csrc/host/leaf_frame.cpp
@@ -0,0 +1,53 @@
+#include "../leaf_frame.hpp"
+#include "../../../include/mi_scene_host.h"
+
+#include <cstring>
+#include <vector>
+
+extern "C" void mi_diffuse_frame(const float normal[3], float xb[3], float yb[3]) {
+  mi::f3 x, y;
+  mi::diffuse_frame(mi::mk(normal[0], normal[1], normal[2]), x, y);
+  xb[0] = x.x; xb[1] = x.y; xb[2] = x.z;
+  yb[0] = y.x; yb[1] = y.y; yb[2] = y.z;
+}
+
+extern "C" int mi_leaf_frames(const mi_scene_desc* d, const uint32_t* at, uint32_t count, float* frames, float* normals) {
+  if (!d || (count && !frames) || (d->num_nodes && !d->bvh_nodes)) return MI_ERR_INVALID_ARG;
+  const uint32_t N = d->num_nodes;
+  std::vector<uint8_t> framed(N, 0);
+  std::vector<float> normal(3 * (size_t)N, 0.f);
+  for (uint32_t i = 0; i < N; ++i) {
+    const mi_bvh_node& n = d->bvh_nodes[i];
+    if (n.geom_id == MI_INVALID_GEOM) continue;
+    if (n.geom_id >= d->num_geometry) return MI_ERR_INVALID_ARG;
+    const mi_geom_ref& r = d->geometry[n.geom_id];
+    if (r.type == 0) {
+      if (r.index >= d->num_meshes) return MI_ERR_INVALID_ARG;
+      const mi_mesh_info& m = d->mesh_info[r.index];
+      if (n.prim_or_second_child >= m.num_triangles) return MI_ERR_INVALID_ARG;
+      const size_t base = 3 * ((size_t)m.first_index + n.prim_or_second_child);
+      mi::f3 p[3];
+      for (int k = 0; k < 3; ++k) {
+        const size_t v = (size_t)m.first_vertex + d->mesh_tris[base + k];
+        if (v >= d->num_verts) return MI_ERR_INVALID_ARG;
+        p[k] = mi::mk(d->mesh_verts[v].x, d->mesh_verts[v].y, d->mesh_verts[v].z);
+      }
+      const mi::f3 fn = mi::normalized(mi::cross(p[1] - p[0], p[2] - p[0]));
+      normal[3 * (size_t)i] = fn.x; normal[3 * (size_t)i + 1] = fn.y; normal[3 * (size_t)i + 2] = fn.z;
+      framed[i] = 1;
+    } else if (r.type == 2) {
+      if (r.index >= d->num_discs) return MI_ERR_INVALID_ARG;
+      const mi_disc& c = d->discs[r.index];
+      normal[3 * (size_t)i] = c.nx; normal[3 * (size_t)i + 1] = c.ny; normal[3 * (size_t)i + 2] = c.nz;
+      framed[i] = 1;
+    }
+  }
+  for (uint32_t k = 0; k < count; ++k) if (at && at[k] >= N) return MI_ERR_INVALID_ARG;
+  if (!at && count > N) return MI_ERR_INVALID_ARG;
+  static_assert(sizeof(mi::GLeafFrame) == 8 * sizeof(float), "a record is eight floats");
+  std::vector<mi::GLeafFrame> out(count);
+  mi::fill_leaf_frames(framed.data(), normal.data(), at, count, out.data());
+  if (count) std::memcpy(frames, out.data(), (size_t)count * sizeof(mi::GLeafFrame));
+  if (normals && N) std::memcpy(normals, normal.data(), normal.size() * sizeof(float));
+  return MI_OK;
+}
diff --git a/ipu_ray_lib_amd/csrc/leaf_frame.hpp b/ipu_ray_lib_amd/csrc/leaf_frame.hpp
--- /dev/null
+++ b/ipu_ray_lib_amd/csrc/leaf_frame.hpp
@@ -0,0 +1,29 @@
+#pragma once
+
+#include "ray_math.h"
+
+#include <cstdint>
+
+namespace mi {
+
+struct __attribute__((aligned(16))) GLeafFrame { float xb[3]; float pad0; float yb[3]; float pad1; };
+static_assert(sizeof(GLeafFrame) == 32, "GLeafFrame must stay 32 bytes");
+
+MI_HD GLeafFrame leaf_frame_zero() { GLeafFrame r; r.xb[0] = r.xb[1] = r.xb[2] = r.pad0 = r.yb[0] = r.yb[1] = r.yb[2] = r.pad1 = 0.f; return r; }
+MI_HD GLeafFrame leaf_frame_of(f3 n) {
+  f3 xb, yb;
+  diffuse_frame(n, xb, yb);
+  GLeafFrame r;
+  r.xb[0] = xb.x; r.xb[1] = xb.y; r.xb[2] = xb.z; r.pad0 = 0.f;
+  r.yb[0] = yb.x; r.yb[1] = yb.y; r.yb[2] = yb.z; r.pad1 = 0.f;
+  return r;
+}
+
+inline void fill_leaf_frames(const uint8_t* framed, const float* normal, const uint32_t* at, uint32_t count, GLeafFrame* out) {
+  for (uint32_t k = 0; k < count; ++k) {
+    const uint32_t i = at ? at[k] : k;
+    out[k] = framed[i] ? leaf_frame_of(mk(normal[3 * (size_t)i], normal[3 * (size_t)i + 1], normal[3 * (size_t)i + 2])) : leaf_frame_zero();
+  }
+}
+
+}
diff --git a/ipu_ray_lib_amd/csrc/ray_math.h b/ipu_ray_lib_amd/csrc/ray_math.h
--- a/ipu_ray_lib_amd/csrc/ray_math.h
+++ b/ipu_ray_lib_amd/csrc/ray_math.h
@@ -323,9 +323,10 @@
   if (ux == 0.f && uy == 0.f) { ox = ux; oy = uy; return; }
   const float piby4 = (float)(3.14159265358979323846264338327950288 / 4.0);
   const float piby2 = (float)(3.14159265358979323846264338327950288 / 2.0);
-  float r, th;
-  if (fabsf(ux) > fabsf(uy)) { r = ux; th = piby4 * (uy / ux); }
-  else { r = uy; th = piby2 - piby4 * (ux / uy); }
+  const bool wide = fabsf(ux) > fabsf(uy);
+  const float r = wide ? ux : uy;
+  const float q = piby4 * ((wide ? uy : ux) / (wide ? ux : uy));
+  const float th = wide ? q : piby2 - q;
   float s, c;
   sincos_deg_table(th, sinTbl, s, c);
   ox = r * c; oy = r * s;
@@ -336,14 +337,23 @@
   const float z = sqrtf(fmaxf(0.f, 1.f - x * x - y * y));
   return mk(x, y, z);
 }
-MI_HD f3 sample_diffuse(f3 n, float u1, float u2, const float* sinTbl) {
-  f3 xb;
+MI_HD void diffuse_frame(f3 n, f3& xb, f3& yb) {
   const f3 a = abs3(n), sq = n * n;
-  if (a.x > a.y) { const float il = 1.f / sqrtf(sq.x + sq.z); xb = mk(-n.z * il, 0.f, n.x * il); }
-  else { const float il = 1.f / sqrtf(sq.y + sq.z); xb = mk(0.f, n.z * il, -n.y * il); }
-  const f3 yb = cross(n, xb);
+  const bool wide = a.x > a.y;
+  const float il = 1.f / sqrtf((wide ? sq.x : sq.y) + sq.z);
+  const float m = (wide ? -n.z : n.z) * il;
+  const float z = (wide ? n.x : -n.y) * il;
+  xb = mk(wide ? m : 0.f, wide ? 0.f : m, z);
+  yb = cross(n, xb);
+}
+MI_HD f3 diffuse_in_frame(f3 n, f3 xb, f3 yb, float u1, float u2, const float* sinTbl) {
   const f3 wi = cosine_sample_hemisphere(u1, u2, sinTbl);
   return mk(dot(mk(xb.x, yb.x, n.x), wi), dot(mk(xb.y, yb.y, n.y), wi), dot(mk(xb.z, yb.z, n.z), wi));
+}
+MI_HD f3 sample_diffuse(f3 n, float u1, float u2, const float* sinTbl) {
+  f3 xb, yb;
+  diffuse_frame(n, xb, yb);
+  return diffuse_in_frame(n, xb, yb, u1, u2, sinTbl);
 }
 MI_HD f3 reflect_dir(f3 d, f3 n) {
   const float cosTheta = dot(d, n);
diff --git a/ipu_ray_lib_amd/csrc/raylib.hip b/ipu_ray_lib_amd/csrc/raylib.hip
--- a/ipu_ray_lib_amd/csrc/raylib.hip
+++ b/ipu_ray_lib_amd/csrc/raylib.hip
@@ -125,6 +125,7 @@
   uint32_t nifShape = 7;
   bool leafRot = true;
   bool leanHit = true;
+  bool leafFrame = true;
   bool coords = true;
   int nifOverlap = -1;
   uint32_t nifTraceWgs = 0;
@@ -235,6 +236,7 @@
     if (key == "lean_hit") return flag01(v, leanHit);
     if (key == "auto_rebuild") { if (!autoRebuildValue(v, autoRebuild)) { why = "auto_rebuild takes 0 (off) or a decimal ratio above 1"; return false; } return true; }
     if (key == "leaf_rot") return flag01(v, leafRot);
+    if (key == "leaf_frame") return flag01(v, leafFrame);
     if (key == "hot_nodes") { if (!strcmp(v, "auto")) { hotNodes = kHotNodesAuto; return true; } if (!number(v, 0, 65535, q)) return false; hotNodes = (int)q; return true; }
     if (key == "double_fallback") {
       bool b = doubleFallback;
@@ -280,7 +282,7 @@
                                          {"MI_RAYLIB_POOL_TUNE", "pool_tune"}, {"MI_RAYLIB_POOL_WAVES", "pool_waves"}, {"MI_RAYLIB_CUS", "cus"},
                                          {"MI_RAYLIB_NIF_OVERLAP", "nif_overlap"}, {"MI_RAYLIB_COORDS", "coords"},
                                          {"MI_RAYLIB_NIF_TRACE_WGS", "nif_trace_wgs"}, {"MI_RAYLIB_NIF_SPLIT", "nif_split"}, {"MI_RAYLIB_NIF_GENERATIONS", "nif_generations"},
-                                         {"MI_RAYLIB_HOT_NODES", "hot_nodes"}};
+                                         {"MI_RAYLIB_HOT_NODES", "hot_nodes"}, {"MI_RAYLIB_LEAF_FRAME", "leaf_frame"}};
     for (const auto& m : map) if (const char* e = getenv(m[0])) (void)set(m[1], e);
     if (getenv("MI_RAYLIB_NO_TILES")) tiles = false;
     if (getenv("MI_RAYLIB_NO_ROOT_START")) rootStart = false;
@@ -310,11 +312,11 @@
   std::map<const void*, int> residentPerCU;
   uint32_t cus() const { return opt.cus ? opt.cus : (uint32_t)numCUs; }
   bool nifOverlapOn() const { return opt.nifOverlap < 0 ? (opt.nifSplit > 0 || !((opt.nifShape >= 6 && opt.nifShape <= 8) && nif_asm_covers(nif.regs))) : opt.nifOverlap != 0; }
-  DeviceScene view() const { DeviceScene v = ds; if (!opt.rootStart) v.rootInterior = 0; return v; }
+  DeviceScene view() const { DeviceScene v = ds; if (!opt.rootStart) v.rootInterior = 0; if (!opt.leafFrame && !v.hasNormals) v.leafNormalsOrFrames = nullptr; return v; }
   struct HotCopy { const GNode* nodes = nullptr; const GLeaf* leaves = nullptr; const GLeafRot* rot = nullptr; const float* leafNormals = nullptr; bool valid = false;
                    uint32_t numNodes = 0, thinNodes = 0, exactBase = 0;
                    std::vector<double> share; } hot, thin;
-  DeviceScene hotView(const HotCopy& c) const { DeviceScene v = view(); v.nodes = c.nodes; v.numNodes = c.numNodes; v.exactBase = c.exactBase; v.leaves = c.leaves; v.leavesRot = c.rot; v.leafNormals = c.leafNormals; return v; }
+  DeviceScene hotView(const HotCopy& c) const { DeviceScene v = view(); v.nodes = c.nodes; v.numNodes = c.numNodes; v.exactBase = c.exactBase; v.leaves = c.leaves; v.leavesRot = c.rot; if (v.hasNormals || opt.leafFrame) v.leafNormalsOrFrames = c.leafNormals; return v; }
   DeviceScene& touchArrays() { hot.valid = false; thin.valid = false; return ds; }
   void freeRetiredHot() {
     if (hot.valid || thin.valid) return;
@@ -644,7 +646,7 @@
   ds.materials = S.keep(upload(std::vector<mi_material>(d.materials, d.materials + d.num_materials)));
   ds.numMaterials = d.num_materials;
   ds.hasNormals = d.num_normals ? 1u : 0u;
-  ds.leafNormals = nullptr;
+  ds.leafNormalsOrFrames = nullptr;
   S.hot.leafNormals = S.thin.leafNormals = nullptr;
   S.hot.valid = S.thin.valid = true;
   if (ds.hasNormals) {
@@ -660,7 +662,7 @@
         ln[9 * k + 3 * c] = nn.x; ln[9 * k + 3 * c + 1] = nn.y; ln[9 * k + 3 * c + 2] = nn.z;
       }
     }
-    ds.leafNormals = S.keep(upload(ln));
+    ds.leafNormalsOrFrames = S.keep(upload(ln));
     for (Private& p : priv) {
       std::vector<float> hotLn(9 * p.at.size());
       for (uint32_t k = 0; k < p.at.size(); ++k) memcpy(&hotLn[9 * (size_t)k], &ln[9 * (size_t)p.at[k]], 9 * sizeof(float));
@@ -669,6 +671,22 @@
     ds.meshTris = S.keep(upload(std::vector<uint16_t>(d.mesh_tris, d.mesh_tris + 3 * (size_t)d.num_tris)));
     ds.meshNormals = S.keep(upload(std::vector<mi_vec3>(d.mesh_normals, d.mesh_normals + d.num_normals)));
     ds.geomFirstVertex = S.keep(upload(geomFirstVertex));
+  } else if (N) {
+    std::vector<uint8_t> framed(N);
+    std::vector<float> normal(3 * (size_t)N, 0.f);
+    for (uint32_t i = 0; i < N; ++i) {
+      const GLeaf& L = leaves[i];
+      framed[i] = isLeafNode[i] && leaf_kind(L) != LEAF_SPHERE;
+      if (framed[i]) memcpy(&normal[3 * (size_t)i], leaf_kind(L) == LEAF_TRI ? L.n : L.f, 3 * sizeof(float));
+    }
+    std::vector<GLeafFrame> fr(N);
+    fill_leaf_frames(framed.data(), normal.data(), nullptr, N, fr.data());
+    ds.leafNormalsOrFrames = reinterpret_cast<const float*>(S.keep(upload(fr)));
+    for (Private& p : priv) {
+      std::vector<GLeafFrame> hotFr(p.at.size());
+      fill_leaf_frames(framed.data(), normal.data(), p.at.data(), (uint32_t)p.at.size(), hotFr.data());
+      p.copy->leafNormals = reinterpret_cast<const float*>(S.keep(upload(hotFr)));
+    }
   }
   ds.rootInterior = 0;
   if (N > 1) {
@@ -816,6 +834,8 @@
 }
 
 uint32_t rebuildScene(mi_scene& S, hipStream_t stream);
+float* leafNormalsOf(const DeviceScene& ds) { return ds.hasNormals ? const_cast<float*>(ds.leafNormalsOrFrames) : nullptr; }
+GLeafFrame* leafFramesOf(const DeviceScene& ds) { return ds.hasNormals ? nullptr : reinterpret_cast<GLeafFrame*>(const_cast<float*>(ds.leafNormalsOrFrames)); }
 void refitScene(mi_scene& S, const mi_geometry_update& u, hipStream_t stream) {
   refitTables(S);
   mi_scene::Refit& R = S.refit;
@@ -869,7 +889,7 @@
   if (N) {
     if (timing) HIP_CHECK(hipEventRecord(R.ev[3], stream));
     hipLaunchKernelGGL(refit_write_kernel, dim3((N + 255) / 256), dim3(256), 0, stream, N, R.d_prims, cn, g, const_cast<GNode*>(ds.nodes),
-                       const_cast<GLeaf*>(ds.leaves), const_cast<GLeafRot*>(ds.leavesRot), const_cast<float*>(ds.leafNormals));
+                       const_cast<GLeaf*>(ds.leaves), const_cast<GLeafRot*>(ds.leavesRot), leafNormalsOf(ds), leafFramesOf(ds));
     HIP_CHECK(hipGetLastError());
   }
   if (u.mesh_verts && R.numVerts) HIP_CHECK(hipMemcpyAsync(R.d_verts, u.mesh_verts, (size_t)R.numVerts * sizeof(mi_vec3), hipMemcpyDeviceToDevice, stream));
@@ -1040,7 +1060,7 @@
   refitLevelRoom(S, R, H + 2);
   if (inPlace) for (LaunchSlot& l : S.slots) if (l.stream != stream) HIP_CHECK(hipStreamWaitEvent(stream, l.lastWork, 0));
   hipLaunchKernelGGL(rebuild_scatter_kernel, blocks(N), dim3(256), 0, stream, t, B.d_canon, g, R.d_cnodes[scratch], const_cast<GNode*>(ds.nodes),
-                     const_cast<GLeaf*>(ds.leaves), const_cast<GLeafRot*>(ds.leavesRot), const_cast<float*>(ds.leafNormals), R.d_prims);
+                     const_cast<GLeaf*>(ds.leaves), const_cast<GLeafRot*>(ds.leavesRot), leafNormalsOf(ds), leafFramesOf(ds), R.d_prims);
   HIP_CHECK(hipGetLastError());
   HIP_CHECK(hipMemcpyAsync(R.d_cnodes[1 - scratch], R.d_cnodes[scratch], (size_t)N * sizeof(mi_bvh_node), hipMemcpyDeviceToDevice, stream));
   HIP_CHECK(hipMemcpyAsync(R.d_order, byHeight, (size_t)N * sizeof(uint32_t), hipMemcpyDeviceToDevice, stream));
@@ -1126,11 +1146,11 @@
     for (int k = 0; k < 3; ++k) R.ms[k] = S.refit.ms[k];
     R.ready = true;
     GNode* nodes; GLeaf* leaves; GLeafRot* rot; float* leafNormals;
-    alloc(nodes, N); alloc(leaves, N); alloc(rot, N); alloc(leafNormals, g.num_normals ? 9 * (size_t)N : 0);
+    alloc(nodes, N); alloc(leaves, N); alloc(rot, N); alloc(leafNormals, (g.num_normals ? 9 : sizeof(GLeafFrame) / sizeof(float)) * (size_t)N);
     alloc(R.d_prims, N); alloc(R.d_order, N); alloc(R.d_boxes, N); alloc(R.d_cnodes[0], N); alloc(R.d_cnodes[1], N);
     ds.nodes = nodes; ds.numNodes = N; ds.leaves = leaves; ds.numLeaves = N; ds.leavesRot = rot;
     ds.matIDs = matIDs; ds.materials = materials; ds.numMaterials = g.num_materials;
-    ds.hasNormals = g.num_normals ? 1u : 0u; ds.leafNormals = leafNormals;
+    ds.hasNormals = g.num_normals ? 1u : 0u; ds.leafNormalsOrFrames = leafNormals;
     ds.meshTris = tris; ds.meshNormals = normals; ds.geomFirstVertex = firstVertex;
     ds.rootInterior = 0;
     ds.rootLoX = ds.rootHiX = ds.rootLoY = ds.rootHiY = ds.rootLoZ = ds.rootHiZ = 0.f;
@@ -1168,7 +1188,7 @@
   for (void* p : staged) (void)hipFree(p);
   const DeviceScene& o = S.ds;
   const mi_scene::Refit& oR = S.refit;
-  std::vector<const void*> old = {o.nodes, o.leaves, o.leavesRot, o.matIDs, o.materials, o.leafNormals, o.meshTris, o.meshNormals, o.geomFirstVertex,
+  std::vector<const void*> old = {o.nodes, o.leaves, o.leavesRot, o.matIDs, o.materials, o.leafNormalsOrFrames, o.meshTris, o.meshNormals, o.geomFirstVertex,
                                   oR.d_prims, oR.d_order, oR.d_boxes, oR.d_cnodes[0], oR.d_cnodes[1], oR.d_levelStart, oR.d_verts, oR.d_spheres, oR.d_discs,
                                   S.rebuild.d_canon, S.live.d_cost,
                                   S.hot.nodes, S.hot.leaves, S.hot.rot, S.hot.leafNormals,
diff --git a/ipu_ray_lib_amd/csrc/rebuild_kernels.hpp b/ipu_ray_lib_amd/csrc/rebuild_kernels.hpp
--- a/ipu_ray_lib_amd/csrc/rebuild_kernels.hpp
+++ b/ipu_ray_lib_amd/csrc/rebuild_kernels.hpp
@@ -168,7 +168,7 @@
 }
 
 __global__ void __launch_bounds__(256) rebuild_scatter_kernel(RebuildTree t, const RebuildPrim* canon, RefitGeom g, mi_bvh_node* cnodes,
-                                                              GNode* nodes, GLeaf* leaves, GLeafRot* rot, float* leafNormals, RefitPrim* prims) {
+                                                              GNode* nodes, GLeaf* leaves, GLeafRot* rot, float* leafNormals, GLeafFrame* leafFrames, RefitPrim* prims) {
   const uint32_t n = blockIdx.x * blockDim.x + threadIdx.x;
   const uint32_t P = t.numPrims, I = P - 1;
   if (n >= 2 * P - 1) return;
@@ -186,6 +186,7 @@
   __builtin_memset(&L, 0, sizeof L);
   __builtin_memset(&R, 0, sizeof R);
   float vn[9] = {0.f, 0.f, 0.f, 0.f, 0.f, 0.f, 0.f, 0.f, 0.f};
+  GLeafFrame F = leaf_frame_zero();
   RefitPrim rp;
   if (n < I) {
     const uint2 ch = t.child[n];
@@ -210,6 +211,7 @@
         const uint32_t v[3] = {p.a, p.b, p.c};
         for (int k = 0; k < 3; ++k) { const mi_vec3 q = g.normals[v[k]]; vn[3 * k] = q.x; vn[3 * k + 1] = q.y; vn[3 * k + 2] = q.z; }
       }
+      if (leafFrames) F = leaf_frame_of(fn);
     } else if (p.kind == REFIT_SPHERE) {
       const mi_sphere s = g.spheres[p.a];
       L.f[0] = s.x; L.f[1] = s.y; L.f[2] = s.z; L.f[3] = s.radius; L.f[4] = s.radius * s.radius;
@@ -218,6 +220,7 @@
       const mi_disc d = g.discs[p.a];
       L.f[0] = d.nx; L.f[1] = d.ny; L.f[2] = d.nz; L.f[3] = d.cx; L.f[4] = d.cy; L.f[5] = d.cz; L.f[6] = d.r * d.r;
       L.type = LEAF_DISC | (p.geomID << 16);
+      if (leafFrames) F = leaf_frame_of(mk(L.f[0], L.f[1], L.f[2]));
     }
     for (uint32_t kz = 0; kz < 3; ++kz) {
       GLeafBlock& B = R.b[kz];
@@ -235,6 +238,7 @@
   leaves[i] = L;
   rot[i] = R;
   if (leafNormals) for (int k = 0; k < 9; ++k) leafNormals[9 * (size_t)i + k] = vn[k];
-}
-
-}
+  if (leafFrames) leafFrames[i] = F;
+}
+
+}
diff --git a/ipu_ray_lib_amd/csrc/refit_kernels.hpp b/ipu_ray_lib_amd/csrc/refit_kernels.hpp
--- a/ipu_ray_lib_amd/csrc/refit_kernels.hpp
+++ b/ipu_ray_lib_amd/csrc/refit_kernels.hpp
@@ -76,7 +76,7 @@
 }
 
 __global__ void __launch_bounds__(256) refit_write_kernel(uint32_t n, const RefitPrim* prims, const mi_bvh_node* cnodes, RefitGeom g,
-                                                          GNode* nodes, GLeaf* leaves, GLeafRot* rot, float* leafNormals) {
+                                                          GNode* nodes, GLeaf* leaves, GLeafRot* rot, float* leafNormals, GLeafFrame* leafFrames) {
   const uint32_t i = blockIdx.x * blockDim.x + threadIdx.x;
   if (i >= n) return;
   const mi_bvh_node c = cnodes[i];
@@ -108,6 +108,7 @@
     L.f[0] = d.nx; L.f[1] = d.ny; L.f[2] = d.nz; L.f[3] = d.cx; L.f[4] = d.cy; L.f[5] = d.cz; L.f[6] = d.r * d.r;
   }
   leaves[i] = L;
+  if (leafFrames && p.kind != REFIT_SPHERE) leafFrames[i] = leaf_frame_of(p.kind == REFIT_TRI ? mk(L.n[0], L.n[1], L.n[2]) : mk(L.f[0], L.f[1], L.f[2]));
   for (uint32_t kz = 0; kz < 3; ++kz) {
     GLeafBlock B;
     B.type = L.type;
diff --git a/ipu_ray_lib_amd/csrc/trace_kernels.hpp b/ipu_ray_lib_amd/csrc/trace_kernels.hpp
--- a/ipu_ray_lib_amd/csrc/trace_kernels.hpp
+++ b/ipu_ray_lib_amd/csrc/trace_kernels.hpp
@@ -3,6 +3,7 @@
 #include <hip/hip_runtime.h>
 
 #include "ray_math.h"
+#include "leaf_frame.hpp"
 #include "../../include/mi_raylib.h"
 
 namespace mi {
@@ -42,7 +43,7 @@
   const uint32_t* matIDs;
   const mi_material* materials; uint32_t numMaterials;
   const uint16_t* meshTris; const mi_vec3* meshNormals; const uint32_t* geomFirstVertex; uint32_t hasNormals;
-  const float* leafNormals;
+  const float* leafNormalsOrFrames;
   float imageWidth, imageHeight, tanTheta, antiAliasScale;
   uint32_t maxPathLength, rouletteStartDepth, samplesPerPixel;
   uint64_t rngSeed;
@@ -342,7 +343,7 @@
   const GLeaf L = sc.leaves[h.leaf];
   if (leaf_kind(L) == LEAF_TRI) {
     if (!sc.hasNormals) return mk(L.n[0], L.n[1], L.n[2]);
-    const float* q = sc.leafNormals + 9 * (size_t)h.leaf;
+    const float* q = sc.leafNormalsOrFrames + 9 * (size_t)h.leaf;
     return normalized((mk(q[0], q[1], q[2]) * h.b0) + (mk(q[3], q[4], q[5]) * h.b1) + (mk(q[6], q[7], q[8]) * h.b2));
   }
   if (leaf_kind(L) == LEAF_SPHERE) return normalized(hp - mk(L.f[0], L.f[1], L.f[2]));
diff --git a/ipu_ray_lib_amd/csrc/trace_wavefront.hpp b/ipu_ray_lib_amd/csrc/trace_wavefront.hpp
--- a/ipu_ray_lib_amd/csrc/trace_wavefront.hpp
+++ b/ipu_ray_lib_amd/csrc/trace_wavefront.hpp
@@ -416,6 +416,14 @@
         bool terminated = false;
         if (hit.leaf != 0xFFFFFFFFu) {
           const GLeaf L = sc.leaves[hit.leaf];
+          constexpr bool kLeafFrame = !BARY && SLOTS == 0;
+          f3 frX = mk(0.f, 0.f, 0.f), frY = frX;
+          if constexpr (kLeafFrame) {
+            if (sc.leafNormalsOrFrames != nullptr) {
+              const GLeafFrame* fr = reinterpret_cast<const GLeafFrame*>(reinterpret_cast<const char*>(sc.leafNormalsOrFrames) + (hit.leaf << 5));
+              frX = mk(fr->xb[0], fr->xb[1], fr->xb[2]); frY = mk(fr->yb[0], fr->yb[1], fr->yb[2]);
+            }
+          }
           hit.geomID = leaf_geom(L);
           coldU(6) = hit.leaf; coldF(7) = hit.t;
           o = o + d * hit.t;
@@ -427,6 +435,11 @@
           if (mat.type == 0) {
             const float u1 = rng_uniform01(rng);
             const float u2 = rng_uniform01(rng);
+            if constexpr (kLeafFrame) {
+              f3 xb = frX, yb = frY;
+              if ((frX.x == 0.f) & (frX.y == 0.f) & (frX.z == 0.f)) diffuse_frame(nrm, xb, yb);
+              d = diffuse_in_frame(nrm, xb, yb, u1, u2, sinTbl);
+            } else
             d = sample_diffuse(nrm, u1, u2, sinTbl);
             tp = tp * albedo;
           } else if (mat.type == 1) {
```

After: 21.60 billion (median of 6 runs). +2.5%, better.
